# bruniss/multi-task-3d-resencoder-unet

Hardware: AMD Instinct MI355X
Metric: train patches/sec (b,c,z,y,x) ResEncM 1x128^3 (higher is better)
Workload: dtype bf16; 1 GPU; cfg2: ResEncM (6 stages, feats [32, 64, 128, 256, 512, 512], blocks [1, 3, 4, 6, 6, 6]), 1-in, heads ['sheet'], patch 128x128x128, batch 2/GPU, full train step (fwd+loss+bwd+allreduce+clip+AdamW); global_batch=2, parallelism=dp1

## Files before the change

include/rxunet.h:

```cpp
#ifndef RXUNET_H
#define RXUNET_H

#include <stddef.h>
#include <stdint.h>

#ifdef __cplusplus
extern "C" {
#endif

#define RX_OK 0
#define RX_EINVAL (-1)
#define RX_EUNSUPPORTED (-2)
#define RX_ELAUNCH (-3)
#define RX_EWORKSPACE (-4)

typedef enum { RX_F32 = 0, RX_BF16 = 1, RX_F16 = 2 } rx_dtype;
typedef enum { RX_ACT_NONE = 0, RX_ACT_SIGMOID = 1, RX_ACT_SOFTMAX = 2 } rx_head_act;

typedef struct {
  void* ptr;
  int32_t n, z, y, x, c, ld;
  int64_t cs;
} rx_act;

int rx_abi_version(void);
const char* rx_last_error(void);
int rx_device_arch_ok(void);
const char* rx_last_conv_kernel(void);

int rx_pack_conv_weight(rx_dtype dt, const float* w, int co, int ci, int taps, void* w_fwd, void* w_bwd,
                        void* stream);
int rx_pack_convT_weight(rx_dtype dt, const float* w, int ci, int co, int taps, void* w_fwd, void* w_bwd,
                         void* stream);
int rx_pack_multi(rx_dtype dt, int count, const float* const* w, const int* kind, const int* A, const int* B,
                  const int* taps, void* const* w_fwd, void* const* w_bwd, void* stream);

size_t rx_conv_workspace_hint(void);
int rx_conv3d_fwd(rx_dtype dt, const rx_act* x, const void* w_fwd, const float* bias, const rx_act* y,
                  const int32_t kernel[3], const int32_t stride[3], void* ws, size_t ws_bytes, void* stream);
int rx_conv3d_fwd_stats(rx_dtype dt, const rx_act* x, const void* w_fwd, const float* bias, const rx_act* y,
                        const int32_t kernel[3], const int32_t stride[3], float eps, float* stats, void* ws,
                        size_t ws_bytes, void* stream);
int rx_conv3d_bwd_data(rx_dtype dt, const rx_act* dy, const void* w_bwd, const rx_act* dx,
                       const int32_t kernel[3], const int32_t stride[3], int accumulate, void* ws,
                       size_t ws_bytes, void* stream);
int rx_conv3d_bwd_data_instats(rx_dtype dt, const rx_act* dy, const void* w_bwd, const rx_act* dx,
                               const int32_t kernel[3], const int32_t stride[3], int accumulate, const rx_act* in_y,
                               const float* in_stats, float slope, float* m12, int* fused, void* ws, size_t ws_bytes,
                               void* stream);
size_t rx_conv3d_bwd_weight_workspace(const rx_act* x, const rx_act* dy, const int32_t kernel[3]);
int rx_conv3d_bwd_weight(rx_dtype dt, const rx_act* x, const rx_act* dy, float* dw, const int32_t kernel[3],
                         const int32_t stride[3], void* ws, size_t ws_bytes, void* stream);

int rx_convT3d_fwd(rx_dtype dt, const rx_act* x, const void* w_fwd, const float* bias, const rx_act* y,
                   const int32_t stride[3], void* ws, size_t ws_bytes, void* stream);
int rx_convT3d_bwd_data(rx_dtype dt, const rx_act* dy, const void* w_bwd, const rx_act* dx,
                        const int32_t stride[3], int accumulate, void* ws, size_t ws_bytes, void* stream);
size_t rx_convT3d_bwd_weight_workspace(const rx_act* x, const rx_act* dy, const int32_t stride[3]);
int rx_convT3d_bwd_weight(rx_dtype dt, const rx_act* x, const rx_act* dy, float* dw, const int32_t stride[3],
                          void* ws, size_t ws_bytes, void* stream);

size_t rx_instnorm_stats_workspace(const rx_act* y);
int rx_instnorm_stats(rx_dtype dt, const rx_act* y, float eps, float* stats, void* ws, size_t ws_bytes,
                      void* stream);
int rx_instnorm_stats_mask(float* stats, const float* keep, int count, void* stream);
int rx_instnorm_act_fwd(rx_dtype dt, const rx_act* y, const float* stats, const rx_act* residual,
                        const rx_act* out, float slope, void* stream);
int rx_instnorm_fwd(rx_dtype dt, const rx_act* y, float eps, float* stats, const rx_act* residual,
                    const rx_act* out, float slope, void* ws, size_t ws_bytes, void* stream);
int rx_instnorm_act_bwd(rx_dtype dt, const rx_act* g, const rx_act* y, const float* stats, const rx_act* out,
                        float slope, const rx_act* dy, const rx_act* d_residual, int accumulate_residual,
                        void* ws, size_t ws_bytes, void* stream);

int rx_instnorm_act_bwd_res(rx_dtype dt, const rx_act* g, const rx_act* y, const float* stats, const rx_act* out,
                            float slope, const rx_act* pool_dy, const int32_t pool_stride[3], const rx_act* d_residual,
                            const rx_act* dy, void* ws, size_t ws_bytes, void* stream);

int rx_instnorm_act_bwd_apply(rx_dtype dt, const rx_act* g, const rx_act* y, const float* stats, const rx_act* out,
                              float slope, const float* m12, const rx_act* dy, const rx_act* d_residual,
                              int accumulate_residual, void* stream);

typedef struct {
  const float* w1;
  const float* b1;
  const float* w2;
  const float* b2;
  int32_t rd;
  int32_t keep_x;
} rx_se_params;
size_t rx_se_workspace(const rx_act* y);
int rx_se_gate_fwd(rx_dtype dt, const rx_act* y, const float* stats, const float* path_scale, const rx_se_params* se,
                   float* pooled, float* hidden, float* gate, float* mult, void* ws, size_t ws_bytes, void* stream);
int rx_instnorm_gate_act_fwd(rx_dtype dt, const rx_act* y, const float* stats, const float* mult, int keep_x,
                             const rx_act* residual, const rx_act* out, float slope, void* stream);
int rx_se_gate_bwd(rx_dtype dt, const rx_act* g, const rx_act* y, const float* stats, const rx_act* out, float slope,
                   const float* path_scale, const rx_se_params* se, const float* pooled, const float* hidden,
                   const float* gate, const float* mult, float* dadd, float* m12, float* dw1, float* db1, float* dw2,
                   float* db2, void* ws, size_t ws_bytes, void* stream);
int rx_instnorm_gate_act_bwd(rx_dtype dt, const rx_act* g, const rx_act* y, const float* stats, const rx_act* out,
                             float slope, const float* mult, const float* dadd, const float* m12, int keep_x,
                             const rx_act* dy, const rx_act* d_residual, int accumulate_residual, void* stream);

int rx_avgpool_fwd(rx_dtype dt, const rx_act* x, const rx_act* y, const int32_t stride[3], void* stream);
int rx_instnorm_act_pool_fwd(rx_dtype dt, const rx_act* y, const float* stats, const rx_act* residual,
                             const rx_act* out, const rx_act* pooled, const int32_t stride[3], float slope,
                             void* stream);
int rx_avgpool_bwd(rx_dtype dt, const rx_act* dy, const rx_act* dx, const int32_t stride[3], int accumulate,
                   void* stream);

int rx_stem_conv_fwd(rx_dtype dt, const float* x_ncdhw, int n, int cin, int z, int y, int x, const float* w,
                     const float* bias, const rx_act* out, const int32_t kernel[3], void* stream);
int rx_stem_conv_fwd_stats(rx_dtype dt, const float* x_ncdhw, int n, int cin, int z, int y, int x, const float* w,
                           const float* bias, const rx_act* out, const int32_t kernel[3], float eps, float* stats,
                           void* ws, size_t ws_bytes, void* stream);
size_t rx_stem_conv_bwd_weight_workspace(int cin, int cout, int taps);
int rx_stem_conv_bwd_weight(rx_dtype dt, const float* x_ncdhw, int n, int cin, int z, int y, int x,
                            const rx_act* dy, float* dw, const int32_t kernel[3], void* ws, size_t ws_bytes,
                            void* stream);

int rx_head_fwd(rx_dtype dt, const rx_act* x, const float* w, const float* b, int k, float* out_ncdhw,
                int act, void* stream);
size_t rx_head_bwd_workspace(const rx_act* x, int k);
int rx_head_bwd(rx_dtype dt, const float* dout_ncdhw, const rx_act* x, const float* w, int k, const rx_act* dx,
                float* dw, float* db, void* ws, size_t ws_bytes, void* stream);

int rx_instnorm_act_head_fwd(rx_dtype dt, const rx_act* y, const float* stats, const rx_act* out, float slope,
                             const float* head_w, const float* head_b, int k, float* out_ncdhw, int act, void* stream);

int rx_instnorm_act_bwd_head(rx_dtype dt, const float* dout_ncdhw, int k, const float* head_w, const rx_act* y,
                             const float* stats, float slope, const rx_act* dy, float* head_dw, float* head_db, void* ws,
                             size_t ws_bytes, void* stream);

size_t rx_channel_sum_workspace(const rx_act* x);
int rx_channel_sum(rx_dtype dt, const rx_act* x, float* out, void* ws, size_t ws_bytes, void* stream);

size_t rx_loss_workspace(int n, int c, long v);
int rx_bce_dice_loss_fwd(const float* logits, const float* target, int n, int c, long v, float alpha, float beta,
                         float smoothing, float eps, float* loss, float* coef, void* ws, size_t ws_bytes,
                         void* stream);
int rx_bce_dice_loss_bwd(const float* logits, const float* target, int n, int c, long v, float alpha, float beta,
                         float smoothing, const float* coef, const float* grad_loss, float* dlogits, void* stream);
int rx_masked_cosine_loss_fwd(const float* pred, const float* target, int n, int c, long v, float* loss, float* coef,
                              void* ws, size_t ws_bytes, void* stream);
int rx_masked_cosine_loss_bwd(const float* pred, const float* target, int n, int c, long v, const float* coef,
                              const float* grad_loss, float* dpred, void* stream);

typedef enum { RX_LOSS_BCE_LOGITS = 0, RX_LOSS_BCE_PROB = 1, RX_LOSS_MSE = 2 } rx_elem_loss_kind;
typedef enum { RX_REDUCE_MEAN = 0, RX_REDUCE_SUM = 1 } rx_reduction;
int rx_elem_loss_fwd(int kind, const float* x, const float* target, int n, int c, long v, float smoothing,
                     const float* alpha_z, int z, int reduction, float* loss, void* ws, size_t ws_bytes, void* stream);
int rx_elem_loss_bwd(int kind, const float* x, const float* target, int n, int c, long v, float smoothing,
                     const float* alpha_z, int z, int reduction, const float* grad_loss, float* dx, void* stream);
size_t rx_cross_entropy_loss_workspace(int n, int c, long v);
int rx_cross_entropy_loss_fwd(const float* logits, const float* target_prob, const int64_t* target_index,
                              int64_t ignore_index, int n, int c, long v, int reduction, float* loss, float* coef,
                              float* saved, void* ws, size_t ws_bytes, void* stream);
int rx_cross_entropy_loss_bwd(const float* logits, const float* target_prob, const int64_t* target_index,
                              int64_t ignore_index, int n, int c, long v, const float* coef, const float* saved,
                              const float* grad_loss, float* dlogits, void* stream);

int rx_adamw_pack(rx_dtype dt, float* p, const float* grad, float* exp_avg, float* exp_avg_sq, const float* clip, double lr,
                  double beta1, double beta2, double eps, double weight_decay, int step, int kind, int A, int B, int taps,
                  void* w_fwd, void* w_bwd, void* stream);
int rx_adamw_flat(float* p, const float* grad, float* exp_avg, float* exp_avg_sq, const float* clip, double lr, double beta1,
                  double beta2, double eps, double weight_decay, int step, long n, void* stream);
long rx_grad_norm_clip_partials(int count, const long* numel);
int rx_grad_norm_clip(int count, const float* const* grad, const long* numel, float max_norm, float* partial, long partial_len,
                      float* out, void* stream);
int rx_adamw_flat_multi(int count, float* const* p, const float* const* grad, float* const* exp_avg,
                        float* const* exp_avg_sq, const long* numel, const float* clip, double lr, double beta1,
                        double beta2, double eps, double weight_decay, int step, void* stream);

typedef struct rx_prog rx_prog;
rx_prog* rx_prog_create(void);
void rx_prog_destroy(rx_prog* p);
int rx_prog_begin(rx_prog* p, void* const* streams, int n_streams);
int rx_prog_end(rx_prog* p);
int rx_prog_len(const rx_prog* p);
const char* rx_prog_cmd_name(const rx_prog* p, int i);
const char* rx_prog_cmd_kernel(const rx_prog* p, int i);
int rx_prog_cmd_stream(const rx_prog* p, int i);
int rx_prog_run(rx_prog* p, int first, int last, void* const* streams, int n_streams, float* ms);
int rx_event_new(void);
int rx_event_free(int slot);
int rx_event_slots_in_use(void);
int rx_event_record(int slot, void* stream);
int rx_stream_wait(int slot, void* stream);

typedef enum { RX_SW_U8 = 0, RX_SW_U16 = 1, RX_SW_F32 = 2 } rx_sw_in_dtype;
typedef enum { RX_SW_SCALE = 0, RX_SW_ZSCORE = 1 } rx_sw_norm;
typedef enum { RX_SW_BLEND_AVERAGE = 0, RX_SW_BLEND_UNIT = 1, RX_SW_BLEND_NONE = 2 } rx_sw_blend;
typedef enum { RX_SW_CAST_U8 = 0, RX_SW_CAST_U16 = 1 } rx_sw_cast;
size_t rx_sw_gather_workspace(int batch, int cin, int pz, int py, int px);
int rx_sw_gather(int in_dtype, const void* slab, int cin, int ring, int y, int x, int batch, const int32_t* origins, int pz,
                 int py, int px, int norm, float* out, void* ws, size_t ws_bytes, void* stream);
int rx_sw_accumulate(const float* logits, int batch, int valid, int c, int pz, int py, int px, const int32_t* origins, int act,
                     const float* weight, float* sum, float* wsum, int ring, int y, int x, void* stream);
int rx_sw_finalize(float* sum, float* wsum, int c, int ring, int y, int x, int z0, int rows, int blend, int cast, int reset,
                   float* blended, void* final_out, float* wsum_out, void* stream);

#define RX_AUG_MAX_K 21
#define RX_AUG_MAX_BOXES 4
typedef enum { RX_AUG_PW_NONE = 0, RX_AUG_PW_AFFINE = 1, RX_AUG_PW_PLANE = 2, RX_AUG_PW_NOISE = 3 } rx_aug_pw_mode;
typedef enum { RX_AUG_G3_NONE = 0, RX_AUG_G3_FILTER = 1, RX_AUG_G3_DOWNSCALE = 2 } rx_aug_g3_mode;
typedef struct {
  int32_t pw_mode[2];
  float pw_a[2], pw_b[2];
  int32_t pw_off[2];
  uint32_t key_lo, key_hi;
  int32_t g3_mode, k, g3_off;
  int32_t nbox;
  int32_t box[RX_AUG_MAX_BOXES][6];
  float fill;
  int32_t pad_;
} rx_aug_sample;
size_t rx_aug_workspace(int batch, int c, int z, int y, int x);
int rx_aug_pointwise(const float* in, float* out, float* scratch, size_t scratch_bytes, int batch, int c, int z, int y, int x,
                     const rx_aug_sample* host_table, const void* table, long pool_words, void* stream);
int rx_aug_filter_zy(const float* scratch, float* out, int batch, int c, int z, int y, int x, const rx_aug_sample* host_table,
                     const void* table, long pool_words, void* stream);
int rx_aug_philox_u32(uint64_t key, long n, uint32_t* out, void* stream);

typedef struct {
  int32_t src_axis[3];
  int32_t flip[3];
  int32_t ch_src[3];
  int32_t ch_neg[3];
} rx_geom_sample;
int rx_geom_apply(const float* in, float* out, int batch, int c, int z, int y, int x, const rx_geom_sample* host_table,
                  int vector, void* stream);

int rx_sw_gather_geom(int in_dtype, const void* slab, int cin, int ring, int y, int x, int batch, const int32_t* origins,
                      const rx_geom_sample* ops, int pz, int py, int px, int norm, float* out, void* ws, size_t ws_bytes,
                      void* stream);
int rx_sw_accumulate_geom(const float* logits, int batch, int valid, int c, int pz, int py, int px, const int32_t* origins,
                          const rx_geom_sample* ops, int vector, int act, const float* weight, float* sum, float* wsum, int ring,
                          int y, int x, void* stream);

size_t rx_dilate_workspace(int batch, int c, int z, int y, int x);
int rx_label_dilate(const float* in, float* out, void* scratch, size_t scratch_bytes, int batch, int c, int z, int y, int x,
                    int radius, void* stream);

#ifdef __cplusplus
}
#endif
#endif
```

multi-task-3d-resencoder-unet_amd/csrc/rx_internal.h:

```cpp
#pragma once
#include "rx_common.h"

int rx_note_seq(void);

int rx_conv_halo_try(rx_dtype dt, const rx_act* in, const void* w, const float* bias, const rx_act* out, int flip, int accumulate,
                     hipStream_t st, float* stat_part, size_t stat_bytes, int* stat_chunks, const RxBwdStat* bs);
int rx_pointwise_try(rx_dtype dt, const rx_act* in, const void* w, const float* bias, const rx_act* out, const int32_t stride[3],
                     int accumulate, hipStream_t st);
int rx_dgrad_s2_halo_try(rx_dtype dt, const rx_act* dy, const void* w_bwd, const rx_act* dx, int accumulate, hipStream_t st);

size_t rx_wgrad_halo_ws_bytes(const rx_act* x, const rx_act* dy);
int rx_wgrad_halo_try(rx_dtype dt, const rx_act* x, const rx_act* dy, const int32_t stride[3], float* dw, void* ws, size_t ws_bytes,
                      hipStream_t st);
void rx_wgrad_reduce_launch(const float* slab, int S, int T_, int R, int C, float* dw, hipStream_t st);

int rx_stem_fwd_mfma_try(rx_dtype dt, const float* x, int n, int cin, int z, int y, int xx, const float* w, const float* bias,
                         const rx_act* out, const int32_t kernel[3], hipStream_t st, float* stat_part, size_t stat_bytes, int* stat_chunks);
int rx_stem_wgrad_mfma_try(rx_dtype dt, const float* x, int n, int cin, int z, int y, int xx, const rx_act* dy, const int32_t kernel[3],
                           float* partial, int max_blocks, int* nblocks_out, hipStream_t st);

void rx_colreduce_finalize_launch(hipStream_t st, const float* partial, int N, int nchunks, int nacc, int C, double V, float eps, int mode,
                                  float* out);
void rx_stats_finalize_launch(const float* partial, int N, int nchunks, int C, double V, float eps, float* stats, hipStream_t st);
void rx_inbwd_fused_finalize_launch(const float* partial, int N, int nchunks, int C, double V, const float* stats, float* m12, hipStream_t st);
```

multi-task-3d-resencoder-unet_amd/csrc/rx_pack_optim.hip:

```cpp
#include <math.h>

#include "rx_common.h"

#define RX_PACK_PB 40
#ifndef RX_PACK_THREADS
#define RX_PACK_THREADS 1024
#endif

template <typename T>
__device__ __forceinline__ void pack_tile(const float* __restrict__ w, int A, int B, int TT, unsigned inv_tt, T* __restrict__ same,
                                          int flip_same, T* __restrict__ swp, int flip_swap, const int a0, const int b0) {
  extern __shared__ __attribute__((aligned(16))) unsigned char pack_smem[];
  T* L = reinterpret_cast<T*>(pack_smem);
  const int rowlen = 32 * TT;
  const bool full = a0 + 32 <= A && b0 + 32 <= B && sizeof(T) == 2 && (B & 7) == 0 && (A & 7) == 0;
  if (full && TT > 1 && (rowlen & 3) == 0 && ((size_t)B * TT & 3) == 0) {
    const int q4 = rowlen >> 2;
    for (int q = threadIdx.x; q < 32 * q4; q += RX_PACK_THREADS) {
      const int a = q / q4, c = q - a * q4;
      const f32x4 v = *reinterpret_cast<const f32x4*>(w + ((size_t)(a0 + a) * B + b0) * TT + 4 * c);
#pragma unroll
      for (int j = 0; j < 4; ++j) {
        const unsigned r = 4 * c + j;
        const unsigned b = __umulhi(r, inv_tt), t = r - b * TT;
// ... 380 lines not shown
        pm[j][k] = mj, pv[j][k] = vj;
      }
      *reinterpret_cast<f32x4*>(w + i) = pw[j];
      *reinterpret_cast<f32x4*>(m + i) = pm[j];
      *reinterpret_cast<f32x4*>(v + i) = pv[j];
    }
    return;
  }
  const long end = base + RX_AM_CHUNK < n ? base + RX_AM_CHUNK : n;
  for (long i = base + threadIdx.x; i < end; i += 256) {
    float mj = m[i], vj = v[i];
    w[i] = adamw_update(w[i], grad[i] * cs, mj, vj, aa);
    m[i] = mj, v[i] = vj;
  }
}

extern "C" int rx_adamw_flat_multi(int count, float* const* p, const float* const* grad, float* const* exp_avg, float* const* exp_avg_sq,
                                   const long* numel, const float* clip, double lr, double beta1, double beta2, double eps,
                                   double weight_decay, int step, void* stream) {
  if (count < 0 || (count > 0 && (!p || !grad || !exp_avg || !exp_avg_sq || !numel)) || step < 1) RX_FAIL(RX_EINVAL, "rx_adamw_flat_multi: bad arguments");
  const AdamArgs aa = adam_args(lr, beta1, beta2, eps, weight_decay, step);
  for (int i = 0; i < count; ++i)
    if (!p[i] || !grad[i] || !exp_avg[i] || !exp_avg_sq[i] || numel[i] < 1) RX_FAIL(RX_EINVAL, "rx_adamw_flat_multi: bad tensor %d", i);
  for (int i0 = 0; i0 < count;) {
    AdamMulti t;
    int k = 0;
    long blocks = 0;
    for (; i0 + k < count && k < RX_AM_MAX; ++k) {
      const long nb = (numel[i0 + k] + RX_AM_CHUNK - 1) / RX_AM_CHUNK;
      if (blocks + nb > 0x3fffffffL) break;
      t.p[k] = p[i0 + k], t.g[k] = grad[i0 + k], t.m[k] = exp_avg[i0 + k], t.v[k] = exp_avg_sq[i0 + k], t.n[k] = numel[i0 + k];
      t.start[k] = (int)blocks;
      blocks += nb;
    }
    if (k == 0) RX_FAIL(RX_EINVAL, "rx_adamw_flat_multi: tensor %d too large", i0);
    for (int q = k; q <= RX_AM_MAX; ++q) t.start[q] = (int)blocks;
    for (int q = k; q < RX_AM_MAX; ++q) t.p[q] = nullptr, t.g[q] = nullptr, t.m[q] = nullptr, t.v[q] = nullptr, t.n[q] = 0;
    t.count = k;
    hipLaunchKernelGGL(adamw_multi_kernel, dim3((unsigned)blocks), dim3(256), 0, (hipStream_t)stream, t, clip, aa);
    i0 += k;
  }
  RX_CHECK_LAUNCH("rx_adamw_flat_multi");
  return RX_OK;
}

struct SqnormMulti {
  const float* g[RX_AM_MAX];
  long n[RX_AM_MAX];
  int start[RX_AM_MAX + 1];
  int count;
};

__global__ __launch_bounds__(256) void sqnorm_multi_kernel(const SqnormMulti t, float* __restrict__ partial) {
  __shared__ float red[4];
  const int b = blockIdx.x;
  int lo = 0, hi = t.count;
  while (hi - lo > 1) {
    const int mid = (lo + hi) >> 1;
    if (t.start[mid] <= b) lo = mid; else hi = mid;
  }
  const long base = (long)(b - t.start[lo]) * RX_AM_CHUNK;
  const long n = t.n[lo];
  const float* __restrict__ g = t.g[lo];
  float s = 0.f;
  if ((((uintptr_t)g) & 15) == 0 && base + RX_AM_CHUNK <= n) {
    f32x4 v[4];
#pragma unroll
    for (int j = 0; j < 4; ++j) v[j] = *reinterpret_cast<const f32x4*>(g + base + (long)(j * 256 + threadIdx.x) * 4);
#pragma unroll
    for (int j = 0; j < 4; ++j)
#pragma unroll
      for (int k = 0; k < 4; ++k) s += v[j][k] * v[j][k];
  } else {
    const long end = base + RX_AM_CHUNK < n ? base + RX_AM_CHUNK : n;
    for (long i = base + threadIdx.x; i < end; i += 256) s += g[i] * g[i];
  }
  for (int o = 32; o > 0; o >>= 1) s += __shfl_xor(s, o, 64);
  if ((threadIdx.x & 63) == 0) red[threadIdx.x >> 6] = s;
  __syncthreads();
  if (threadIdx.x == 0) partial[b] = (red[0] + red[1]) + (red[2] + red[3]);
}

__global__ __launch_bounds__(1024) void sqnorm_finalize_kernel(const float* __restrict__ partial, int nblocks, float max_norm,
                                                               float* __restrict__ out ) {
  __shared__ double red[1024];
  double s[8] = {0.0, 0.0, 0.0, 0.0, 0.0, 0.0, 0.0, 0.0};
  int i = threadIdx.x;
  for (; i + 7 * 1024 < nblocks; i += 8 * 1024) {
    float v[8];
#pragma unroll
    for (int u = 0; u < 8; ++u) v[u] = partial[i + u * 1024];
#pragma unroll
    for (int u = 0; u < 8; ++u) s[u] += (double)v[u];
  }
  for (; i < nblocks; i += 1024) s[0] += (double)partial[i];
  red[threadIdx.x] = ((s[0] + s[1]) + (s[2] + s[3])) + ((s[4] + s[5]) + (s[6] + s[7]));
  __syncthreads();
  for (int o = 512; o > 0; o >>= 1) {
    if ((int)threadIdx.x < o) red[threadIdx.x] += red[threadIdx.x + o];
    __syncthreads();
  }
  if (threadIdx.x == 0) {
    const float norm = (float)sqrt(red[0]);
    const float coef = max_norm / (norm + 1e-6f);
    out[0] = norm;
    out[1] = coef < 1.f ? coef : 1.f;
  }
}

extern "C" long rx_grad_norm_clip_partials(int count, const long* numel) {
  long blocks = 0;
  for (int i = 0; i < count; ++i) blocks += (numel[i] + RX_AM_CHUNK - 1) / RX_AM_CHUNK;
  return blocks;
}

extern "C" int rx_grad_norm_clip(int count, const float* const* grad, const long* numel, float max_norm, float* partial, long partial_len,
                                 float* out, void* stream) {
  if (count < 1 || !grad || !numel || !partial || !out) RX_FAIL(RX_EINVAL, "rx_grad_norm_clip: bad arguments");
  const long need = rx_grad_norm_clip_partials(count, numel);
  if (need > partial_len || need > 0x3fffffffL) RX_FAIL(RX_EWORKSPACE, "rx_grad_norm_clip: %ld partials needed, %ld given", need, partial_len);
  long done = 0;
  for (int i0 = 0; i0 < count;) {
    SqnormMulti t;
    int k = 0;
    long blocks = 0;
    for (; i0 + k < count && k < RX_AM_MAX; ++k) {
      if (!grad[i0 + k] || numel[i0 + k] < 1) RX_FAIL(RX_EINVAL, "rx_grad_norm_clip: bad tensor %d", i0 + k);
      t.g[k] = grad[i0 + k], t.n[k] = numel[i0 + k];
      t.start[k] = (int)blocks;
      blocks += (numel[i0 + k] + RX_AM_CHUNK - 1) / RX_AM_CHUNK;
    }
    for (int q = k; q <= RX_AM_MAX; ++q) t.start[q] = (int)blocks;
    for (int q = k; q < RX_AM_MAX; ++q) t.g[q] = nullptr, t.n[q] = 0;
    t.count = k;
    hipLaunchKernelGGL(sqnorm_multi_kernel, dim3((unsigned)blocks), dim3(256), 0, (hipStream_t)stream, t, partial + done);
    done += blocks;
    i0 += k;
  }
  hipLaunchKernelGGL(sqnorm_finalize_kernel, dim3(1), dim3(1024), 0, (hipStream_t)stream, (const float*)partial, (int)done, max_norm, out);
  RX_CHECK_LAUNCH("rx_grad_norm_clip");
  return RX_OK;
}
```

multi-task-3d-resencoder-unet_amd/csrc/rx_wgrad.hip:

```cpp
#include <stdlib.h>

#include "rx_common.h"
#include "rx_internal.h"


struct WgradGeom {
  int Qz, Qy, Qx, Vq, NQ;
  int R, ldg;
  long g_ss;
  int Zx, Yx, Xx, Cc, ldx;
  long x_ss;
  int isz, isy, isx;
  int ntaps, ksplit, q_per_split, tiles_c;
  RxTap taps[RX_MAX_TAPS];
};


typedef __attribute__((address_space(3))) s16x4 lds_s16x4;

template <typename T>
__device__ inline u32x4 fetch_frag(const T* panel, int ks, int lane) {
  if constexpr (sizeof(T) == 2) {
    const int g16 = lane >> 4, half = g16 & 1, h = g16 >> 1, l15 = lane & 15, q4 = l15 >> 2, p4 = l15 & 3;
    const T* a0 = panel + (ks * 16 + 8 * h + q4) * 32 + 16 * half + 4 * p4;
// ... 50 lines not shown
        const int n = q / g.Vq, vq = q - n * g.Vq;
        const int qx = vq % g.Qx, t = vq / g.Qx;
        const int qy = t % g.Qy, qz = t / g.Qy;
        const int z = qz * g.isz + tp.dz, y = qy * g.isy + tp.dy, x = qx * g.isx + tp.dx;
        if ((unsigned)z < (unsigned)g.Zx && (unsigned)y < (unsigned)g.Yx && (unsigned)x < (unsigned)g.Xx)
          v = *reinterpret_cast<const u32x4*>(xt + n * g.x_ss + ((long)(z * g.Yx + y) * g.Xx + x) * g.ldx + c0 + cv * P);
      }
      xr[j] = v;
    }
  };
  auto store_tile = [&](int buf) {
    T* base = sbuf + buf * TILE_ELEMS;
#pragma unroll
    for (int j = 0; j < GV; ++j) {
      const int i = tid + 256 * j, vox = i / (BR / P), cv = i - vox * (BR / P);
      const int c = cv * P;
      *reinterpret_cast<u32x4*>(base + ((c >> 5) * 64 + vox) * 32 + (c & 31)) = gr[j];
    }
    T* xb = base + 64 * BR;
#pragma unroll
    for (int j = 0; j < XV; ++j) {
      const int i = tid + 256 * j, vox = i / (BC / P), cv = i - vox * (BC / P);
      const int c = cv * P;
      *reinterpret_cast<u32x4*>(xb + ((c >> 5) * 64 + vox) * 32 + (c & 31)) = xr[j];
    }
  };

  f32x16 acc[NR][NC];
#pragma unroll
  for (int a = 0; a < NR; ++a)
#pragma unroll
    for (int b = 0; b < NC; ++b)
#pragma unroll
      for (int r = 0; r < 16; ++r) acc[a][b][r] = 0.f;

  if (q_begin < q_end) {
    load_tile(q_begin);
    store_tile(0);
  }
  __syncthreads();
  int it = 0;
  for (int q0 = q_begin; q0 < q_end; q0 += 64, ++it) {
    const int buf = it & 1;
    if (q0 + 64 < q_end) load_tile(q0 + 64);
    const T* base = sbuf + buf * TILE_ELEMS;
#pragma unroll
    for (int kk = 0; kk < KSTEPS / 4; ++kk) {
      const int ks = wave + 4 * kk;
      u32x4 af[NR], bf[NC];
#pragma unroll
      for (int a = 0; a < NR; ++a) af[a] = fetch_frag<T>(base + a * 64 * 32, ks, lane);
#pragma unroll
      for (int b = 0; b < NC; ++b) bf[b] = fetch_frag<T>(base + 64 * BR + b * 64 * 32, ks, lane);
#pragma unroll
      for (int a = 0; a < NR; ++a)
#pragma unroll
        for (int b = 0; b < NC; ++b) Mma<T>::run(acc[a][b], af[a], bf[b]);
    }
    if (q0 + 64 < q_end) store_tile(buf ^ 1);
    __syncthreads();
  }

  float* red = reinterpret_cast<float*>(smem);
  const int col = lane & 31, fh = lane >> 5;
#pragma unroll
  for (int a = 0; a < NR; ++a)
#pragma unroll
    for (int b = 0; b < NC; ++b)
#pragma unroll
      for (int r = 0; r < 16; ++r) {
        const int row = (r & 3) + 8 * (r >> 2) + 4 * fh;
        red[(((wave * NR + a) * NC + b) * 32 + row) * 32 + col] = acc[a][b][r];
      }
  __syncthreads();
  float* out = slab + ((long)blockIdx.z * g.ntaps + blockIdx.y) * g.R * g.Cc;
  for (int i = tid; i < NR * NC * 1024; i += 256) {
    const int blk = i >> 10, rc = i & 1023, row = rc >> 5, cc = rc & 31;
    const int a = blk / NC, b = blk - a * NC;
    float s = red[i] + red[i + NR * NC * 1024] + red[i + 2 * NR * NC * 1024] + red[i + 3 * NR * NC * 1024];
    out[(long)(r0 + a * 32 + row) * g.Cc + c0 + b * 32 + cc] = s;
  }
}

__global__ __launch_bounds__(256) void wgrad_reduce(const float* __restrict__ slab, int S, int T_, int R, int C, float* __restrict__ dw) {
  __shared__ float tile[27 * 257];
  const long RC = (long)R * C;
  const long base = (long)blockIdx.x * 256;
  const long i = base + threadIdx.x;
  for (int t = 0; t < T_; ++t) {
    float s = 0.f;
    if (i < RC)
      for (int k = 0; k < S; ++k) s += slab[((long)k * T_ + t) * RC + i];
    tile[t * 257 + threadIdx.x] = s;
  }
  __syncthreads();
  const long n_here = (RC - base < 256 ? RC - base : 256) * T_;
  for (long j = threadIdx.x; j < n_here; j += 256) {
    int pair = (int)(j / T_), t = (int)(j - (long)pair * T_);
    dw[base * T_ + j] = tile[t * 257 + pair];
  }
}

__global__ __launch_bounds__(256) void wgrad_reduce_manysplits(const float* __restrict__ slab, int S, int T_, int R, int C,
                                                               float* __restrict__ dw) {
  const long RC = (long)R * C;
  const long i = (long)blockIdx.x * 256 + threadIdx.x;
  const int t = blockIdx.y;
  if (i >= RC) return;
  const float* p = slab + (long)t * RC + i;
  const long stride = (long)T_ * RC;
  float a0 = 0.f, a1 = 0.f, a2 = 0.f, a3 = 0.f, a4 = 0.f, a5 = 0.f, a6 = 0.f, a7 = 0.f;
  int k = 0;
  for (; k + 8 <= S; k += 8) {
    a0 += p[(k + 0) * stride];
    a1 += p[(k + 1) * stride];
    a2 += p[(k + 2) * stride];
    a3 += p[(k + 3) * stride];
    a4 += p[(k + 4) * stride];
    a5 += p[(k + 5) * stride];
    a6 += p[(k + 6) * stride];
    a7 += p[(k + 7) * stride];
  }
  for (; k < S; ++k) a0 += p[k * stride];
  dw[i * T_ + t] = ((a0 + a1) + (a2 + a3)) + ((a4 + a5) + (a6 + a7));
}

static int plan_split(const WgradGeom& g, int BR, int BC, size_t ws_bytes, int* ksplit, int* qps) {
  const long tiles = (long)(g.R / BR) * (g.Cc / BC) * g.ntaps;
  const long ktiles = ((long)g.NQ + 63) / 64;
  long S = (1024 + tiles - 1) / tiles;
  if (S > ktiles / 4) S = ktiles / 4;
  if (S < 1) S = 1;
  const size_t slab1 = (size_t)g.ntaps * g.R * g.Cc * sizeof(float);
  while (S > 1 && S * slab1 > ws_bytes) --S;
  if (slab1 > ws_bytes) return RX_EWORKSPACE;
  long per = (ktiles + S - 1) / S;
  S = (ktiles + per - 1) / per;
  *ksplit = (int)S;
  *qps = (int)(per * 64);
  return RX_OK;
}

static size_t wgrad_ws_bytes(int R, int C, int taps, long NQ) {
  const size_t slab1 = (size_t)taps * R * C * sizeof(float);
  const long tiles = (long)((R + 63) / 64) * ((C + 63) / 64) * taps;
  long S = (1024 + tiles - 1) / tiles;
  long ktiles = (NQ + 63) / 64;
  if (S > ktiles / 4) S = ktiles / 4;
  if (S < 1) S = 1;
  if (R % 64 || C % 64) {
    const long t32 = (long)(R / 32) * (C / 32) * taps;
    long S2 = (1024 + t32 - 1) / t32;
    if (S2 > S) S = S2;
  }
  return S * slab1 + 256;
}

template <typename T>
static void wgrad_dispatch(int BR, int BC, dim3 grid, hipStream_t st, const void* gt, const void* xt, float* slab, const WgradGeom& g) {
  const size_t lds = 65536;
#define RX_WG(BR_, BC_)                                                                                                            \
  do {                                                                                                                             \
    (void)hipFuncSetAttribute(reinterpret_cast<const void*>(&wgrad_kernel<T, BR_, BC_>), hipFuncAttributeMaxDynamicSharedMemorySize, \
                              (int)lds);                                                                                           \
    hipLaunchKernelGGL((wgrad_kernel<T, BR_, BC_>), grid, dim3(256), lds, st, (const T*)gt, (const T*)xt, slab, g);                \
  } while (0)
  if (BR == 64 && BC == 64)
    RX_WG(64, 64);
  else if (BR == 64 && BC == 32)
    RX_WG(64, 32);
  else if (BR == 32 && BC == 64)
    RX_WG(32, 64);
  else
    RX_WG(32, 32);
#undef RX_WG
}

static int wgrad_launch(rx_dtype dt, const void* gt, const void* xt, float* dw, WgradGeom& g, void* ws, size_t ws_bytes, hipStream_t st) {
  const int per16 = dt == RX_F32 ? 4 : 8;
  if (g.R % 32 || g.Cc % 32) RX_FAIL(RX_EUNSUPPORTED, "wgrad: channel counts must be multiples of 32 (R=%d C=%d)", g.R, g.Cc);
  if (g.ldg % per16 || g.ldx % per16 || ((uintptr_t)gt & 15) || ((uintptr_t)xt & 15)) RX_FAIL(RX_EUNSUPPORTED, "wgrad: misaligned operand");
  if (!ws || !dw) RX_FAIL(RX_EINVAL, "wgrad: null workspace / output");
  const int BR = g.R % 64 == 0 ? 64 : 32, BC = g.Cc % 64 == 0 ? 64 : 32;
  g.tiles_c = g.Cc / BC;
  int rc = plan_split(g, BR, BC, ws_bytes, &g.ksplit, &g.q_per_split);
  if (rc) RX_FAIL(rc, "wgrad: workspace too small (%zu bytes)", ws_bytes);
  dim3 grid((g.R / BR) * (g.Cc / BC), g.ntaps, g.ksplit);
  rx_note_kernel(BR == 64 ? (BC == 64 ? "wgrad_kernel<64,64>" : "wgrad_kernel<64,32>") : (BC == 64 ? "wgrad_kernel<32,64>" : "wgrad_kernel<32,32>"));
  RX_DISPATCH_DTYPE(dt, T, wgrad_dispatch<T>(BR, BC, grid, st, gt, xt, (float*)ws, g));
  rx_wgrad_reduce_launch((const float*)ws, g.ksplit, g.ntaps, g.R, g.Cc, dw, st);
  RX_CHECK_LAUNCH("wgrad");
  return RX_OK;
}

static int conv_out_dim(int in, int k, int s) { return (in + 2 * ((k - 1) / 2) - k) / s + 1; }

void rx_wgrad_reduce_launch(const float* slab, int S, int T_, int R, int C, float* dw, hipStream_t st) {
  long RC = (long)R * C;
  if (S >= 8 || T_ > 27)
    hipLaunchKernelGGL(wgrad_reduce_manysplits, dim3((unsigned)((RC + 255) / 256), T_), dim3(256), 0, st, slab, S, T_, R, C, dw);
  else
    hipLaunchKernelGGL(wgrad_reduce, dim3((unsigned)((RC + 255) / 256)), dim3(256), 0, st, slab, S, T_, R, C, dw);
}

extern "C" size_t rx_conv3d_bwd_weight_workspace(const rx_act* x, const rx_act* dy, const int32_t kernel[3]) {
  if (!rx_act_ok_planar(x) || !rx_act_ok(dy)) return 0;
  size_t a = wgrad_ws_bytes(dy->c, x->c, kernel[0] * kernel[1] * kernel[2], (long)dy->n * rx_act_voxels(dy));
  size_t b = (kernel[0] == 3 && kernel[1] == 3 && kernel[2] == 3) ? rx_wgrad_halo_ws_bytes(x, dy) : 0;
  return a > b ? a : b;
}

extern "C" int rx_conv3d_bwd_weight(rx_dtype dt, const rx_act* x, const rx_act* dy, float* dw, const int32_t kernel[3],
                                    const int32_t stride[3], void* ws, size_t ws_bytes, void* stream) {
  RX_RECORD(stream, [=, x_ = RxActV(x), dy_ = RxActV(dy), kernel_ = RxI3V(kernel), stride_ = RxI3V(stride)](void* s) { return rx_conv3d_bwd_weight(dt, x_.p(), dy_.p(), dw, kernel_.v, stride_.v, ws, ws_bytes, s); });
  if (!rx_act_ok_planar(x) || !rx_act_ok(dy)) RX_FAIL(RX_EINVAL, "rx_conv3d_bwd_weight: bad arguments");
  for (int i = 0; i < 3; ++i) {
    if (kernel[i] < 1 || kernel[i] > RX_MAX_KERNEL) RX_FAIL(RX_EUNSUPPORTED, "rx_conv3d_bwd_weight: kernel sizes must be 1..%d per axis", RX_MAX_KERNEL);
    if (stride[i] < 1 || stride[i] > RX_MAX_STRIDE) RX_FAIL(RX_EUNSUPPORTED, "rx_conv3d_bwd_weight: strides must be 1..%d per axis", RX_MAX_STRIDE);
  }
  if (dy->n != x->n || dy->z != conv_out_dim(x->z, kernel[0], stride[0]) || dy->y != conv_out_dim(x->y, kernel[1], stride[1]) ||
      dy->x != conv_out_dim(x->x, kernel[2], stride[2]))
    RX_FAIL(RX_EINVAL, "rx_conv3d_bwd_weight: geometry mismatch");
  if (kernel[0] == 3 && kernel[1] == 3 && kernel[2] == 3 && ws && dw) {
    int rc = rx_wgrad_halo_try(dt, x, dy, stride, dw, ws, ws_bytes, (hipStream_t)stream);
    if (rc < 0) return rc;
    if (rc == 1) return RX_OK;
  }
  if (x->cs) RX_FAIL(RX_EUNSUPPORTED, "rx_conv3d_bwd_weight: a planar-concat x needs the LDS-halo weight-gradient kernels");
  WgradGeom g;
  memset(&g, 0, sizeof(g));
  g.Qz = dy->z, g.Qy = dy->y, g.Qx = dy->x, g.Vq = (int)rx_act_voxels(dy), g.NQ = dy->n * g.Vq;
  g.R = dy->c, g.ldg = dy->ld, g.g_ss = (long)g.Vq * dy->ld;
  g.Zx = x->z, g.Yx = x->y, g.Xx = x->x, g.Cc = x->c, g.ldx = x->ld, g.x_ss = rx_act_voxels(x) * (long)x->ld;
  g.isz = stride[0], g.isy = stride[1], g.isx = stride[2];
  const int pz = (kernel[0] - 1) / 2, py = (kernel[1] - 1) / 2, px = (kernel[2] - 1) / 2;
  for (int a = 0; a < kernel[0]; ++a)
    for (int b = 0; b < kernel[1]; ++b)
      for (int c = 0; c < kernel[2]; ++c) {
        RxTap& t = g.taps[g.ntaps];
        t.dz = (int8_t)(a - pz), t.dy = (int8_t)(b - py), t.dx = (int8_t)(c - px);
        t.w = (uint16_t)g.ntaps;
        ++g.ntaps;
      }
  return wgrad_launch(dt, dy->ptr, x->ptr, dw, g, ws, ws_bytes, (hipStream_t)stream);
}

struct ConvTWgGeom {
  int Vq, NQ, Qy, Qx;
  int R, ldr;
  long r_ss;
  int Yf, Xf, Cc, ldc;
  long c_ss;
  int sz, sy, sx, ntaps;
  int q_per_split;
};

template <typename T, int NR, int NC>
__global__ __launch_bounds__(512) void convT_wgrad_kernel(const T* __restrict__ xt, const T* __restrict__ yt, float* __restrict__ slab,
                                                          const ConvTWgGeom g) {
  constexpr int P = Elem<T>::PER16;
  constexpr int BR = 32 * NR, BC = 32 * NC;
  constexpr int XV = (64 * BR / P + 511) / 512;
  constexpr int YV = (64 * BC / P + 511) / 512;
  extern __shared__ __attribute__((aligned(16))) unsigned char smem[];
  T* sX = reinterpret_cast<T*>(smem);
  T* sY = sX + 64 * BR;
  const int tid = threadIdx.x, lane = tid & 63;
  const int wave = __builtin_amdgcn_readfirstlane(tid >> 6);
  const int q_begin = blockIdx.x * g.q_per_split;
  const int q_end = min(g.NQ, q_begin + g.q_per_split);

  u32x4 xr[XV], yr[8][YV];
  auto load_tile = [&](int q0) {
#pragma unroll
    for (int j = 0; j < XV; ++j) {
      const int i = tid + 512 * j, vox = i / (BR / P), cv = i - vox * (BR / P);
      const int q = q0 + vox;
      u32x4 v = u32x4{0u, 0u, 0u, 0u};
      if (vox < 64 && q < q_end) {
        const int n = q / g.Vq, vq = q - n * g.Vq;
        v = *reinterpret_cast<const u32x4*>(xt + n * g.r_ss + (long)vq * g.ldr + cv * P);
      }
      xr[j] = v;
    }
#pragma unroll
    for (int j = 0; j < YV; ++j) {
      const int i = tid + 512 * j, vox = i / (BC / P), cv = i - vox * (BC / P);
      const int q = q0 + vox;
      const bool ok = vox < 64 && q < q_end;
      const int n = ok ? q / g.Vq : 0, vq = ok ? q - n * g.Vq : 0;
      const int qx = vq % g.Qx, t2 = vq / g.Qx;
      const int qy = t2 % g.Qy, qz = t2 / g.Qy;
      const T* base = yt + n * g.c_ss + cv * P;
#pragma unroll
      for (int t = 0; t < 8; ++t) {
        u32x4 v = u32x4{0u, 0u, 0u, 0u};
        if (ok && t < g.ntaps) {
          const int c = t % g.sx, b = (t / g.sx) % g.sy, a = t / (g.sx * g.sy);
          const long fv = ((long)(qz * g.sz + a) * g.Yf + (qy * g.sy + b)) * g.Xf + (qx * g.sx + c);
          v = *reinterpret_cast<const u32x4*>(base + fv * g.ldc);
        }
        yr[t][j] = v;
      }
    }
  };
  auto store_tile = [&]() {
#pragma unroll
    for (int j = 0; j < XV; ++j) {
      const int i = tid + 512 * j, vox = i / (BR / P), cv = i - vox * (BR / P);
      const int c = cv * P;
      if (vox < 64) *reinterpret_cast<u32x4*>(sX + ((c >> 5) * 64 + vox) * 32 + (c & 31)) = xr[j];
    }
#pragma unroll
    for (int j = 0; j < YV; ++j) {
      const int i = tid + 512 * j, vox = i / (BC / P), cv = i - vox * (BC / P);
      const int c = cv * P;
      if (vox < 64) {
#pragma unroll
        for (int t = 0; t < 8; ++t)
          if (t < g.ntaps) *reinterpret_cast<u32x4*>(sY + (long)t * 64 * BC + ((c >> 5) * 64 + vox) * 32 + (c & 31)) = yr[t][j];
      }
    }
  };

  f32x16 acc[NR][NC];
#pragma unroll
  for (int a = 0; a < NR; ++a)
#pragma unroll
    for (int b = 0; b < NC; ++b)
#pragma unroll
      for (int r = 0; r < 16; ++r) acc[a][b][r] = 0.f;

  if (q_begin < q_end) load_tile(q_begin);
  for (int q0 = q_begin; q0 < q_end; q0 += 64) {
    __syncthreads();
    store_tile();
    __syncthreads();
    if (q0 + 64 < q_end) load_tile(q0 + 64);
    if (wave < g.ntaps) {
      const T* yb = sY + (long)wave * 64 * BC;
#pragma unroll
      for (int ks = 0; ks < 4; ++ks) {
        u32x4 af[NR], bf[NC];
#pragma unroll
        for (int a = 0; a < NR; ++a) af[a] = fetch_frag<T>(sX + a * 64 * 32, ks, lane);
#pragma unroll
        for (int b = 0; b < NC; ++b) bf[b] = fetch_frag<T>(yb + b * 64 * 32, ks, lane);
#pragma unroll
        for (int a = 0; a < NR; ++a)
#pragma unroll
          for (int b = 0; b < NC; ++b) Mma<T>::run(acc[a][b], af[a], bf[b]);
      }
    }
  }
  if (wave < g.ntaps) {
    const int col = lane & 31, fh = lane >> 5;
    float* out = slab + ((long)blockIdx.x * g.ntaps + wave) * g.R * g.Cc;
#pragma unroll
    for (int a = 0; a < NR; ++a)
#pragma unroll
      for (int b = 0; b < NC; ++b)
#pragma unroll
        for (int r = 0; r < 16; ++r) {
          const int row = (r & 3) + 8 * (r >> 2) + 4 * fh;
          out[(long)(a * 32 + row) * g.Cc + b * 32 + col] = acc[a][b][r];
        }
  }
}

static int convT_wgrad_splits(long NQ, size_t slab1) {
  long ktiles = (NQ + 63) / 64;
  long S = ktiles / 8;
  if (S > 256) S = 256;
  while (S > 32 && (size_t)S * slab1 > ((size_t)32 << 20)) S /= 2;
  if (S < 1) S = 1;
  return (int)S;
}

static int convT_wgrad_try(rx_dtype dt, const rx_act* x, const rx_act* dy, const int32_t stride[3], float* dw, void* ws, size_t ws_bytes,
                           hipStream_t st) {
  const int taps = stride[0] * stride[1] * stride[2];
  const int R = x->c, C = dy->c;
  if (dt == RX_F32 || taps > 8 || R % 32 || C % 32 || x->ld % 8 || dy->ld % 8 || ((uintptr_t)x->ptr & 15) || ((uintptr_t)dy->ptr & 15)) return 0;
  const int NR = R / 32, NC = C / 32;
  if (!((NR == 2 && NC == 1) || (NR == 4 && NC == 2) || (NR == 1 && NC == 1) || (NR == 2 && NC == 2))) return 0;
  const long NQ = (long)x->n * rx_act_voxels(x);
  if (NQ < 32768) return 0;
  const size_t slab1 = (size_t)taps * R * C * sizeof(float);
  const int S = convT_wgrad_splits(NQ, slab1);
  if ((size_t)S * slab1 > ws_bytes) return 0;
  ConvTWgGeom g;
  g.Vq = (int)rx_act_voxels(x), g.NQ = (int)NQ, g.Qy = x->y, g.Qx = x->x;
  g.R = R, g.ldr = x->ld, g.r_ss = (long)g.Vq * x->ld;
  g.Yf = dy->y, g.Xf = dy->x, g.Cc = C, g.ldc = dy->ld, g.c_ss = rx_act_voxels(dy) * (long)dy->ld;
  g.sz = stride[0], g.sy = stride[1], g.sx = stride[2], g.ntaps = taps;
  const long ktiles = (NQ + 63) / 64;
  g.q_per_split = (int)(((ktiles + S - 1) / S) * 64);
  const int S2 = (int)((NQ + g.q_per_split - 1) / g.q_per_split);
  const size_t lds = (size_t)64 * (R + taps * C) * 2;
  rx_note_kernel("convT_wgrad_kernel");
#define RX_CTW(NR_, NC_)                                                                                                              \
  do {                                                                                                                                \
    (void)hipFuncSetAttribute(reinterpret_cast<const void*>(&convT_wgrad_kernel<T, NR_, NC_>), hipFuncAttributeMaxDynamicSharedMemorySize, 160 * 1024); \
    hipLaunchKernelGGL((convT_wgrad_kernel<T, NR_, NC_>), dim3(S2), dim3(512), lds, st, (const T*)x->ptr, (const T*)dy->ptr, (float*)ws, g);            \
  } while (0)
#define RX_CTW_ALL()                       \
  if (NR == 2 && NC == 1) RX_CTW(2, 1);    \
  else if (NR == 4 && NC == 2) RX_CTW(4, 2); \
  else if (NR == 1 && NC == 1) RX_CTW(1, 1); \
  else RX_CTW(2, 2)
  if (dt == RX_BF16) {
    using T = bf16_t;
    RX_CTW_ALL();
  } else {
    using T = f16_t;
    RX_CTW_ALL();
  }
#undef RX_CTW_ALL
#undef RX_CTW
  rx_wgrad_reduce_launch((const float*)ws, S2, taps, R, C, dw, st);
  return 1;
}

extern "C" size_t rx_convT3d_bwd_weight_workspace(const rx_act* x, const rx_act* dy, const int32_t stride[3]) {
  if (!rx_act_ok(x) || !rx_act_ok(dy)) return 0;
  const int taps = stride[0] * stride[1] * stride[2];
  const long NQ = (long)x->n * rx_act_voxels(x);
  const size_t slab1 = (size_t)taps * x->c * dy->c * sizeof(float);
  const size_t a = wgrad_ws_bytes(x->c, dy->c, taps, NQ);
  const size_t b = (size_t)convT_wgrad_splits(NQ, slab1) * slab1 + 256;
  return a > b ? a : b;
}

extern "C" int rx_convT3d_bwd_weight(rx_dtype dt, const rx_act* x, const rx_act* dy, float* dw, const int32_t stride[3], void* ws,
                                     size_t ws_bytes, void* stream) {
  RX_RECORD(stream, [=, x_ = RxActV(x), dy_ = RxActV(dy), stride_ = RxI3V(stride)](void* s) { return rx_convT3d_bwd_weight(dt, x_.p(), dy_.p(), dw, stride_.v, ws, ws_bytes, s); });
  if (!rx_act_ok(x) || !rx_act_ok(dy)) RX_FAIL(RX_EINVAL, "rx_convT3d_bwd_weight: bad arguments");
  for (int i = 0; i < 3; ++i)
    if (stride[i] < 1 || stride[i] > RX_MAX_STRIDE) RX_FAIL(RX_EUNSUPPORTED, "rx_convT3d_bwd_weight: strides must be 1..%d per axis", RX_MAX_STRIDE);
  if (dy->n != x->n || dy->z != x->z * stride[0] || dy->y != x->y * stride[1] || dy->x != x->x * stride[2])
    RX_FAIL(RX_EINVAL, "rx_convT3d_bwd_weight: geometry mismatch");
  if (ws && dw) {
    const int rc = convT_wgrad_try(dt, x, dy, stride, dw, ws, ws_bytes, (hipStream_t)stream);
    if (rc < 0) return rc;
    if (rc == 1) {
      RX_CHECK_LAUNCH("rx_convT3d_bwd_weight(convT_wgrad)");
      return RX_OK;
    }
  }
  WgradGeom g;
  memset(&g, 0, sizeof(g));
  g.Qz = x->z, g.Qy = x->y, g.Qx = x->x, g.Vq = (int)rx_act_voxels(x), g.NQ = x->n * g.Vq;
  g.R = x->c, g.ldg = x->ld, g.g_ss = (long)g.Vq * x->ld;
  g.Zx = dy->z, g.Yx = dy->y, g.Xx = dy->x, g.Cc = dy->c, g.ldx = dy->ld, g.x_ss = rx_act_voxels(dy) * (long)dy->ld;
  g.isz = stride[0], g.isy = stride[1], g.isx = stride[2];
  for (int a = 0; a < stride[0]; ++a)
    for (int b = 0; b < stride[1]; ++b)
      for (int c = 0; c < stride[2]; ++c) {
        RxTap& t = g.taps[g.ntaps];
        t.dz = (int8_t)a, t.dy = (int8_t)b, t.dx = (int8_t)c;
        t.w = (uint16_t)g.ntaps;
        ++g.ntaps;
      }
  return wgrad_launch(dt, x->ptr, dy->ptr, dw, g, ws, ws_bytes, (hipStream_t)stream);
}
```

multi-task-3d-resencoder-unet_amd/csrc/rx_wgrad_halo.hip:

```cpp
#include <stdlib.h>

#include <type_traits>

#include "rx_common.h"
#include "rx_internal.h"

struct WgHaloGeom {
  int N, Z, Y, X;
  int R, Cc, ldg, ldx;
  long g_ss, x_ss;
  long x_cs;
  int TZ, TY, TX, lTX, lTY;
  int HY, HX, HV, VT;
  int tz_n, ty_n, tx_n, NT;
  int S, tiles_per_split, panels_c;
  int sz, sy, sx;
  int Zi, Yi, Xi;
  int order;
  int dbg;
};

typedef __attribute__((address_space(3))) s16x4 lds_s16x4_h;

#define RX_WGH_MAX_HV 768
#define RX_WGH_MAX_VT 256
#define RX_WGH_XPIECES ((RX_WGH_MAX_HV * 4 + 255) / 256)
#define RX_WGH_GPIECES (RX_WGH_MAX_VT * 4 / 256)

template <typename T>
__device__ inline u32x4 tr_frag(const T* p0, const T* p1) {
  s16x4 t0 = __builtin_amdgcn_ds_read_tr16_b64_v4i16((lds_s16x4_h*)(p0));
  s16x4 t1 = __builtin_amdgcn_ds_read_tr16_b64_v4i16((lds_s16x4_h*)(p1));
  u32x2 lo = __builtin_bit_cast(u32x2, t0), hi = __builtin_bit_cast(u32x2, t1);
  return u32x4{lo[0], lo[1], hi[0], hi[1]};
}

template <typename T>
__global__ __launch_bounds__(256, 2) void wgrad_halo_kernel(const T* __restrict__ gt, const T* __restrict__ xt, float* __restrict__ slab,
                                                            float* __restrict__ dw, const WgHaloGeom g) {
  extern __shared__ __attribute__((aligned(16))) unsigned char smem[];
  T* sG = reinterpret_cast<T*>(smem);
  T* sX = sG + RX_WGH_MAX_VT * 32;

  const int tid = threadIdx.x, lane = tid & 63;
  const int wave = __builtin_amdgcn_readfirstlane(tid >> 6);
  const int PPn = gridDim.x, lid = rx_xcd_remap(blockIdx.y * PPn + blockIdx.x, PPn * gridDim.y);
  const int split = lid / PPn, pp = lid - split * PPn;
  const int pr = pp / g.panels_c, pc = pp - pr * g.panels_c;
  const int r0 = pr * 32, c0 = pc * 32;
  const long xc0 = g.x_cs ? (long)pc * g.x_cs : (long)c0;
  const int t_begin = split * g.tiles_per_split;
  const int t_end = min(g.NT, t_begin + g.tiles_per_split);

  const int chunk = tid & 3;
  int xh[RX_WGH_XPIECES];
#pragma unroll
  for (int p = 0; p < RX_WGH_XPIECES; ++p) {
    int row = (tid >> 2) + 64 * p;
    if (row < g.HV) {
      int hx = row % g.HX, t = row / g.HX;
      int hy = t % g.HY, hz = t / g.HY;
      xh[p] = (hz << 16) | (hy << 8) | hx;
    } else
      xh[p] = -1;
  }

  const int g16 = lane >> 4, half = g16 & 1, h = g16 >> 1, l15 = lane & 15, q4 = l15 >> 2, p4 = l15 & 3;
  const int coloff = 16 * half + 4 * p4;
  int toff[7];
#pragma unroll
  for (int j = 0; j < 7; ++j) {
    int t = wave + 4 * j;
    int dz = t / 9 - 1, dy = (t / 3) % 3 - 1, dx = t % 3 - 1;
    toff[j] = t < 27 ? ((dz * g.HY + dy) * g.HX + dx) * 32 : 0;
  }

  f32x16 acc[7];
#pragma unroll
  for (int j = 0; j < 7; ++j)
#pragma unroll
    for (int r = 0; r < 16; ++r) acc[j][r] = 0.f;

  const int ksteps = g.VT >> 4;
  u32x4 gv[RX_WGH_GPIECES], xv[RX_WGH_XPIECES];
  auto load_tile = [&](int tile) {
    int tx, ty, tz, n;
    rx_tile_coords(tile, g.tx_n, g.ty_n, g.tz_n, g.order, n, tz, ty, tx);
    const int z0 = tz * g.TZ, y0 = ty * g.TY, x0 = tx * g.TX;
    const T* gn = gt + n * g.g_ss + r0;
    const T* xn = xt + n * g.x_ss + xc0;
#pragma unroll
    for (int p = 0; p < RX_WGH_GPIECES; ++p) {
      int v = (tid >> 2) + 64 * p;
      u32x4 val = u32x4{0u, 0u, 0u, 0u};
      if (v < g.VT) {
        int vx = v & (g.TX - 1), vy = (v >> g.lTX) & (g.TY - 1), vz = v >> (g.lTX + g.lTY);
        int z = z0 + vz, y = y0 + vy, x = x0 + vx;
        if (z < g.Z && y < g.Y && x < g.X)
          val = *reinterpret_cast<const u32x4*>(gn + ((long)(z * g.Y + y) * g.X + x) * g.ldg + chunk * 8);
      }
      gv[p] = val;
    }
#pragma unroll
    for (int p = 0; p < RX_WGH_XPIECES; ++p) {
      u32x4 val = u32x4{0u, 0u, 0u, 0u};
      if (xh[p] >= 0) {
        int z = z0 * g.sz + (xh[p] >> 16) - 1, y = y0 * g.sy + ((xh[p] >> 8) & 255) - 1, x = x0 * g.sx + (xh[p] & 255) - 1;
        if ((unsigned)z < (unsigned)g.Zi && (unsigned)y < (unsigned)g.Yi && (unsigned)x < (unsigned)g.Xi)
          val = *reinterpret_cast<const u32x4*>(xn + ((long)(z * g.Yi + y) * g.Xi + x) * g.ldx + chunk * 8);
      }
      xv[p] = val;
    }
  };
  if (t_begin < t_end) load_tile(t_begin);
  for (int tile = t_begin; tile < t_end; ++tile) {
    __syncthreads();
#pragma unroll
    for (int p = 0; p < RX_WGH_GPIECES; ++p) {
      int v = (tid >> 2) + 64 * p;
      if (v < g.VT) *reinterpret_cast<u32x4*>(sG + v * 32 + chunk * 8) = gv[p];
    }
#pragma unroll
    for (int p = 0; p < RX_WGH_XPIECES; ++p) {
      int row = (tid >> 2) + 64 * p;
      if (xh[p] >= 0) *reinterpret_cast<u32x4*>(sX + row * 32 + chunk * 8) = xv[p];
    }
    __syncthreads();
    if (tile + 1 < t_end) load_tile(tile + 1);
    for (int s = 0; s < ksteps; ++s) {
      const int v = 16 * s + 8 * h + q4;
      const int vx = v & (g.TX - 1), vy = (v >> g.lTX) & (g.TY - 1), vz = v >> (g.lTX + g.lTY);
      const int hr = ((vz * g.sz + 1) * g.HY + (vy * g.sy + 1)) * g.HX + vx * g.sx + 1;
      int hr4;
      if (g.TX >= 8)
        hr4 = hr + 4 * g.sx;
      else {
        const int v2 = v + 4;
        const int vy2 = (v2 >> g.lTX) & (g.TY - 1), vz2 = v2 >> (g.lTX + g.lTY);
        hr4 = ((vz2 * g.sz + 1) * g.HY + (vy2 * g.sy + 1)) * g.HX + (v2 & (g.TX - 1)) * g.sx + 1;
      }
      const u32x4 a = tr_frag<T>(sG + v * 32 + coloff, sG + (v + 4) * 32 + coloff);
      const T* b0 = sX + hr * 32 + coloff;
      const T* b1 = sX + hr4 * 32 + coloff;
      u32x4 bf[7];
#pragma unroll
      for (int j = 0; j < 7; ++j)
        if (j < 6 || wave < 3) bf[j] = tr_frag<T>(b0 + toff[j], b1 + toff[j]);
      __builtin_amdgcn_sched_barrier(0);
#pragma unroll
      for (int j = 0; j < 7; ++j)
        if (j < 6 || wave < 3) Mma<T>::run(acc[j], a, bf[j]);
      __builtin_amdgcn_sched_barrier(0);
    }
  }

  const int col = lane & 31, fh = lane >> 5;
  if (g.S == 1) {
    float* sT = reinterpret_cast<float*>(smem);
#pragma unroll
    for (int hb = 0; hb < 2; ++hb) {
      __syncthreads();
#pragma unroll
      for (int j = 0; j < 7; ++j) {
        const int t = wave + 4 * j;
        if (t < 27) {
#pragma unroll
          for (int r = 8 * hb; r < 8 * hb + 8; ++r) {
            const int lr = (r & 3) + 8 * ((r >> 2) & 1) + 4 * fh;
            sT[(lr * 32 + col) * 27 + t] = acc[j][r];
          }
        }
      }
      __syncthreads();
      for (int idx = tid; idx < 16 * 216; idx += 256) {
        const int lr = idx / 216, i = idx - lr * 216;
        *reinterpret_cast<f32x4*>(dw + ((long)(r0 + 16 * hb + lr) * g.Cc + c0) * 27 + 4 * i) = *reinterpret_cast<const f32x4*>(sT + 4 * idx);
      }
    }
    return;
  }
#pragma unroll
  for (int j = 0; j < 7; ++j) {
    const int t = wave + 4 * j;
    if (t < 27) {
      float* out = slab + (((long)split * 27 + t) * g.R + r0) * g.Cc + c0;
#pragma unroll
      for (int r = 0; r < 16; ++r) {
        const int row = (r & 3) + 8 * (r >> 2) + 4 * fh;
        out[(long)row * g.Cc + col] = acc[j][r];
      }
    }
  }
}


typedef __attribute__((address_space(3))) unsigned char lds_byte;

__device__ inline u32x4 tr_frag_at(const lds_byte* p, int off0, int off1) {
  s16x4 t0 = __builtin_amdgcn_ds_read_tr16_b64_v4i16((lds_s16x4_h*)(p + off0));
  s16x4 t1 = __builtin_amdgcn_ds_read_tr16_b64_v4i16((lds_s16x4_h*)(p + off1));
  u32x2 lo = __builtin_bit_cast(u32x2, t0), hi = __builtin_bit_cast(u32x2, t1);
  return u32x4{lo[0], lo[1], hi[0], hi[1]};
}

#define WGH16_HY 6
#define WGH16_HX 18
#define WGH16_HV 648
#define WGH16_XPIECES 11

template <typename T, int W, typename Stage>
__device__ __forceinline__ void wgh16_tile_mma(const lds_byte* gb, const lds_byte* xb, f32x16 (&acc)[7], Stage&& stage) {
  constexpr int NT = W < 3 ? 7 : 6;
  u32x4 fa[2], fb[7];
  auto read_a = [&](int s) { return tr_frag_at(gb, s * 1024, s * 1024 + 256); };
  auto read_b = [&](int s, int j) {
    const int vy = s & 3, vz = s >> 2;
    const int t = W + 4 * j;
    const int dz = t / 9, dy = (t / 3) % 3, dx = t % 3;
    const int off = (((vz + dz) * WGH16_HY + (vy + dy)) * WGH16_HX + dx) * 64;
    return tr_frag_at(xb, off, off + 256);
  };
  fa[0] = read_a(0);
#pragma unroll
  for (int j = 0; j < NT; ++j) fb[j] = read_b(0, j);
#pragma unroll
  for (int s = 0; s < 16; ++s) {
    if (s + 1 < 16) fa[(s + 1) & 1] = read_a(s + 1);
    __builtin_amdgcn_sched_barrier(0);
#pragma unroll
    for (int j = 0; j < NT; ++j) {
      Mma<T>::run(acc[j], fa[s & 1], fb[j]);
      if (s + 1 < 16) fb[j] = read_b(s + 1, j);
      __builtin_amdgcn_sched_barrier(0);
    }
    stage(s);
    __builtin_amdgcn_sched_barrier(0);
  }
}

#define WGH16_BUF_BYTES ((256 + WGH16_HV) * 64)

template <typename T, bool DMA>
__global__ __launch_bounds__(512, 1) void wgrad_halo16ws_kernel(const T* __restrict__ gt, const T* __restrict__ xt, float* __restrict__ slab,
                                                                float* __restrict__ dw, const WgHaloGeom g) {
  extern __shared__ __attribute__((aligned(16))) unsigned char smem[];
  const int tid = threadIdx.x, lane = tid & 63;
  const int wave = __builtin_amdgcn_readfirstlane(tid >> 6);
  const int PPn = gridDim.x, lid = rx_xcd_remap(blockIdx.y * PPn + blockIdx.x, PPn * gridDim.y);
  const int split = lid / PPn, pp = lid - split * PPn;
  const int pr = pp / g.panels_c, pc = pp - pr * g.panels_c;
  const int r0 = pr * 32, c0 = pc * 32;
  const long xc0 = g.x_cs ? (long)pc * g.x_cs : (long)c0;
  const int t_begin = split * g.tiles_per_split;
  const int t_end = min(g.NT, t_begin + g.tiles_per_split);

  f32x16 acc[7];
  if (wave >= 4) {
    const int ptid = tid - 256, chunk = ptid & 3;
    int xh[WGH16_XPIECES];
#pragma unroll
    for (int p = 0; p < WGH16_XPIECES; ++p) {
// ... 42 lines not shown
      __amdgpu_buffer_rsrc_t rG = __builtin_amdgcn_make_buffer_rsrc((void*)gt, 0, (unsigned)(gbytes > 0xfffffff0L ? 0xfffffff0L : gbytes), 0x00020000);
      __amdgpu_buffer_rsrc_t rX = __builtin_amdgcn_make_buffer_rsrc((void*)xt, 0, (unsigned)(xbytes > 0xfffffff0L ? 0xfffffff0L : xbytes), 0x00020000);
      const int pw = wave - 4;
      auto dma_tile = [&](int tile, int buf) {
        int tx, ty, tz, n;
        rx_tile_coords(tile, g.tx_n, g.ty_n, g.tz_n, g.order, n, tz, ty, tx);
        const int z0 = tz * 4, y0 = ty * 4, x0 = tx * 16;
        const unsigned gbase = (unsigned)((n * g.g_ss + r0 + chunk * 8) * 2);
        const unsigned xbase = (unsigned)((n * g.x_ss + xc0 + chunk * 8) * 2);
        __attribute__((address_space(3))) unsigned char* lG =
            (__attribute__((address_space(3))) unsigned char*)(smem + buf * WGH16_BUF_BYTES) + 1024 * pw;
        __attribute__((address_space(3))) unsigned char* lX = lG + 256 * 64;
#pragma unroll
        for (int p = 0; p < 4; ++p) {
          const int v = (ptid >> 2) + 64 * p;
          const int z = z0 + (v >> 6), y = y0 + ((v >> 4) & 3), x = x0 + (v & 15);
          const unsigned off = (z < g.Z && y < g.Y && x < g.X) ? gbase + (unsigned)(((z * g.Y + y) * g.X + x) * g.ldg * 2) : OOB;
          __builtin_amdgcn_raw_ptr_buffer_load_lds(rG, (__attribute__((address_space(3))) void*)(lG + 4096 * p), 16, off, 0, 0, 0);
        }
#pragma unroll
        for (int p = 0; p < WGH16_XPIECES; ++p) {
          if (xh[p] >= 0) {
            const int z = z0 + (xh[p] >> 16) - 1, y = y0 + ((xh[p] >> 8) & 255) - 1, x = x0 + (xh[p] & 255) - 1;
            const bool ok = (unsigned)z < (unsigned)g.Z && (unsigned)y < (unsigned)g.Y && (unsigned)x < (unsigned)g.X;
            const unsigned off = ok ? xbase + (unsigned)(((z * g.Y + y) * g.X + x) * g.ldx * 2) : OOB;
            __builtin_amdgcn_raw_ptr_buffer_load_lds(rX, (__attribute__((address_space(3))) void*)(lX + 4096 * p), 16, off, 0, 0, 0);
          }
        }
      };
      if (t_begin < t_end) dma_tile(t_begin, 0);
      asm volatile("s_waitcnt vmcnt(0)" ::: "memory");
      __syncthreads();
      for (int tile = t_begin; tile < t_end; ++tile) {
        const int buf = (tile - t_begin) & 1;
        if (tile + 1 < t_end) dma_tile(tile + 1, buf ^ 1);
        asm volatile("s_waitcnt vmcnt(0)" ::: "memory");
        __syncthreads();
      }
    } else {
    if (t_begin < t_end) {
      load_tile(t_begin);
      commit(0);
      if (t_begin + 1 < t_end) load_tile(t_begin + 1);
    }
    __syncthreads();
    for (int tile = t_begin; tile < t_end; ++tile) {
      const int buf = (tile - t_begin) & 1;
      if (tile + 1 < t_end) {
        commit(buf ^ 1);
        if (tile + 2 < t_end) load_tile(tile + 2);
      }
      __syncthreads();
    }
    }
  } else {
#pragma unroll
    for (int j = 0; j < 7; ++j)
#pragma unroll
      for (int r = 0; r < 16; ++r) acc[j][r] = 0.f;
    const int g16 = lane >> 4, half = g16 & 1, h = g16 >> 1, l15 = lane & 15, q4 = l15 >> 2, p4 = l15 & 3;
    const int lane_off = ((8 * h + q4) * 32 + 16 * half + 4 * p4) * 2;
    auto stage = [](int) {};
    auto run = [&](auto wc) {
      constexpr int W = decltype(wc)::value;
      __syncthreads();
      for (int tile = t_begin; tile < t_end; ++tile) {
        const int buf = (tile - t_begin) & 1;
        const lds_byte* gb = (const lds_byte*)(smem) + buf * WGH16_BUF_BYTES + lane_off;
        if (!RX_ABLATE(g, 2)) wgh16_tile_mma<T, W>(gb, gb + 256 * 64, acc, stage);
        __syncthreads();
      }
    };
    switch (wave) {
      case 0: run(std::integral_constant<int, 0>{}); break;
      case 1: run(std::integral_constant<int, 1>{}); break;
      case 2: run(std::integral_constant<int, 2>{}); break;
      default: run(std::integral_constant<int, 3>{}); break;
    }
  }

  const int col = lane & 31, fh = lane >> 5;
  if (g.S == 1) {
    float* sT = reinterpret_cast<float*>(smem);
#pragma unroll
    for (int hb = 0; hb < 2; ++hb) {
      __syncthreads();
      if (wave < 4) {
#pragma unroll
        for (int j = 0; j < 7; ++j) {
          const int t = wave + 4 * j;
          if (t < 27) {
#pragma unroll
            for (int r = 8 * hb; r < 8 * hb + 8; ++r) {
              const int lr = (r & 3) + 8 * ((r >> 2) & 1) + 4 * fh;
              sT[(lr * 32 + col) * 27 + t] = acc[j][r];
            }
          }
        }
      }
      __syncthreads();
      for (int idx = tid; idx < 16 * 216; idx += 512) {
        const int lr = idx / 216, i = idx - lr * 216;
        *reinterpret_cast<f32x4*>(dw + ((long)(r0 + 16 * hb + lr) * g.Cc + c0) * 27 + 4 * i) = *reinterpret_cast<const f32x4*>(sT + 4 * idx);
      }
    }
    return;
  }
  if (wave < 4) {
#pragma unroll
    for (int j = 0; j < 7; ++j) {
      const int t = wave + 4 * j;
      if (t < 27) {
        float* out = slab + (((long)split * 27 + t) * g.R + r0) * g.Cc + c0;
#pragma unroll
        for (int r = 0; r < 16; ++r) {
          const int row = (r & 3) + 8 * (r >> 2) + 4 * fh;
          out[(long)row * g.Cc + col] = acc[j][r];
        }
      }
    }
  }
}

static int p2ceil(int v) {
  int p = 1;
  while (p < v) p <<= 1;
  return p;
}
static int ilog2(int v) {
  int l = 0;
  while ((1 << l) < v) ++l;
  return l;
}

static int wgh_plan(const rx_act* x, const rx_act* dy, const int32_t stride[3], WgHaloGeom* g, size_t ws_bytes) {
  memset(g, 0, sizeof(*g));
  g->N = dy->n, g->Z = dy->z, g->Y = dy->y, g->X = dy->x;
  g->Zi = x->z, g->Yi = x->y, g->Xi = x->x;
  g->sz = stride[0], g->sy = stride[1], g->sx = stride[2];
  g->R = dy->c, g->Cc = x->c, g->ldg = dy->ld, g->ldx = x->ld;
  g->g_ss = rx_act_voxels(dy) * (long)dy->ld;
  g->x_ss = rx_act_voxels(x) * (long)x->ld;
  g->x_cs = x->cs;
  const bool strided = stride[0] > 1 || stride[1] > 1 || stride[2] > 1;
  int TX = p2ceil(g->X);
  TX = TX < 4 ? 4 : (TX > 16 ? 16 : TX);
  if (strided && TX > 8) TX = 8;
  int budget = strided ? 64 : 256;
  int rem = budget / TX;
  int TY = p2ceil(g->Y);
  int capy = TX == 16 ? 4 : (strided ? 4 : 8);
  if (TY > capy) TY = capy;
  if (TY > rem) TY = rem;
  int TZ = p2ceil(g->Z);
  if (TZ > rem / TY) TZ = rem / TY;
  g->TZ = TZ, g->TY = TY, g->TX = TX, g->lTX = ilog2(TX), g->lTY = ilog2(TY);
  g->VT = TZ * TY * TX;
  const int HZ = g->sz * (TZ - 1) + 3;
  g->HY = g->sy * (TY - 1) + 3, g->HX = g->sx * (TX - 1) + 3, g->HV = HZ * g->HY * g->HX;
  if (g->VT < 16 || g->VT > RX_WGH_MAX_VT || g->HV > RX_WGH_MAX_HV || HZ > 255 || g->HY > 255 || g->HX > 255) return 0;
  g->tz_n = (g->Z + TZ - 1) / TZ, g->ty_n = (g->Y + TY - 1) / TY, g->tx_n = (g->X + TX - 1) / TX;
  g->NT = g->N * g->tz_n * g->ty_n * g->tx_n;
  g->panels_c = g->Cc / 32;
  const long PP = (long)(g->R / 32) * g->panels_c;
  long target = (!strided && TZ == 4 && TY == 4 && TX == 16) ? 256 : 512;
  if (target == 256 && g->NT * PP < 16 * 256) target = 512;
  long S = (target + PP - 1) / PP;
  if (PP >= 256) S = 1;
  if (S > g->NT) S = g->NT;
  if (S < 1) S = 1;
  const size_t slab1 = (size_t)27 * g->R * g->Cc * sizeof(float);
  while (S > 1 && S * slab1 > ws_bytes) --S;
  if (S > 1 && slab1 > ws_bytes) return 0;
  g->tiles_per_split = (int)((g->NT + S - 1) / S);
  g->S = (g->NT + g->tiles_per_split - 1) / g->tiles_per_split;
  return 1;
}

size_t rx_wgrad_halo_ws_bytes(const rx_act* x, const rx_act* dy) {
  const long PP = (long)(dy->c / 32) * (x->c / 32);
  long S = PP > 0 ? (512 + PP - 1) / PP : 1;
  return (size_t)S * 27 * dy->c * x->c * sizeof(float) + 256;
}

int rx_wgrad_halo_try(rx_dtype dt, const rx_act* x, const rx_act* dy, const int32_t stride[3], float* dw, void* ws, size_t ws_bytes,
                      hipStream_t st) {
  if (dt == RX_F32) return 0;
  if (x->c % 32 || dy->c % 32 || x->ld % 8 || dy->ld % 8 || ((uintptr_t)x->ptr & 15) || ((uintptr_t)dy->ptr & 15)) return 0;
  WgHaloGeom g;
  if (!wgh_plan(x, dy, stride, &g, ws_bytes)) return 0;
  const size_t lds = (size_t)(RX_WGH_MAX_VT + RX_WGH_MAX_HV) * 64;
  dim3 grid((g.R / 32) * g.panels_c, g.S);
  static const int dbg = rx_env_mask("RX_DBG");
  g.dbg = dbg;
  g.order = 1;
  if (g.TZ == 4 && g.TY == 4 && g.TX == 16 && g.sz == 1 && g.sy == 1 && g.sx == 1) {
    const size_t lds16 = (size_t)WGH16_BUF_BYTES;
    (void)hipFuncSetAttribute(reinterpret_cast<const void*>(&wgrad_halo16ws_kernel<bf16_t, false>), hipFuncAttributeMaxDynamicSharedMemorySize, (int)(2 * lds16));
    (void)hipFuncSetAttribute(reinterpret_cast<const void*>(&wgrad_halo16ws_kernel<f16_t, false>), hipFuncAttributeMaxDynamicSharedMemorySize, (int)(2 * lds16));
    (void)hipFuncSetAttribute(reinterpret_cast<const void*>(&wgrad_halo16ws_kernel<bf16_t, true>), hipFuncAttributeMaxDynamicSharedMemorySize, (int)(2 * lds16));
    (void)hipFuncSetAttribute(reinterpret_cast<const void*>(&wgrad_halo16ws_kernel<f16_t, true>), hipFuncAttributeMaxDynamicSharedMemorySize, (int)(2 * lds16));
    rx_note_kernel("wgrad_halo16ws_kernel");
    const bool dma_ok = (long)g.N * g.g_ss * 2 < 0x7fffff00L &&
                        ((long)g.N * g.x_ss + (g.x_cs ? (long)(g.Cc / 32 - 1) * g.x_cs : 0)) * 2 < 0x7fffff00L;
    if (dma_ok && dt == RX_BF16)
      hipLaunchKernelGGL((wgrad_halo16ws_kernel<bf16_t, true>), grid, dim3(512), 2 * lds16, st, (const bf16_t*)dy->ptr, (const bf16_t*)x->ptr, (float*)ws, dw, g);
    else if (dma_ok)
      hipLaunchKernelGGL((wgrad_halo16ws_kernel<f16_t, true>), grid, dim3(512), 2 * lds16, st, (const f16_t*)dy->ptr, (const f16_t*)x->ptr, (float*)ws, dw, g);
    else if (dt == RX_BF16)
      hipLaunchKernelGGL((wgrad_halo16ws_kernel<bf16_t, false>), grid, dim3(512), 2 * lds16, st, (const bf16_t*)dy->ptr, (const bf16_t*)x->ptr, (float*)ws, dw, g);
    else
      hipLaunchKernelGGL((wgrad_halo16ws_kernel<f16_t, false>), grid, dim3(512), 2 * lds16, st, (const f16_t*)dy->ptr, (const f16_t*)x->ptr, (float*)ws, dw, g);
    if (g.S > 1) rx_wgrad_reduce_launch((const float*)ws, g.S, 27, g.R, g.Cc, dw, st);
    hipError_t e16 = hipGetLastError();
    if (e16 != hipSuccess) {
      rx_set_error("wgrad_halo16: %s", hipGetErrorString(e16));
      return RX_ELAUNCH;
    }
    return 1;
  }
  rx_note_kernel("wgrad_halo_kernel");
  if (dt == RX_BF16) {
    (void)hipFuncSetAttribute(reinterpret_cast<const void*>(&wgrad_halo_kernel<bf16_t>), hipFuncAttributeMaxDynamicSharedMemorySize, (int)lds);
    hipLaunchKernelGGL((wgrad_halo_kernel<bf16_t>), grid, dim3(256), lds, st, (const bf16_t*)dy->ptr, (const bf16_t*)x->ptr, (float*)ws, dw, g);
  } else {
    (void)hipFuncSetAttribute(reinterpret_cast<const void*>(&wgrad_halo_kernel<f16_t>), hipFuncAttributeMaxDynamicSharedMemorySize, (int)lds);
    hipLaunchKernelGGL((wgrad_halo_kernel<f16_t>), grid, dim3(256), lds, st, (const f16_t*)dy->ptr, (const f16_t*)x->ptr, (float*)ws, dw, g);
  }
  if (g.S > 1) rx_wgrad_reduce_launch((const float*)ws, g.S, 27, g.R, g.Cc, dw, st);
  hipError_t e = hipGetLastError();
  if (e != hipSuccess) {
    rx_set_error("wgrad_halo: %s", hipGetErrorString(e));
    return RX_ELAUNCH;
  }
  return 1;
}
```

multi-task-3d-resencoder-unet_amd/engine/lib.py:

```python
import ctypes
import os
from ctypes import POINTER, c_char_p, c_double, c_float, c_int, c_int32, c_long, c_size_t, c_void_p

import torch

_HERE = os.path.dirname(os.path.abspath(__file__))
LIB_PATH = os.environ.get("RX_LIBRARY") or os.path.join(os.path.dirname(_HERE), "csrc", "librxunet.so")

RX_F32, RX_BF16, RX_F16 = 0, 1, 2
RX_ACT_NONE, RX_ACT_SIGMOID, RX_ACT_SOFTMAX = 0, 1, 2
DTYPE_CODE = {torch.float32: RX_F32, torch.bfloat16: RX_BF16, torch.float16: RX_F16}
RX_SW_U8, RX_SW_U16, RX_SW_F32 = 0, 1, 2
RX_SW_SCALE, RX_SW_ZSCORE = 0, 1
RX_SW_BLEND_AVERAGE, RX_SW_BLEND_UNIT, RX_SW_BLEND_NONE = 0, 1, 2
RX_SW_CAST_U8, RX_SW_CAST_U16 = 0, 1
RX_AUG_PW_NONE, RX_AUG_PW_AFFINE, RX_AUG_PW_PLANE, RX_AUG_PW_NOISE = 0, 1, 2, 3
RX_AUG_G3_NONE, RX_AUG_G3_FILTER, RX_AUG_G3_DOWNSCALE = 0, 1, 2
RX_AUG_MAX_K, RX_AUG_MAX_BOXES = 21, 4
RX_LOSS_BCE_LOGITS, RX_LOSS_BCE_PROB, RX_LOSS_MSE = 0, 1, 2
RX_REDUCE_MEAN, RX_REDUCE_SUM = 0, 1


class RxError(RuntimeError):
    pass


class RxAct(ctypes.Structure):
    _fields_ = [("ptr", c_void_p), ("n", c_int32), ("z", c_int32), ("y", c_int32), ("x", c_int32),
                ("c", c_int32), ("ld", c_int32), ("cs", ctypes.c_int64)]


class RxSeParams(ctypes.Structure):
    _fields_ = [("w1", c_void_p), ("b1", c_void_p), ("w2", c_void_p), ("b2", c_void_p), ("rd", c_int32),
                ("keep_x", c_int32)]


I3 = c_int32 * 3
_P = POINTER(RxAct)
_PSE = POINTER(RxSeParams)

_SIGNATURES = {
    "rx_abi_version": (c_int, []),
    "rx_last_error": (c_char_p, []),
    "rx_device_arch_ok": (c_int, []),
    "rx_last_conv_kernel": (c_char_p, []),
    "rx_pack_conv_weight": (c_int, [c_int, c_void_p, c_int, c_int, c_int, c_void_p, c_void_p, c_void_p]),
    "rx_pack_convT_weight": (c_int, [c_int, c_void_p, c_int, c_int, c_int, c_void_p, c_void_p, c_void_p]),
    "rx_pack_multi": (c_int, [c_int, c_int, c_void_p, c_void_p, c_void_p, c_void_p, c_void_p, c_void_p, c_void_p, c_void_p]),
    "rx_conv_workspace_hint": (c_size_t, []),
    "rx_conv3d_fwd": (c_int, [c_int, _P, c_void_p, c_void_p, _P, I3, I3, c_void_p, c_size_t, c_void_p]),
    "rx_conv3d_fwd_stats": (c_int, [c_int, _P, c_void_p, c_void_p, _P, I3, I3, c_float, c_void_p, c_void_p, c_size_t, c_void_p]),
    "rx_conv3d_bwd_data": (c_int, [c_int, _P, c_void_p, _P, I3, I3, c_int, c_void_p, c_size_t, c_void_p]),
    "rx_conv3d_bwd_data_instats": (c_int, [c_int, _P, c_void_p, _P, I3, I3, c_int, _P, c_void_p, c_float, c_void_p, POINTER(c_int),
                                           c_void_p, c_size_t, c_void_p]),
    "rx_instnorm_act_bwd_apply": (c_int, [c_int, _P, _P, c_void_p, _P, c_float, c_void_p, _P, _P, c_int, c_void_p]),
    "rx_conv3d_bwd_weight_workspace": (c_size_t, [_P, _P, I3]),
    "rx_conv3d_bwd_weight": (c_int, [c_int, _P, _P, c_void_p, I3, I3, c_void_p, c_size_t, c_void_p]),
    "rx_convT3d_fwd": (c_int, [c_int, _P, c_void_p, c_void_p, _P, I3, c_void_p, c_size_t, c_void_p]),
    "rx_convT3d_bwd_data": (c_int, [c_int, _P, c_void_p, _P, I3, c_int, c_void_p, c_size_t, c_void_p]),
    "rx_convT3d_bwd_weight_workspace": (c_size_t, [_P, _P, I3]),
    "rx_convT3d_bwd_weight": (c_int, [c_int, _P, _P, c_void_p, I3, c_void_p, c_size_t, c_void_p]),
    "rx_instnorm_stats_workspace": (c_size_t, [_P]),
    "rx_instnorm_stats": (c_int, [c_int, _P, c_float, c_void_p, c_void_p, c_size_t, c_void_p]),
    "rx_instnorm_act_fwd": (c_int, [c_int, _P, c_void_p, _P, _P, c_float, c_void_p]),
    "rx_instnorm_stats_mask": (c_int, [c_void_p, c_void_p, c_int, c_void_p]),
    "rx_instnorm_fwd": (c_int, [c_int, _P, c_float, c_void_p, _P, _P, c_float, c_void_p, c_size_t, c_void_p]),
    "rx_instnorm_act_bwd": (c_int, [c_int, _P, _P, c_void_p, _P, c_float, _P, _P, c_int, c_void_p, c_size_t,
                                    c_void_p]),
    "rx_instnorm_act_bwd_res": (c_int, [c_int, _P, _P, c_void_p, _P, c_float, _P, I3, _P, _P, c_void_p, c_size_t, c_void_p]),
    "rx_se_workspace": (c_size_t, [_P]),
    "rx_se_gate_fwd": (c_int, [c_int, _P, c_void_p, c_void_p, _PSE, c_void_p, c_void_p, c_void_p, c_void_p, c_void_p, c_size_t,
                               c_void_p]),
    "rx_instnorm_gate_act_fwd": (c_int, [c_int, _P, c_void_p, c_void_p, c_int, _P, _P, c_float, c_void_p]),
    "rx_se_gate_bwd": (c_int, [c_int, _P, _P, c_void_p, _P, c_float, c_void_p, _PSE, c_void_p, c_void_p, c_void_p, c_void_p,
                               c_void_p, c_void_p, c_void_p, c_void_p, c_void_p, c_void_p, c_void_p, c_size_t, c_void_p]),
    "rx_instnorm_gate_act_bwd": (c_int, [c_int, _P, _P, c_void_p, _P, c_float, c_void_p, c_void_p, c_void_p, c_int, _P, _P,
                                         c_int, c_void_p]),
    "rx_avgpool_fwd": (c_int, [c_int, _P, _P, I3, c_void_p]),
    "rx_instnorm_act_pool_fwd": (c_int, [c_int, _P, c_void_p, _P, _P, _P, I3, c_float, c_void_p]),
    "rx_avgpool_bwd": (c_int, [c_int, _P, _P, I3, c_int, c_void_p]),
    "rx_stem_conv_fwd": (c_int, [c_int, c_void_p, c_int, c_int, c_int, c_int, c_int, c_void_p, c_void_p, _P, I3,
                                 c_void_p]),
    "rx_stem_conv_fwd_stats": (c_int, [c_int, c_void_p, c_int, c_int, c_int, c_int, c_int, c_void_p, c_void_p, _P, I3,
                                       c_float, c_void_p, c_void_p, c_size_t, c_void_p]),
    "rx_stem_conv_bwd_weight_workspace": (c_size_t, [c_int, c_int, c_int]),
    "rx_stem_conv_bwd_weight": (c_int, [c_int, c_void_p, c_int, c_int, c_int, c_int, c_int, _P, c_void_p, I3,
                                        c_void_p, c_size_t, c_void_p]),
    "rx_head_fwd": (c_int, [c_int, _P, c_void_p, c_void_p, c_int, c_void_p, c_int, c_void_p]),
    "rx_head_bwd_workspace": (c_size_t, [_P, c_int]),
    "rx_instnorm_act_head_fwd": (c_int, [c_int, _P, c_void_p, _P, c_float, c_void_p, c_void_p, c_int, c_void_p, c_int, c_void_p]),
    "rx_instnorm_act_bwd_head": (c_int, [c_int, c_void_p, c_int, c_void_p, _P, c_void_p, c_float, _P, c_void_p, c_void_p, c_void_p, c_size_t,
                                         c_void_p]),
    "rx_grad_norm_clip_partials": (ctypes.c_long, [c_int, c_void_p]),
    "rx_grad_norm_clip": (c_int, [c_int, c_void_p, c_void_p, c_float, c_void_p, ctypes.c_long, c_void_p, c_void_p]),
    "rx_head_bwd": (c_int, [c_int, c_void_p, _P, c_void_p, c_int, _P, c_void_p, c_void_p, c_void_p, c_size_t,
                            c_void_p]),
    "rx_channel_sum_workspace": (c_size_t, [_P]),
    "rx_channel_sum": (c_int, [c_int, _P, c_void_p, c_void_p, c_size_t, c_void_p]),
    "rx_loss_workspace": (c_size_t, [c_int, c_int, c_long]),
    "rx_bce_dice_loss_fwd": (c_int, [c_void_p, c_void_p, c_int, c_int, c_long, c_float, c_float, c_float, c_float, c_void_p,
                                     c_void_p, c_void_p, c_size_t, c_void_p]),
    "rx_bce_dice_loss_bwd": (c_int, [c_void_p, c_void_p, c_int, c_int, c_long, c_float, c_float, c_float, c_void_p, c_void_p,
                                     c_void_p, c_void_p]),
    "rx_masked_cosine_loss_fwd": (c_int, [c_void_p, c_void_p, c_int, c_int, c_long, c_void_p, c_void_p, c_void_p, c_size_t,
                                          c_void_p]),
    "rx_masked_cosine_loss_bwd": (c_int, [c_void_p, c_void_p, c_int, c_int, c_long, c_void_p, c_void_p, c_void_p, c_void_p]),
    "rx_elem_loss_fwd": (c_int, [c_int, c_void_p, c_void_p, c_int, c_int, c_long, c_float, c_void_p, c_int, c_int, c_void_p, c_void_p,
                                 c_size_t, c_void_p]),
    "rx_elem_loss_bwd": (c_int, [c_int, c_void_p, c_void_p, c_int, c_int, c_long, c_float, c_void_p, c_int, c_int, c_void_p, c_void_p,
                                 c_void_p]),
    "rx_cross_entropy_loss_workspace": (c_size_t, [c_int, c_int, c_long]),
    "rx_cross_entropy_loss_fwd": (c_int, [c_void_p, c_void_p, c_void_p, ctypes.c_int64, c_int, c_int, c_long, c_int, c_void_p, c_void_p,
                                          c_void_p, c_void_p, c_size_t, c_void_p]),
    "rx_cross_entropy_loss_bwd": (c_int, [c_void_p, c_void_p, c_void_p, ctypes.c_int64, c_int, c_int, c_long, c_void_p, c_void_p,
                                          c_void_p, c_void_p, c_void_p]),
    "rx_adamw_pack": (c_int, [c_int, c_void_p, c_void_p, c_void_p, c_void_p, c_void_p, c_double, c_double, c_double, c_double, c_double,
                              c_int, c_int, c_int, c_int, c_int, c_void_p, c_void_p, c_void_p]),
    "rx_adamw_flat_multi": (c_int, [c_int, c_void_p, c_void_p, c_void_p, c_void_p, c_void_p, c_void_p, c_double, c_double, c_double,
                                    c_double, c_double, c_int, c_void_p]),
    "rx_prog_create": (c_void_p, []),
    "rx_prog_destroy": (None, [c_void_p]),
    "rx_prog_begin": (c_int, [c_void_p, c_void_p, c_int]),
    "rx_prog_end": (c_int, [c_void_p]),
    "rx_prog_len": (c_int, [c_void_p]),
    "rx_prog_cmd_name": (c_char_p, [c_void_p, c_int]),
    "rx_prog_cmd_kernel": (c_char_p, [c_void_p, c_int]),
    "rx_prog_cmd_stream": (c_int, [c_void_p, c_int]),
    "rx_prog_run": (c_int, [c_void_p, c_int, c_int, c_void_p, c_int, c_void_p]),
    "rx_event_new": (c_int, []),
    "rx_event_free": (c_int, [c_int]),
    "rx_event_slots_in_use": (c_int, []),
    "rx_event_record": (c_int, [c_int, c_void_p]),
    "rx_stream_wait": (c_int, [c_int, c_void_p]),
    "rx_adamw_flat": (c_int, [c_void_p, c_void_p, c_void_p, c_void_p, c_void_p, c_double, c_double, c_double, c_double, c_double, c_int,
                              c_long, c_void_p]),
    "rx_sw_gather_workspace": (c_size_t, [c_int, c_int, c_int, c_int, c_int]),
    "rx_sw_gather": (c_int, [c_int, c_void_p, c_int, c_int, c_int, c_int, c_int, c_void_p, c_int, c_int, c_int, c_int, c_void_p,
                             c_void_p, c_size_t, c_void_p]),
    "rx_sw_accumulate": (c_int, [c_void_p, c_int, c_int, c_int, c_int, c_int, c_int, c_void_p, c_int, c_void_p, c_void_p, c_void_p,
                                 c_int, c_int, c_int, c_void_p]),
    "rx_sw_finalize": (c_int, [c_void_p, c_void_p, c_int, c_int, c_int, c_int, c_int, c_int, c_int, c_int, c_int, c_void_p, c_void_p,
                               c_void_p, c_void_p]),
    "rx_aug_workspace": (c_size_t, [c_int, c_int, c_int, c_int, c_int]),
    "rx_aug_pointwise": (c_int, [c_void_p, c_void_p, c_void_p, c_size_t, c_int, c_int, c_int, c_int, c_int, c_void_p, c_void_p, c_long,
                                 c_void_p]),
    "rx_aug_filter_zy": (c_int, [c_void_p, c_void_p, c_int, c_int, c_int, c_int, c_int, c_void_p, c_void_p, c_long, c_void_p]),
    "rx_aug_philox_u32": (c_int, [ctypes.c_uint64, c_long, c_void_p, c_void_p]),
    "rx_geom_apply": (c_int, [c_void_p, c_void_p, c_int, c_int, c_int, c_int, c_int, c_void_p, c_int, c_void_p]),
    "rx_sw_gather_geom": (c_int, [c_int, c_void_p, c_int, c_int, c_int, c_int, c_int, c_void_p, c_void_p, c_int, c_int, c_int, c_int,
                                  c_void_p, c_void_p, c_size_t, c_void_p]),
    "rx_sw_accumulate_geom": (c_int, [c_void_p, c_int, c_int, c_int, c_int, c_int, c_int, c_void_p, c_void_p, c_int, c_int, c_void_p,
                                      c_void_p, c_void_p, c_int, c_int, c_int, c_void_p]),
    "rx_dilate_workspace": (c_size_t, [c_int, c_int, c_int, c_int, c_int]),
    "rx_label_dilate": (c_int, [c_void_p, c_void_p, c_void_p, c_size_t, c_int, c_int, c_int, c_int, c_int, c_int, c_void_p]),
}

_lib = None


def load():
    global _lib
    if _lib is not None:
        return _lib
    if not os.path.exists(LIB_PATH):
        raise RxError(f"{LIB_PATH} not found: build it with `python __graft_entry__.py` "
                      "(hipcc --offload-arch=gfx950); this engine has no PyTorch/CPU fallback")
    lib = ctypes.CDLL(LIB_PATH)
    for name, (res, args) in _SIGNATURES.items():
        fn = getattr(lib, name)
        fn.restype = res
        fn.argtypes = args
    _lib = lib
    return lib


def exported_symbols():
    return sorted(_SIGNATURES)
# ... 24 lines not shown
```

multi-task-3d-resencoder-unet_amd/engine/ops.py:

```python
from ctypes import byref, c_void_p

import numpy as np
import torch

from . import lib as _l
from .lib import I3, RxAct, check, load, stream_ptr

_WS = {}
_PROF = None


def set_profiler(p):
    global _PROF
    _PROF = p


class LaunchProfiler:

    def __init__(self):
        self.pending = []
        self.groups = {}
        self.pending_hbm = []
        self.hbm = {}

# ... 240 lines not shown
    if n == 0:
        return
    VP, IA = ctypes.c_void_p * n, ctypes.c_int * n
    wp = VP(*[w.data_ptr() for w, _, _, _ in items])
    kind = IA(*[k for _, k, _, _ in items])
    A = IA(*[w.shape[0] for w, _, _, _ in items])
    B = IA(*[w.shape[1] for w, _, _, _ in items])
    T = IA(*[w[0, 0].numel() for w, _, _, _ in items])
    fw = VP(*[(f.data_ptr() if f is not None else None) for _, _, f, _ in items])
    bw = VP(*[(b.data_ptr() if b is not None else None) for _, _, _, b in items])
    esz = torch.empty((), dtype=dtype).element_size()
    nbytes = sum(w.numel() * (4 + (esz if f is not None else 0) + (esz if b is not None else 0)) for w, _, f, b in items)
    timed_bytes("pack", nbytes, lambda: check(load().rx_pack_multi(_code(dtype), n, wp, kind, A, B, T, fw, bw, stream_ptr()),
                                             "rx_pack_multi"))


def _taps(kernel):
    return kernel[0] * kernel[1] * kernel[2]


def conv3d_fwd(x, w_fwd, bias, y, kernel, stride, ws=None):
    ws = workspace() if ws is None else ws

    def go():
        check(load().rx_conv3d_fwd(_code(x.dtype), byref(x.desc()), _ptr(w_fwd), _ptr(bias), byref(y.desc()),
                                   I3(*kernel), I3(*stride), *_ws_args(ws), stream_ptr()), "rx_conv3d_fwd")
    if _PROF is None:
        return go()
    n = y.dims[0]
    _PROF.run("fwd:" + LaunchProfiler.igemm_name(y.voxels, y.c), 2.0 * n * y.voxels * y.c * x.c * _taps(kernel), 1, go)


def conv3d_fwd_stats(x, w_fwd, bias, y, kernel, stride, stats, eps=1e-5, ws=None):
    ws = workspace() if ws is None else ws

    def go():
        check(load().rx_conv3d_fwd_stats(_code(x.dtype), byref(x.desc()), _ptr(w_fwd), _ptr(bias), byref(y.desc()),
                                         I3(*kernel), I3(*stride), float(eps), _ptr(stats), *_ws_args(ws), stream_ptr()),
              "rx_conv3d_fwd_stats")
    if _PROF is None:
        return go()
    n = y.dims[0]
    _PROF.run("fwd:" + LaunchProfiler.igemm_name(y.voxels, y.c), 2.0 * n * y.voxels * y.c * x.c * _taps(kernel), 1, go)


def conv3d_bwd_data(dy, w_bwd, dx, kernel, stride, accumulate=False, ws=None):
    ws = workspace() if ws is None else ws

    def go():
        check(load().rx_conv3d_bwd_data(_code(dy.dtype), byref(dy.desc()), _ptr(w_bwd), byref(dx.desc()), I3(*kernel),
                                        I3(*stride), int(accumulate), *_ws_args(ws), stream_ptr()),
              "rx_conv3d_bwd_data")
    if _PROF is None:
        return go()
    n = dy.dims[0]
    _PROF.run("dgrad:" + LaunchProfiler.igemm_name(dx.voxels, dx.c), 2.0 * n * dy.voxels * dy.c * dx.c * _taps(kernel), 1, go)


def conv3d_bwd_data_instats(dy, w_bwd, dx, kernel, stride, accumulate, in_y, in_stats, slope, m12, ws=None):
    from ctypes import c_int
    ws = workspace() if ws is None else ws
    fused = c_int(0)

    def go():
        check(load().rx_conv3d_bwd_data_instats(_code(dy.dtype), byref(dy.desc()), _ptr(w_bwd), byref(dx.desc()), I3(*kernel),
                                                I3(*stride), int(accumulate), byref(in_y.desc()), _ptr(in_stats), float(slope),
                                                _ptr(m12), byref(fused), *_ws_args(ws), stream_ptr()), "rx_conv3d_bwd_data_instats")
    if _PROF is None:
        go()
    else:
        n = dx.dims[0]
        _PROF.run("dgrad:" + LaunchProfiler.igemm_name(dx.voxels, dx.c), 2.0 * n * dx.voxels * dx.c * dy.c * _taps(kernel), 1, go)
    return bool(fused.value)


def instnorm_act_bwd_apply(g, y, stats, out, dy, m12, slope=0.01, d_residual=None, accumulate_residual=False):
    check(load().rx_instnorm_act_bwd_apply(_code(y.dtype), byref(g.desc()), byref(y.desc()), _ptr(stats),
                                           byref(out.desc()) if out is not None else None, float(slope), _ptr(m12),
                                           byref(dy.desc()),
                                           byref(d_residual.desc()) if d_residual is not None else None,
                                           int(accumulate_residual), stream_ptr()), "rx_instnorm_act_bwd_apply")


def conv3d_bwd_weight(x, dy, dw, kernel, stride, ws=None):
    need = load().rx_conv3d_bwd_weight_workspace(byref(x.desc()), byref(dy.desc()), I3(*kernel))
    ws = workspace(need) if ws is None else ws

    def go():
        check(load().rx_conv3d_bwd_weight(_code(x.dtype), byref(x.desc()), byref(dy.desc()), _ptr(dw), I3(*kernel),
                                          I3(*stride), *_ws_args(ws), stream_ptr()), "rx_conv3d_bwd_weight")
    if _PROF is None:
        return go()
    n = dy.dims[0]
    name = f"wgrad:wgrad_kernel<{64 if dy.c % 64 == 0 else 32},{64 if x.c % 64 == 0 else 32}>"
    _PROF.run(name, 2.0 * n * dy.voxels * dy.c * x.c * _taps(kernel), 1, go)


def convT3d_fwd(x, w_fwd, bias, y, stride, ws=None):
    ws = workspace() if ws is None else ws
    check(load().rx_convT3d_fwd(_code(x.dtype), byref(x.desc()), _ptr(w_fwd), _ptr(bias), byref(y.desc()),
                                I3(*stride), *_ws_args(ws), stream_ptr()), "rx_convT3d_fwd")


def convT3d_bwd_data(dy, w_bwd, dx, stride, accumulate=False, ws=None):
    ws = workspace() if ws is None else ws
    check(load().rx_convT3d_bwd_data(_code(dy.dtype), byref(dy.desc()), _ptr(w_bwd), byref(dx.desc()), I3(*stride),
                                     int(accumulate), *_ws_args(ws), stream_ptr()), "rx_convT3d_bwd_data")


def convT3d_bwd_weight(x, dy, dw, stride, ws=None):
    need = load().rx_convT3d_bwd_weight_workspace(byref(x.desc()), byref(dy.desc()), I3(*stride))
    ws = workspace(need) if ws is None else ws
    check(load().rx_convT3d_bwd_weight(_code(x.dtype), byref(x.desc()), byref(dy.desc()), _ptr(dw), I3(*stride),
                                       *_ws_args(ws), stream_ptr()), "rx_convT3d_bwd_weight")


def instnorm_stats(y, stats, eps=1e-5, ws=None):
    ws = workspace() if ws is None else ws
    check(load().rx_instnorm_stats(_code(y.dtype), byref(y.desc()), eps, _ptr(stats), *_ws_args(ws), stream_ptr()),
          "rx_instnorm_stats")


def instnorm_stats_mask(stats, keep):
    check(load().rx_instnorm_stats_mask(_ptr(stats), _ptr(keep), int(keep.numel()), stream_ptr()), "rx_instnorm_stats_mask")


def instnorm_act_fwd(y, stats, out, slope=0.01, residual=None):
    check(load().rx_instnorm_act_fwd(_code(y.dtype), byref(y.desc()), _ptr(stats),
                                     byref(residual.desc()) if residual is not None else None, byref(out.desc()),
                                     float(slope), stream_ptr()), "rx_instnorm_act_fwd")


def instnorm_fwd(y, stats, out, slope=0.01, residual=None, eps=1e-5, ws=None):
    ws = workspace() if ws is None else ws
    check(load().rx_instnorm_fwd(_code(y.dtype), byref(y.desc()), eps, _ptr(stats),
                                 byref(residual.desc()) if residual is not None else None, byref(out.desc()),
                                 float(slope), *_ws_args(ws), stream_ptr()), "rx_instnorm_fwd")


def instnorm_act_bwd(g, y, stats, out, dy, slope=0.01, d_residual=None, accumulate_residual=False, ws=None):
    ws = workspace() if ws is None else ws
    check(load().rx_instnorm_act_bwd(_code(y.dtype), byref(g.desc()), byref(y.desc()), _ptr(stats),
                                     byref(out.desc()) if out is not None else None, float(slope), byref(dy.desc()),
                                     byref(d_residual.desc()) if d_residual is not None else None,
                                     int(accumulate_residual), *_ws_args(ws), stream_ptr()), "rx_instnorm_act_bwd")


def instnorm_act_bwd_res(g, y, stats, out, dy, d_residual, slope=0.01, pool_dy=None, pool_stride=(1, 1, 1), ws=None):
    ws = workspace() if ws is None else ws
    check(load().rx_instnorm_act_bwd_res(_code(y.dtype), byref(g.desc()), byref(y.desc()), _ptr(stats), byref(out.desc()),
                                         float(slope), byref(pool_dy.desc()) if pool_dy is not None else None, I3(*pool_stride),
                                         byref(d_residual.desc()), byref(dy.desc()), *_ws_args(ws), stream_ptr()),
          "rx_instnorm_act_bwd_res")


def _se_params(se):
    if se is None:
        return None
    return byref(_l.RxSeParams(se["w1"].data_ptr(), se["b1"].data_ptr(), se["w2"].data_ptr(), se["b2"].data_ptr(),
                               int(se["rd"]), int(se["keep_x"])))


def se_workspace_bytes(y):
    return load().rx_se_workspace(byref(y.desc()))


def se_gate_fwd(y, stats, se, pooled, hidden, gate, mult, path_scale=None, ws=None):
    ws = workspace(se_workspace_bytes(y)) if ws is None else ws
    check(load().rx_se_gate_fwd(_code(y.dtype), byref(y.desc()), _ptr(stats), _ptr(path_scale), _se_params(se), _ptr(pooled),
                                _ptr(hidden), _ptr(gate), _ptr(mult), *_ws_args(ws), stream_ptr()), "rx_se_gate_fwd")


def instnorm_gate_act_fwd(y, stats, mult, keep_x, out, slope=0.01, residual=None):
    check(load().rx_instnorm_gate_act_fwd(_code(y.dtype), byref(y.desc()), _ptr(stats), _ptr(mult), int(keep_x),
                                          byref(residual.desc()) if residual is not None else None, byref(out.desc()),
                                          float(slope), stream_ptr()), "rx_instnorm_gate_act_fwd")


def se_gate_bwd(g, y, stats, out, slope, se, pooled, hidden, gate, mult, dadd, m12, dw1=None, db1=None, dw2=None, db2=None,
                path_scale=None, ws=None):
    ws = workspace(se_workspace_bytes(y)) if ws is None else ws
    check(load().rx_se_gate_bwd(_code(y.dtype), byref(g.desc()), byref(y.desc()), _ptr(stats),
                                byref(out.desc()) if out is not None else None, float(slope), _ptr(path_scale), _se_params(se),
                                _ptr(pooled), _ptr(hidden), _ptr(gate), _ptr(mult), _ptr(dadd), _ptr(m12), _ptr(dw1), _ptr(db1),
                                _ptr(dw2), _ptr(db2), *_ws_args(ws), stream_ptr()), "rx_se_gate_bwd")


def instnorm_gate_act_bwd(g, y, stats, out, slope, mult, dadd, m12, keep_x, dy, d_residual=None, accumulate_residual=False):
    check(load().rx_instnorm_gate_act_bwd(_code(y.dtype), byref(g.desc()), byref(y.desc()), _ptr(stats),
                                          byref(out.desc()) if out is not None else None, float(slope), _ptr(mult), _ptr(dadd),
                                          _ptr(m12), int(keep_x), byref(dy.desc()),
                                          byref(d_residual.desc()) if d_residual is not None else None,
                                          int(accumulate_residual), stream_ptr()), "rx_instnorm_gate_act_bwd")


def avgpool_fwd(x, y, stride):
    check(load().rx_avgpool_fwd(_code(x.dtype), byref(x.desc()), byref(y.desc()), I3(*stride), stream_ptr()),
# ... 222 lines not shown
    check(load().rx_label_dilate(_ptr(src), _ptr(out), _ptr(scratch), nbytes, b, c, z, y, x, int(radius), stream_ptr()),
          "rx_label_dilate")
    if out is src and src is not tensor:
        tensor.copy_(src)
        return tensor
    return out


def aug_philox_u32(key, n, device):
    out = torch.empty(n, dtype=torch.int32, device=device)
    check(load().rx_aug_philox_u32(int(key), n, _ptr(out), stream_ptr()), "rx_aug_philox_u32")
    return out.to(torch.int64) & 0xFFFFFFFF


def timed_bytes(name, nbytes, fn):
    if _PROF is None:
        return fn()
    return _PROF.run_bytes(name, nbytes, fn)


def _tb(a):
    return 0 if a is None else a.dims[0] * a.voxels * a.c * a.t.element_size()


def _hbm(label, nbytes):
    def deco(f):
        def wrapped(*a, **k):
            if _PROF is None:
                return f(*a, **k)
            return _PROF.run_bytes(label, nbytes(*a, **k), lambda: f(*a, **k))
        wrapped.__name__, wrapped.__doc__ = f.__name__, f.__doc__
        return wrapped
    return deco


def _bwd_bytes(g, y, out, dy, d_residual, acc):
    return _tb(g) + _tb(y) + _tb(dy) + _tb(out) + _tb(d_residual) * (2 if acc else 1)


def _pack_bytes(w, dtype, w_fwd=None, w_bwd=None, want_fwd=True, want_bwd=True):
    e = torch.empty((), dtype=dtype).element_size()
    return w.numel() * (4 + (e if want_fwd else 0) + (e if want_bwd else 0))


instnorm_stats = _hbm("in_stats(colreduce)", lambda y, stats, eps=1e-5, ws=None: _tb(y))(instnorm_stats)
instnorm_act_fwd = _hbm("in_act_fwd", lambda y, stats, out, slope=0.01, residual=None: _tb(y) + _tb(out) + _tb(residual))(instnorm_act_fwd)
instnorm_fwd = _hbm("in_fwd(stats+apply)", lambda y, stats, out, slope=0.01, residual=None, eps=1e-5, ws=None:
                    _tb(y) + _tb(out) + _tb(residual))(instnorm_fwd)
instnorm_act_bwd = _hbm("in_act_bwd(colreduce+apply)",
                        lambda g, y, stats, out, dy, slope=0.01, d_residual=None, accumulate_residual=False, ws=None:
                        _bwd_bytes(g, y, out, dy, d_residual, accumulate_residual))(instnorm_act_bwd)
instnorm_act_bwd_res = _hbm("in_act_bwd_res(colreduce+apply)",
                            lambda g, y, stats, out, dy, d_residual, slope=0.01, pool_dy=None, pool_stride=(1, 1, 1), ws=None:
                            _tb(g) + _tb(y) + _tb(out) + _tb(dy) + _tb(d_residual) + _tb(pool_dy))(instnorm_act_bwd_res)
instnorm_act_bwd_apply = _hbm("in_act_bwd_apply",
                              lambda g, y, stats, out, dy, m12, slope=0.01, d_residual=None, accumulate_residual=False:
                              _bwd_bytes(g, y, out, dy, d_residual, accumulate_residual))(instnorm_act_bwd_apply)
se_gate_fwd = _hbm("se_gate_fwd(linesum+gate)", lambda y, *a, **k: _tb(y))(se_gate_fwd)
instnorm_gate_act_fwd = _hbm("in_gate_act_fwd", lambda y, stats, mult, keep_x, out, slope=0.01, residual=None:
                             _tb(y) + _tb(out) + _tb(residual))(instnorm_gate_act_fwd)
se_gate_bwd = _hbm("se_gate_bwd(linesums+gate)", lambda g, y, stats, out, *a, **k: _tb(g) + _tb(y) + _tb(out))(se_gate_bwd)
instnorm_gate_act_bwd = _hbm("in_gate_act_bwd",
                             lambda g, y, stats, out, slope, mult, dadd, m12, keep_x, dy, d_residual=None, accumulate_residual=False:
                             _bwd_bytes(g, y, out, dy, d_residual, accumulate_residual))(instnorm_gate_act_bwd)
avgpool_fwd = _hbm("avgpool_fwd", lambda x, y, stride: _tb(x) + _tb(y))(avgpool_fwd)
instnorm_act_pool_fwd = _hbm("in_act_pool_fwd", lambda y, stats, out, pooled, stride, slope=0.01, residual=None:
                             _tb(y) + _tb(out) + _tb(pooled) + _tb(residual))(instnorm_act_pool_fwd)
avgpool_bwd = _hbm("avgpool_bwd", lambda dy, dx, stride, accumulate=False: _tb(dy) + _tb(dx) * (2 if accumulate else 1))(avgpool_bwd)
head_fwd = _hbm("head_fwd", lambda x, w, b, out_ncdhw, act=0: _tb(x) + out_ncdhw.numel() * 4)(head_fwd)
head_bwd = _hbm("head_bwd", lambda dout_ncdhw, x, w, dx, dw, db, ws=None: dout_ncdhw.numel() * 4 + _tb(x) + _tb(dx))(head_bwd)
instnorm_act_head_fwd = _hbm("in_act_head_fwd", lambda y, stats, out, w, b, out_ncdhw, act, slope=0.01:
                             _tb(y) + _tb(out) + out_ncdhw.numel() * 4)(instnorm_act_head_fwd)
instnorm_act_bwd_head = _hbm("in_act_bwd_head(colreduce+apply)", lambda dout_ncdhw, w, y, stats, dy, slope=0.01, ws=None, dw=None, db=None:
                             dout_ncdhw.numel() * 4 + _tb(y) + _tb(dy))(instnorm_act_bwd_head)
channel_sum = _hbm("channel_sum", lambda x, out, ws=None: _tb(x))(channel_sum)
pack_conv_weight = _hbm("pack", _pack_bytes)(pack_conv_weight)
pack_convT_weight = _hbm("pack", _pack_bytes)(pack_convT_weight)
stem_conv_fwd = _hbm("stem_conv_fwd", lambda x_ncdhw, w, bias, out, kernel: x_ncdhw.numel() * 4 + _tb(out))(stem_conv_fwd)
stem_conv_fwd_stats = _hbm("stem_conv_fwd", lambda x_ncdhw, w, bias, out, kernel, stats, eps=1e-5, ws=None: x_ncdhw.numel() * 4 + _tb(out))(stem_conv_fwd_stats)
stem_conv_bwd_weight = _hbm("stem_conv_bwd_weight", lambda x_ncdhw, dy, dw, kernel, ws=None: x_ncdhw.numel() * 4 + _tb(dy))(stem_conv_bwd_weight)
convT3d_fwd = _hbm("convT_fwd", lambda x, w_fwd, bias, y, stride, ws=None: _tb(x) + _tb(y))(convT3d_fwd)
convT3d_bwd_data = _hbm("convT_bwd_data", lambda dy, w_bwd, dx, stride, accumulate=False, ws=None:
                        _tb(dy) + _tb(dx) * (2 if accumulate else 1))(convT3d_bwd_data)
convT3d_bwd_weight = _hbm("convT_bwd_weight", lambda x, dy, dw, stride, ws=None: _tb(x) + _tb(dy))(convT3d_bwd_weight)
```

multi-task-3d-resencoder-unet_amd/engine/plan.py:

```python
from dataclasses import dataclass, field
from typing import Callable, Dict, List, Optional

import os

import torch
from torch import nn

from . import lib as _l
from . import ops
from .ops import Act


class UnsupportedConfig(NotImplementedError):
    pass


_SIDE_STREAMS: Dict[str, "torch.cuda.Stream"] = {}


def side_stream(device):
    key = str(device)
    st = _SIDE_STREAMS.get(key)
    if st is None:
        st = _SIDE_STREAMS[key] = torch.cuda.Stream(device=device)
    return st


class _NullCtx:
    def __enter__(self):
        return self

    def __exit__(self, *a):
        return False


@dataclass(eq=False)
class AT:
    act: Act
    name: str
    gact: Optional[Act] = None
    written: bool = False
    needs_grad: bool = True


@dataclass(eq=False)
class Rec:
    kind: str
    a: dict = field(default_factory=dict)


def _slope_of(nonlin):
    if nonlin is None:
        return 1.0
    if isinstance(nonlin, nn.LeakyReLU):
        return float(nonlin.negative_slope)
    if isinstance(nonlin, nn.ReLU):
        return 0.0
    raise UnsupportedConfig(f"nonlinearity {type(nonlin).__name__} has no HIP kernel (LeakyReLU / ReLU only)")


def _check_norm(norm):
    if norm is None:
        raise UnsupportedConfig("conv blocks without a norm layer are never produced by NetworkFromConfig")
    if not isinstance(norm, (nn.InstanceNorm3d, nn.InstanceNorm2d)) or norm.affine or norm.track_running_stats:
        raise UnsupportedConfig("only InstanceNorm(affine=False, track_running_stats=False) has a HIP kernel")
    return float(norm.eps)


class Plan:
    def __init__(self, net, in_shape, dtype, device, needs_grad):
        device = torch.device(device)
        if device.type != "meta":
            _l.require_device()
        self.net = net
        self.dtype = dtype
        self.device = device
        self.needs_grad = needs_grad
        self.in_shape = tuple(in_shape)
        self.generation = 0
        self.two_d = net.op_dims == 2
        B, Cin = in_shape[0], in_shape[1]
        spatial = tuple(in_shape[2:])
        if self.two_d:
            spatial = (1,) + spatial
        self.B, self.Cin, self.spatial = B, Cin, spatial

        self.params: List[nn.Parameter] = []
        self._pidx: Dict[int, int] = {}
        self.packs: List[dict] = []
        self.enc_tape: List[Rec] = []
        self.dec_tapes: List[List[Rec]] = []
        self.fwd: List[Callable] = []
        self.bwd: List[Callable] = []
        self.dy_pool: Dict[tuple, Act] = {}
        self._gbase: Dict[int, torch.Tensor] = {}
        self.outputs: Dict[str, torch.Tensor] = {}
        self.bytes_alloc = 0
        self._x = None
        self._dlogits: Dict[str, torch.Tensor] = {}
        self._grads: List[Optional[torch.Tensor]] = []
        self.grad_order: List[int] = []
        self.grad_sync = None
        import os
        self.overlap_wgrad = os.environ.get("RX_OVERLAP_WGRAD", "1") != "0"
        self.dy_ring = 4
        self._side = None
        self._ws2 = None
        self._dy_turn: Dict[tuple, int] = {}
        self._dy_free: Dict[int, int] = {}
        self._dy_ev: Dict[int, int] = {}
        self._ev_fork = None
        self._ev_join = None
        self._pack_groups = None
        self._gates: List[dict] = []
        self._drops: List[dict] = []
        self._shadows: List[dict] = []
        self._shadow_of: Dict[int, dict] = {}
        self._pad_idx: Dict[int, dict] = {}
        self._pad_done: List[int] = []
        self.use_programs = os.environ.get("RX_PROGRAMS", "1") == "1"
        self._pstate: Dict[tuple, dict] = {}
        self._gflat = None
        self._gviews: Dict[int, torch.Tensor] = {}
        self._marks: List[tuple] = []
        self._recording = None
        self._on_side = False
        self._use_gstore = False
        self._gflat_range = (0, 0)
        self._pack_slots: List[int] = []
        self._unstable_params = False
        self._ws_refs: List[object] = []
        self._raw_seen = None
        self.use_graphs = os.environ.get("RX_GRAPHS", "0") == "1"
        self._gstate: Dict[tuple, dict] = {}
        self._x_static = None
        self._dl_static: Dict[str, torch.Tensor] = {}
        self._image_t = None
        self._pack_delay_at = None
        self._pack_deferred = None
        self._build()

    def release(self):
        try:
            self._pstate.clear()
            slots = set(self._dy_ev.values()) | set(self._pack_slots)
            for s in (self._ev_fork, self._ev_join):
                if s is not None:
                    slots.add(s)
            self._dy_ev, self._pack_slots, self._ev_fork, self._ev_join = {}, [], None, None
            self._dy_free = {}
            for ent in self.packs:
                ent["event"] = None
            for s in slots:
                ops.event_free(s)
        except Exception:
            pass

    def __del__(self):
        self.release()

    def _k3(self, v):
        v = list(v)
        return [1] + v if self.two_d else v

    def _check_extent(self, numel, name):
        per_sample = numel // max(self.B, 1)
        if per_sample * self.dtype.itemsize > (1 << 31):
            raise UnsupportedConfig(f"activation tensor {name} would have {per_sample} elements per sample "
                                    f"({per_sample * self.dtype.itemsize} bytes > 2^31): lower the patch size")

    def _new(self, dims, c, name, ld=None, needs_grad=True):
        self._check_extent(self.B * dims[0] * dims[1] * dims[2] * (ld or c), name)
        t = torch.empty((self.B, *dims, ld or c), dtype=self.dtype, device=self.device)
        self.bytes_alloc += t.numel() * t.element_size()
        return AT(Act(t, 0, c), name, needs_grad=needs_grad)

    def _new_cat(self, dims, c, name, allow_planar=True):
        vox = dims[0] * dims[1] * dims[2]
        min_vox = int(os.environ.get("RX_PLANAR_MIN_VOXELS", str(64 ** 3)))
        planar = (allow_planar and c == 32 and self.dtype != torch.float32 and not self.two_d and dims[2] % 16 == 0 and vox >= min_vox
                  and self.B * (dims[0] // 4) * (dims[1] // 4) * (dims[2] // 16) >= 256
                  and os.environ.get("RX_PLANAR_CAT", "1") != "0")
        if not planar:
            return self._new(dims, 2 * c, name, ld=2 * c)
        self._check_extent(self.B * vox * 32, name)
        root = torch.empty((2, self.B, *dims, 32), dtype=self.dtype, device=self.device)
        self.bytes_alloc += root.numel() * root.element_size()
        return AT(Act.planar(root), name)

    def _param(self, p):
        if id(p) not in self._pidx:
            self._pidx[id(p)] = len(self.params)
            self.params.append(p)
        return self._pidx[id(p)]

    def _pack(self, p, kind):
        if p.dim() != (4 if self.two_d else 5):
            raise UnsupportedConfig("unexpected weight rank")
        a, b = p.shape[0], p.shape[1]
        taps = p[0, 0].numel()
        co, ci = (a, b) if kind == "conv" else (b, a)
        ent = dict(param=p, kind=kind, version=-1,
                   w_fwd=torch.empty((taps, co, ci), dtype=self.dtype, device=self.device),
                   w_bwd=torch.empty((taps, ci, co), dtype=self.dtype, device=self.device) if self.needs_grad else None)
        self.bytes_alloc += 2 * ent["w_fwd"].numel() * ent["w_fwd"].element_size()
        self.packs.append(ent)
        return ent

    def _cp(self, c):
        return (c + 31) // 32 * 32

# ... 573 lines not shown
                                a["head_dw_fused"] = True
                                gw[1]["dw_fused"] = True
                    if (gw[0] == "conv" and a["gate"] is None and res is None and self.dtype != torch.float32
                            and out.act.full_buffer and out.act.root is None and out.act.c % 32 == 0 and out.act.voxels > 512
                            and out.act.dims[3] >= 16):
                        a["m12"] = torch.empty((self.B, out.act.c, 2), dtype=torch.float32, device=self.device)
                        a["m12_valid"] = False
                        gw[1]["inact"] = a
                    def gistep(a=a, gout=gout, dy=dy, gres=gres, acc=acc):
                        g = a["gate"]
                        before_dy_write(dy)
                        if g["se"] is None and g.get("scale_now") is None:
                            ops.instnorm_act_bwd(gout, a["y"].act, a["stats"],
                                                 a["out"].act if (a["slope"] != 1.0 and a["res"] is not None) else None, dy,
                                                 a["slope"], gres, acc)
                            return
                        grads = [new_grad(i) for i in g["se"]["idx"]] if g["se"] is not None else [None] * 4
                        ops.se_gate_bwd(gout, a["y"].act, a["stats"], a["out"].act, a["slope"], P._se_args(g), g["pooled"],
                                        g["hidden"], g["gate"], g["mult"], g["dadd"], g["m12"], *grads,
                                        path_scale=g.get("scale_now"))
                        ops.instnorm_gate_act_bwd(gout, a["y"].act, a["stats"], a["out"].act, a["slope"], g["mult"], g["dadd"],
                                                  g["m12"], g["keep_x"], dy, gres, acc)
                        if g["se"] is not None:
                            for i in g["se"]["idx"]:
                                done(i)
                    if a["gate"] is not None:
                        if a["gate"]["se"] is not None:
                            order += a["gate"]["se"]["idx"]
                        b.append(gistep)
                        continue

                    pend = getattr(out, "_pool_pending", None)
                    out._pool_pending = None
                    fuse_res = gres is not None and not acc and res is not None and y.act.voxels > 512
                    if pend is not None and not fuse_res:
                        b.append(lambda pend=pend: ops.avgpool_bwd(pend["gy"], pend["gx"], pend["stride"], True))
                        pend = None
                    if fuse_res:
                        def rstep(a=a, gout=gout, dy=dy, gres=gres, pend=pend):
                            before_dy_write(dy)
                            ops.instnorm_act_bwd_res(gout, a["y"].act, a["stats"], a["out"].act, dy, gres, a["slope"],
                                                     pool_dy=pend["gy"] if pend is not None else None,
                                                     pool_stride=pend["stride"] if pend is not None else (1, 1, 1))
                        b.append(rstep)
                        continue

                    def istep(a=a, gout=gout, dy=dy, gres=gres, acc=acc):
                        before_dy_write(dy)
                        mask_out = a["out"].act if (a["slope"] != 1.0 and a["res"] is not None) else None
                        hs = a.get("head_src")
                        dl = P._dlogits.get(hs["name"]) if hs is not None else None
                        if dl is not None and a.get("head_dw_fused"):
                            dw, db = new_grad(hs["widx"]), new_grad(hs["bidx"])
                            ops.instnorm_act_bwd_head(dl, hs["w"].view(hs["k"], -1), a["y"].act, a["stats"], dy, a["slope"],
                                                      dw=dw.view(hs["k"], -1), db=db)
                            done(hs["widx"])
                            done(hs["bidx"])
                        elif dl is not None:
                            ops.instnorm_act_bwd_head(dl, hs["w"].view(hs["k"], -1), a["y"].act, a["stats"], dy, a["slope"])
                        elif a.get("m12_valid"):
                            a["m12_valid"] = False
                            ops.instnorm_act_bwd_apply(gout, a["y"].act, a["stats"], mask_out, dy, a["m12"], a["slope"], gres, acc)
                        elif "inbwd_reduce" in skip and a["y"].act.voxels > 512:
                            if "m12x" not in a:
                                a["m12x"] = torch.zeros((self.B, a["y"].act.c, 2), dtype=torch.float32, device=self.device)
                            ops.instnorm_act_bwd_apply(gout, a["y"].act, a["stats"], mask_out, dy, a["m12x"], a["slope"], gres, acc)
                        else:
                            ops.instnorm_act_bwd(gout, a["y"].act, a["stats"], mask_out, dy, a["slope"], gres, acc)
                    b.append(istep)
                elif rec.kind in ("conv", "stem"):
                    y = a["y"]
                    dy = y.gact

                    def wstep(a=a, dy=dy, kind=rec.kind):
                        dw = new_grad(a["widx"])
                        db = new_grad(a["bidx"]) if a["bidx"] is not None else None

                        def launches(ws):
                            if "wgrad" in skip and kind != "stem":
                                pass
                            elif kind == "stem":
                                ops.stem_conv_bwd_weight(P._x, dy, dw, a["kernel"], ws)
                            else:
                                ops.conv3d_bwd_weight(a["x"].act, dy, dw, a["kernel"], a["stride"], ws)
                            done(a["widx"])
                            if db is not None:
                                ops.channel_sum(dy, db, ws)
                                done(a["bidx"])
                        side_run(launches, dy)
                    order += [a["widx"]] + ([a["bidx"]] if a["bidx"] is not None else [])
                    b.append(wstep)
                    if rec.kind == "conv" and a["x"].needs_grad:
                        x = a["x"]
                        gx = self._grad_buf(x)
                        acc = view_written(x)
                        x.written = True
                        if x.act.full_buffer:
                            mark_cat(x)
                        bsinfo = {"inact": None}
                        wrote(x, "conv", bsinfo)

                        def dstep(a=a, dy=dy, gx=gx, acc=acc, bsinfo=bsinfo):
                            if "dgrad" in skip:
                                return
                            ia = bsinfo["inact"]
                            if ia is None:
                                ops.conv3d_bwd_data(dy, a["pk"]["w_bwd"], gx, a["kernel"], a["stride"], acc)
                            else:
                                ia["m12_valid"] = ops.conv3d_bwd_data_instats(dy, a["pk"]["w_bwd"], gx, a["kernel"], a["stride"], acc,
                                                                              ia["y"].act, ia["stats"], ia["slope"], ia["m12"])
                        b.append(dstep)
                elif rec.kind == "convT":
                    x, y = a["x"], a["y"]
                    if not view_written(y):
                        raise RuntimeError("plan bug: concat gradient not initialised before the transposed conv")
                    gy = y.act.like(a["cat"].gact.root if a["cat"].gact.root is not None else a["cat"].gact.t)
                    gx = self._grad_buf(x)
                    acc = view_written(x)
                    x.written = True
                    wrote(x, "convT")

                    def step(a=a, gy=gy, gx=gx, acc=acc):
                        dw = new_grad(a["widx"])
                        db = new_grad(a["bidx"]) if a["bidx"] is not None else None

                        def launches(ws):
                            ops.convT3d_bwd_weight(a["x"].act, gy, dw, a["stride"], ws)
                            done(a["widx"])
                            if db is not None:
                                ops.channel_sum(gy, db, ws)
                                done(a["bidx"])
                        side_run(launches, gy)
                        ops.convT3d_bwd_data(gy, a["pk"]["w_bwd"], gx, a["stride"], acc)
                    order += [a["widx"]] + ([a["bidx"]] if a["bidx"] is not None else [])
                    b.append(step)
                elif rec.kind == "pool":
                    x, y = a["x"], a["y"]
                    if not x.needs_grad:
                        continue
                    gx = self._grad_buf(x)
                    acc = view_written(x)
                    x.written = True
                    wrote(x, "pool")
                    assert y.gact is not None, "plan bug: pooled tensor has no gradient"
                    ti = next(i for i, r in enumerate(tape) if r is rec)
                    prev = tape[ti - 1] if ti > 0 else None
                    if (acc and prev is not None and prev.kind == "inact" and prev.a["out"] is x and prev.a["res"] is not None
                            and prev.a["gate"] is None and x.act.voxels > 512):
                        x._pool_pending = dict(gy=y.gact, gx=gx, stride=a["stride"])
                        continue
                    b.append(lambda a=a, gy=y.gact, gx=gx, acc=acc: ops.avgpool_bwd(gy, gx, a["stride"], acc))
                elif rec.kind == "copy":
                    x, y = a["x"], a["y"]
                    gy = y.act.like(a["cat"].gact.root if a["cat"].gact.root is not None else a["cat"].gact.t)
                    gx = self._grad_buf(x)
                    acc = view_written(x)
                    x.written = True
                    wrote(x, "copy")
                    b.append(lambda gy=gy, gx=gx, acc=acc: ops.avgpool_bwd(gy, gx, (1, 1, 1), acc))

    def _grad_buf(self, at: AT):
        if at.gact is not None:
            return at.gact
        base = at.act.root if at.act.root is not None else at.act.t
        if at.act.key not in self._gbase:
            t = torch.empty_like(base)
            self.bytes_alloc += t.numel() * t.element_size()
            self._gbase[at.act.key] = t
        at.gact = at.act.like(self._gbase[at.act.key])
        return at.gact

    def _ensure_side(self):
        if self.device.type == "cuda" and self.overlap_wgrad and self._side is None:
            self._side = side_stream(self.device)
            self._ws2 = torch.empty(ops.workspace().numel(), dtype=torch.uint8, device=self.device)
        if self._ev_fork is None and self.device.type == "cuda":
            self._ev_fork, self._ev_join = ops.event_new(), ops.event_new()

    def _await_pack(self, ent):
        if ent.get("deferred") and self._pack_deferred is not None:
            self._issue_deferred_packs()
        slot = ent.get("event")
        if slot is not None:
            ops.stream_wait(slot)
            for e in ent["group"]:
                e["event"] = None

    def _packs_stale(self, force=False):
        epoch = getattr(self.net, "_weights_epoch", 0)
        return [e for e in self.packs
                if force or e.get("epoch") != epoch
                or not (e["version"] == e["param"]._version and e.get("ptr") == e["param"].data_ptr())]

    def refresh_packs(self, force=False):
        stale = self._packs_stale(force)
        if not stale:
            return
        side = None
        if self.device.type == "cuda" and self.overlap_wgrad:
            self._ensure_side()
            side = self._side
            ops.event_record(self._ev_fork)
            ops.stream_wait(self._ev_fork, side)
        self._pack_entries(stale, side, defer=True)

    def _issue_deferred_packs(self):
        d, self._pack_deferred = self._pack_deferred, None
        if d is not None:
            groups, side = d
            ops.event_record(self._ev_fork)
# ... 24 lines not shown
    def _pack_groups_now(self, groups, side, gi0):
        ctx = torch.cuda.stream(side) if side is not None else _NullCtx()
        with ctx:
            for gi, grp in enumerate(groups, gi0):
                items = []
                for ent in grp:
                    w = ent["param"].detach()
                    if w.dtype != torch.float32 or not w.is_contiguous():
                        w = w.float().contiguous()
                        self._unstable_params = True
                    if self.two_d:
                        w = w.unsqueeze(2)
                    items.append((w, 0 if ent["kind"] == "conv" else 1, ent["w_fwd"], ent["w_bwd"]))
                ops.pack_weights_multi(items, self.dtype)
                slot = None
                if side is not None:
                    while len(self._pack_slots) <= gi:
                        self._pack_slots.append(ops.event_new())
                    slot = self._pack_slots[gi]
                    ops.event_record(slot)
                for ent in grp:
                    p = ent["param"]
                    ent["deferred"] = False
                    ent["event"], ent["group"] = slot, grp
                    ent["version"], ent["ptr"] = p._version, p.data_ptr()
                    ent["epoch"] = getattr(self.net, "_weights_epoch", 0)

    def repack(self, entries):
        self._pack_entries(entries, self._side)

    def _programs_on(self):
        return (self.use_programs and not self.use_graphs and self.device.type == "cuda" and ops._PROF is None
                and not getattr(self, "_unstable_params", False))

    def _streams(self):
        main = torch.cuda.current_stream()
        return [main] + ([self._side] if self._side is not None else [])

    def _programmed(self, key, body, segments=None):
        st = self._pstate.setdefault(key, {"calls": 0})
        ptrs = self._param_ptrs()
        if st.get("prog") is not None and st["ptrs"] != ptrs:
            st.clear()
            st["calls"] = 0
        if st.get("prog") is not None:
            streams = self._streams()
            if segments is not None:
                segments(st, streams)
            else:
                st["prog"].run(streams)
            return st, True
        if st["calls"] < 2:
            st["calls"] += 1
            st["result"] = body()
            return st, False
        prog = ops.Program()
        self._ws_refs += [ops.workspace(), self._ws2]
        self._marks = []
        self._recording = prog
        self._on_side = False
        prog.begin(self._streams())
        try:
            st["result"] = body()
        finally:
            self._recording = None
            prog.end()
        st["prog"], st["ptrs"], st["marks"] = prog, ptrs, list(self._marks)
        return st, False

    def _grad_store(self):
        if self._gflat is None:
            offs, n = {}, 0
            for idx in self.grad_order:
                if idx not in offs:
                    offs[idx] = n
                    n += (self.params[idx].numel() + 63) // 64 * 64
            self._gflat = torch.empty(max(n, 1), dtype=torch.float32, device=self.device)
            self.bytes_alloc += self._gflat.numel() * 4
            lo, hi = self._gflat.data_ptr(), self._gflat.data_ptr() + self._gflat.numel() * 4
            self._gflat_range = (lo, hi)
            for idx, o in offs.items():
                p = self.params[idx]
                self._gviews[idx] = self._gflat[o:o + p.numel()].view(p.shape)
        lo, hi = self._gflat_range
        for p in self.params:
            gr = p.grad
            if gr is not None and lo <= gr.data_ptr() < hi:
                p.grad = gr.clone()

    def _graphs_on(self):
        return (self.use_graphs and self.device.type == "cuda" and self.needs_grad
                and self.grad_sync is None and ops._PROF is None and not self._drops)

    def _param_ptrs(self):
        return tuple(p.data_ptr() for p in self.params)

    def _graphed(self, key, body):
        st = self._gstate.setdefault(key, {"calls": 0})
        ptrs = self._param_ptrs()
        if st.get("graph") is not None and st["ptrs"] != ptrs:
            st.clear()
            st["calls"] = 0
        if st.get("graph") is not None:
            st["graph"].replay()
        elif st["calls"] < 2:
            st["calls"] += 1
            st["result"] = body()
            st["eager"] = True
            return st
        else:
            torch.cuda.synchronize(self.device)
            g = torch.cuda.CUDAGraph()
            with torch.cuda.graph(g):
                st["result"] = body()
            st["graph"], st["ptrs"] = g, ptrs
            g.replay()
        st["eager"] = False
        return st

    def _forward_pre(self):
        ev = getattr(self.net, "_raw_param_event", None)
        if ev is not None and ev is not self._raw_seen:
            torch.cuda.current_stream().wait_event(ev)
            self._raw_seen = ev
        for g in self._gates:
            g["scale_now"] = self._draw_path_scale(g)
        if self._shadows:
            self._refresh_shadows()
        training = bool(self.net.training)
        for d in self._drops:
            d["active"] = training
            d["eps_now"] = d["eps"] * (1.0 - d["p"]) ** 2 if training else d["eps"]
            if training:
                self._draw_dropout(d)

    def _forward_body(self, force_packs):
        self.refresh_packs(force=force_packs)
        for i, step in enumerate(self.fwd):
            if i == self._pack_delay_at:
                self._issue_deferred_packs()
            step()
        self._issue_deferred_packs()
        for ent in self.packs:
            self._await_pack(ent)

    def _mark_packs_fresh(self):
        epoch = getattr(self.net, "_weights_epoch", 0)
        for ent in self.packs:
            ent["version"], ent["ptr"], ent["event"] = ent["param"]._version, ent["param"].data_ptr(), None
            ent["epoch"] = epoch

    def run_forward(self, x, apply_act):
        if tuple(x.shape) != self.in_shape:
            raise ValueError(f"plan built for input {self.in_shape}, got {tuple(x.shape)}")
        x = x.detach()
        if x.dtype != torch.float32 or not x.is_contiguous():
            x = x.float().contiguous()
        self._apply_act = apply_act
        self._forward_pre()
        if self._graphs_on():
            if self._x_static is None:
                self._x_static = torch.empty(self.in_shape, dtype=torch.float32, device=self.device)
            self._x_static.copy_(x)
            self._x = self._x_static.unsqueeze(2) if self.two_d else self._x_static
            self._fill_image_t()
            st = self._gstate.get(("f", apply_act))
            capturing = st is not None and st.get("graph") is None and st["calls"] >= 2
            self._graphed(("f", apply_act), lambda: self._forward_body(force_packs=capturing))
            st = self._gstate[("f", apply_act)]
            if not st["eager"]:
                self._mark_packs_fresh()
# ... 64 lines not shown
            want = (self.B, c, *at.act.dims[1:4])
            if tuple(t.shape) != want:
                raise ValueError(f"encoder output of shape {tuple(t.shape)} where the plan holds {want}")
            act = at.act
            act.t[..., act.c0:act.c0 + c].copy_(t.permute(0, 2, 3, 4, 1))
            if act.c > c:
                act.t[..., act.c0 + c:act.c0 + act.c].zero_()
        a = self.fwd_dec_start[d]
        b = self.fwd_dec_start[d + 1] if d + 1 < len(self.fwd_dec_start) else len(self.fwd)
        for step in self.fwd[a:b]:
            step()
        self.generation += 1
        v = self.outputs[name]
        return (v.squeeze(2) if self.two_d else v).clone()

    def _backward_body(self):
        self._dy_free.clear()
        for step in self.bwd:
            step()
        if self._side is not None:
            ops.event_record(self._ev_join, self._side)
            ops.stream_wait(self._ev_join)

    def _backward_finish(self):
        grads = self._grads
        if self._pad_idx:
            sync = self.grad_sync
            for idx in sorted(set(self._pad_done)):
                ent = self._pad_idx[idx]
                q = ent["param"]
                if sync is not None:
                    real = sync.alloc(idx)
                elif self._use_gstore:
                    real = self._gviews[idx]
                else:
                    real = torch.empty_like(q, memory_format=torch.contiguous_format)
                for dst, sidx in ent["pairs"]:
                    real[sidx].copy_(ent["gpad"][dst])
                grads[idx] = real
                if sync is not None:
                    sync.ready(idx)
            self._pad_done = []
        if self.grad_sync is not None:
            self.grad_sync.finish()
            if not self.grad_sync.returns_grads:
                grads = [None] * len(self.params)
        self._grads = []
        return grads

    def _replay_backward_segments(self, st, streams):
        prog, sync, pos = st["prog"], self.grad_sync, 0
        for cmd, idx, on_side in st["marks"]:
            if cmd > pos:
                prog.run(streams, pos, cmd)
                pos = cmd
            self._grads[idx] = sync.alloc(idx)
            if on_side and self._side is not None:
                with torch.cuda.stream(self._side):
                    sync.ready(idx)
            else:
                sync.ready(idx)
        prog.run(streams, pos, -1)

    def run_backward(self, dlogits: Dict[str, Optional[torch.Tensor]]):
        graphs = self._graphs_on()
        programs = (not graphs) and self._programs_on() and all(dlogits.get(k) is not None for k in self.outputs)
        self._dlogits = {}
        for k, g in dlogits.items():
            if g is None:
                continue
            g = g.detach()
            if g.dtype != torch.float32 or not g.is_contiguous():
                g = g.float().contiguous()
            if graphs or programs:
                buf = self._dl_static.get(k)
                if buf is None or buf.shape != g.shape:
                    buf = self._dl_static[k] = torch.empty_like(g)
                buf.copy_(g)
                g = buf
            self._dlogits[k] = g.unsqueeze(2) if self.two_d else g
        self._ensure_side()
        self.net._weights_epoch = getattr(self.net, "_weights_epoch", 0) + 1
        self._grads = [None] * len(self.params)
        if programs:
            sync = self.grad_sync
            self._use_gstore = sync is None
            if sync is None:
                self._grad_store()
            else:
                sync.persistent = True
                sync.begin(self)
            key = ("b", tuple(sorted(self._dlogits)), id(sync) if sync is not None else 0, self.overlap_wgrad)
            st, replayed = self._programmed(key, self._backward_body,
                                            segments=self._replay_backward_segments if sync is not None else None)
            if replayed:
                self._pad_done = [idx for idx in set(self.grad_order) if idx in self._pad_idx]
            if replayed and sync is None:
                for idx in set(self.grad_order):
                    self._grads[idx] = self._gviews[idx]
            grads = self._backward_finish()
            return [t.detach() if t is not None else None for t in grads]
        self._use_gstore = False
        if self.grad_sync is not None:
            self.grad_sync.persistent = False
            self.grad_sync.begin(self)
        if not graphs:
            self._backward_body()
            return self._backward_finish()
        key = ("b", tuple(sorted(self._dlogits)))
        st = self._gstate.get(key)
        if st is not None and st.get("graph") is not None:
            owned = st["owned"]
            for p in self.params:
                gr = p.grad
                if gr is not None and gr.data_ptr() in owned:
                    p.grad = gr.clone()

        def body():
            self._backward_body()
            return self._backward_finish()
        st = self._graphed(key, body)
        grads = st["result"]
        if st["eager"]:
            return grads
        if "owned" not in st:
            st["owned"] = {t.data_ptr() for t in grads if t is not None}
        return [t.detach() if t is not None else None for t in grads]
```

multi-task-3d-resencoder-unet_amd/training/optim/engine_adamw.py:

```python
import ctypes
from ctypes import c_void_p

import torch

from ...engine import lib as _l
from ...engine.lib import check, load, stream_ptr


def _p(t):
    return c_void_p(t.data_ptr()) if t is not None else c_void_p(0)


class EngineAdamW(torch.optim.Optimizer):
    def __init__(self, params, model=None, lr=1e-3, betas=(0.9, 0.999), eps=1e-8, weight_decay=1e-2):
        defaults = dict(lr=lr, betas=betas, eps=eps, weight_decay=weight_decay)
        super().__init__(params, defaults)
        self.model = model
        self._clip = None
        self._norm_ws = None

    @torch.no_grad()
    def clip_grad_norm(self, max_norm, norm_type=2.0):
        grads = [p.grad for g in self.param_groups for p in g["params"] if p.grad is not None]
        if not grads:
            return torch.zeros(())
        if (float(norm_type) == 2.0
                and all(g.is_cuda and g.dtype == torch.float32 and g.is_contiguous() for g in grads)):
            n = len(grads)
            VP, LP = ctypes.c_void_p * n, ctypes.c_long * n
            numel = LP(*[g.numel() for g in grads])
            need = load().rx_grad_norm_clip_partials(n, numel)
            if self._norm_ws is None or self._norm_ws.numel() < need or self._norm_ws.device != grads[0].device:
                self._norm_ws = torch.empty(int(need), dtype=torch.float32, device=grads[0].device)
            out = torch.empty(2, dtype=torch.float32, device=grads[0].device)
            from ...engine import ops as _ops
            _ops.timed_bytes("grad_norm_clip", 4 * sum(g.numel() for g in grads), lambda: check(
                load().rx_grad_norm_clip(n, VP(*[g.data_ptr() for g in grads]), numel, float(max_norm), _p(self._norm_ws),
                                         self._norm_ws.numel(), _p(out), stream_ptr()), "rx_grad_norm_clip"))
            self._clip = out[1:2]
            return out[0]
        norms = torch._foreach_norm(grads, norm_type)
        total = torch.linalg.vector_norm(torch.stack(norms), norm_type)
        self._clip = torch.clamp(max_norm / (total + 1e-6), max=1.0).to(torch.float32).reshape(1)
        return total

    def _plan(self):
        plans = [p for p in getattr(self.model, "_plans", {}).values() if p.needs_grad and p.device.type == "cuda"] \
            if self.model is not None else []
        return plans[0] if len(plans) == 1 and not plans[0]._shadows else None

    @torch.no_grad()
    def step(self, closure=None):
        loss = None
        if closure is not None:
            with torch.enable_grad():
                loss = closure()
        plan = self._plan()
        packed = {id(e["param"]): e for e in plan.packs} if plan is not None else {}
        if plan is not None and plan._side is not None:
            torch.cuda.current_stream().wait_stream(plan._side)
        lib = load()
        clip = self._clip
        self._clip = None
        for group in self.param_groups:
            b1, b2 = group["betas"]
            flat = []
            for p in group["params"]:
                if p.grad is None:
                    continue
                if not p.is_cuda or p.dtype != torch.float32 or not p.is_contiguous():
                    raise _l.RxError("EngineAdamW updates contiguous fp32 parameters on the HIP device only")
                g = p.grad if p.grad.is_contiguous() else p.grad.contiguous()
                st = self.state[p]
                if not st:
                    st["step"] = 0
                    st["exp_avg"] = torch.zeros_like(p, memory_format=torch.contiguous_format)
                    st["exp_avg_sq"] = torch.zeros_like(p, memory_format=torch.contiguous_format)
                st["step"] = int(st["step"]) + 1
                ent = packed.get(id(p))
                if ent is not None:
                    kind = 0 if ent["kind"] == "conv" else 1
                    A, B = p.shape[0], p.shape[1]
                    taps = p[0, 0].numel()
                    check(lib.rx_adamw_pack(_l.DTYPE_CODE[plan.dtype], _p(p), _p(g), _p(st["exp_avg"]), _p(st["exp_avg_sq"]), _p(clip),
                                            group["lr"], b1, b2, group["eps"], group["weight_decay"], st["step"], kind, A, B, taps,
                                            _p(ent["w_fwd"]), _p(ent["w_bwd"]), stream_ptr()), "rx_adamw_pack")
                    ent["version"], ent["ptr"], ent["event"] = p._version, p.data_ptr(), None
                    ent["epoch"] = getattr(plan.net, "_weights_epoch", 0)
                else:
                    flat.append((p, g, st))
            self._flat_update(group, flat, clip)
        return loss

    def _flat_update(self, group, items, clip):
        b1, b2 = group["betas"]
        by_step = {}
        for p, g, st in items:
            by_step.setdefault(st["step"], []).append((p, g, st))
        for step_no, its in by_step.items():
            n = len(its)
            VP, LP = ctypes.c_void_p * n, ctypes.c_long * n
            from ...engine import ops as _ops
            _ops.timed_bytes("adamw", 28 * sum(p.numel() for p, _, _ in its), lambda: check(
                load().rx_adamw_flat_multi(n, VP(*[p.data_ptr() for p, _, _ in its]), VP(*[g.data_ptr() for _, g, _ in its]),
                                           VP(*[st["exp_avg"].data_ptr() for _, _, st in its]),
                                           VP(*[st["exp_avg_sq"].data_ptr() for _, _, st in its]),
                                           LP(*[p.numel() for p, _, _ in its]), _p(clip), group["lr"], b1, b2, group["eps"],
                                           group["weight_decay"], step_no, stream_ptr()), "rx_adamw_flat_multi"))

    def take_clip(self):
        clip, self._clip = self._clip, None
        return clip

    @torch.no_grad()
    def update_subset(self, params, clip):
        group_of = {id(p): g for g in self.param_groups for p in g["params"]}
        per_group = {}
        for p in params:
            if p.grad is None:
                continue
            if not p.is_cuda or p.dtype != torch.float32 or not p.is_contiguous():
# ... 13 lines not shown
```

Before: 118.1 patches/s.

## Fuse grad sum-of-squares into wgrad reduce and reuse partials for clipping

The weight-gradient reduce kernels now have variants that also write per-block sum-of-squares partials while storing dw. The plan keeps a partials buffer per conv weight and stamps it with the gradient store version. The clip step then sums these small partials instead of re-reading the full conv gradients, scanning only the tensors that have no valid span. This removes a full read of most gradient memory in grad-norm clipping, at the cost of extra reductions and syncs in the wgrad reduce, extra bookkeeping, and version checks that may silently fall back to the full scan.

```diff
diff --git a/include/rxunet.h b/include/rxunet.h
--- a/include/rxunet.h
+++ b/include/rxunet.h
@@ -51,6 +51,10 @@
 size_t rx_conv3d_bwd_weight_workspace(const rx_act* x, const rx_act* dy, const int32_t kernel[3]);
 int rx_conv3d_bwd_weight(rx_dtype dt, const rx_act* x, const rx_act* dy, float* dw, const int32_t kernel[3],
                          const int32_t stride[3], void* ws, size_t ws_bytes, void* stream);
+long rx_conv3d_bwd_weight_sq_partials(rx_dtype dt, const rx_act* x, const rx_act* dy, const int32_t kernel[3],
+                                      const int32_t stride[3], void* ws, size_t ws_bytes);
+int rx_conv3d_bwd_weight_sq(rx_dtype dt, const rx_act* x, const rx_act* dy, float* dw, const int32_t kernel[3],
+                            const int32_t stride[3], void* ws, size_t ws_bytes, float* sq_partial, long sq_len, void* stream);
 
 int rx_convT3d_fwd(rx_dtype dt, const rx_act* x, const void* w_fwd, const float* bias, const rx_act* y,
                    const int32_t stride[3], void* ws, size_t ws_bytes, void* stream);
@@ -59,6 +63,10 @@
 size_t rx_convT3d_bwd_weight_workspace(const rx_act* x, const rx_act* dy, const int32_t stride[3]);
 int rx_convT3d_bwd_weight(rx_dtype dt, const rx_act* x, const rx_act* dy, float* dw, const int32_t stride[3],
                           void* ws, size_t ws_bytes, void* stream);
+long rx_convT3d_bwd_weight_sq_partials(rx_dtype dt, const rx_act* x, const rx_act* dy, const int32_t stride[3], void* ws,
+                                       size_t ws_bytes);
+int rx_convT3d_bwd_weight_sq(rx_dtype dt, const rx_act* x, const rx_act* dy, float* dw, const int32_t stride[3],
+                             void* ws, size_t ws_bytes, float* sq_partial, long sq_len, void* stream);
 
 size_t rx_instnorm_stats_workspace(const rx_act* y);
 int rx_instnorm_stats(rx_dtype dt, const rx_act* y, float eps, float* stats, void* ws, size_t ws_bytes,
@@ -167,6 +175,9 @@
 long rx_grad_norm_clip_partials(int count, const long* numel);
 int rx_grad_norm_clip(int count, const float* const* grad, const long* numel, float max_norm, float* partial, long partial_len,
                       float* out, void* stream);
+int rx_grad_norm_clip_spans(int count, const float* const* grad, const long* numel, int nspans, const float* const* span,
+                            const long* span_len, float max_norm, float* partial, long partial_len, double* span_sums, float* out,
+                            void* stream);
 int rx_adamw_flat_multi(int count, float* const* p, const float* const* grad, float* const* exp_avg,
                         float* const* exp_avg_sq, const long* numel, const float* clip, double lr, double beta1,
                         double beta2, double eps, double weight_decay, int step, void* stream);
diff --git a/multi-task-3d-resencoder-unet_amd/csrc/rx_internal.h b/multi-task-3d-resencoder-unet_amd/csrc/rx_internal.h
--- a/multi-task-3d-resencoder-unet_amd/csrc/rx_internal.h
+++ b/multi-task-3d-resencoder-unet_amd/csrc/rx_internal.h
@@ -9,10 +9,18 @@
                      int accumulate, hipStream_t st);
 int rx_dgrad_s2_halo_try(rx_dtype dt, const rx_act* dy, const void* w_bwd, const rx_act* dx, int accumulate, hipStream_t st);
 
+struct RxSqOut {
+  float* ptr;
+  long cap;
+  long n;
+  bool dry;
+};
+
 size_t rx_wgrad_halo_ws_bytes(const rx_act* x, const rx_act* dy);
 int rx_wgrad_halo_try(rx_dtype dt, const rx_act* x, const rx_act* dy, const int32_t stride[3], float* dw, void* ws, size_t ws_bytes,
-                      hipStream_t st);
-void rx_wgrad_reduce_launch(const float* slab, int S, int T_, int R, int C, float* dw, hipStream_t st);
+                      hipStream_t st, RxSqOut* sq);
+long rx_wgrad_reduce_sq_partials(int S, int T_, int R, int C);
+int rx_wgrad_reduce_launch(const float* slab, int S, int T_, int R, int C, float* dw, hipStream_t st, RxSqOut* sq);
 
 int rx_stem_fwd_mfma_try(rx_dtype dt, const float* x, int n, int cin, int z, int y, int xx, const float* w, const float* bias,
                          const rx_act* out, const int32_t kernel[3], hipStream_t st, float* stat_part, size_t stat_bytes, int* stat_chunks);
diff --git a/multi-task-3d-resencoder-unet_amd/csrc/rx_pack_optim.hip b/multi-task-3d-resencoder-unet_amd/csrc/rx_pack_optim.hip
--- a/multi-task-3d-resencoder-unet_amd/csrc/rx_pack_optim.hip
+++ b/multi-task-3d-resencoder-unet_amd/csrc/rx_pack_optim.hip
@@ -486,7 +486,8 @@
 }
 
 __global__ __launch_bounds__(1024) void sqnorm_finalize_kernel(const float* __restrict__ partial, int nblocks, float max_norm,
-                                                               float* __restrict__ out ) {
+                                                               float* __restrict__ out ,
+                                                               const double* __restrict__ span_sums, int nspans) {
   __shared__ double red[1024];
   double s[8] = {0.0, 0.0, 0.0, 0.0, 0.0, 0.0, 0.0, 0.0};
   int i = threadIdx.x;
@@ -505,7 +506,9 @@
     __syncthreads();
   }
   if (threadIdx.x == 0) {
-    const float norm = (float)sqrt(red[0]);
+    double total = red[0];
+    for (int k = 0; k < nspans; ++k) total += span_sums[k];
+    const float norm = (float)sqrt(total);
     const float coef = max_norm / (norm + 1e-6f);
     out[0] = norm;
     out[1] = coef < 1.f ? coef : 1.f;
@@ -518,9 +521,57 @@
   return blocks;
 }
 
+#define RX_SPAN_MAX 128
+struct SqSpans {
+  const float* p[RX_SPAN_MAX];
+  int n[RX_SPAN_MAX];
+};
+
+__global__ __launch_bounds__(1024) void sqnorm_spans_kernel(const SqSpans t, double* __restrict__ span_sums) {
+  __shared__ double red[16];
+  const float* __restrict__ p = t.p[blockIdx.x];
+  const int n = t.n[blockIdx.x];
+  double s0 = 0.0, s1 = 0.0, s2 = 0.0, s3 = 0.0;
+  int i = threadIdx.x;
+  for (; i + 3 * 1024 < n; i += 4 * 1024) {
+    const float v0 = p[i], v1 = p[i + 1024], v2 = p[i + 2048], v3 = p[i + 3072];
+    s0 += (double)v0, s1 += (double)v1, s2 += (double)v2, s3 += (double)v3;
+  }
+  for (; i < n; i += 1024) s0 += (double)p[i];
+  double s = wave_sum_d((s0 + s1) + (s2 + s3));
+  if ((threadIdx.x & 63) == 0) red[threadIdx.x >> 6] = s;
+  __syncthreads();
+  if (threadIdx.x == 0) {
+    s = 0.0;
+    for (int w = 0; w < 16; ++w) s += red[w];
+    span_sums[blockIdx.x] = s;
+  }
+}
+
+static int grad_norm_clip_impl(int count, const float* const* grad, const long* numel, int nspans, const float* const* span,
+                               const long* span_len, float max_norm, float* partial, long partial_len, double* span_sums, float* out,
+                               void* stream);
+
 extern "C" int rx_grad_norm_clip(int count, const float* const* grad, const long* numel, float max_norm, float* partial, long partial_len,
                                  float* out, void* stream) {
   if (count < 1 || !grad || !numel || !partial || !out) RX_FAIL(RX_EINVAL, "rx_grad_norm_clip: bad arguments");
+  return grad_norm_clip_impl(count, grad, numel, 0, nullptr, nullptr, max_norm, partial, partial_len, nullptr, out, stream);
+}
+
+extern "C" int rx_grad_norm_clip_spans(int count, const float* const* grad, const long* numel, int nspans, const float* const* span,
+                                       const long* span_len, float max_norm, float* partial, long partial_len, double* span_sums,
+                                       float* out, void* stream) {
+  if (count < 0 || nspans < 0 || count + nspans < 1 || !out || (count > 0 && (!grad || !numel || !partial)) ||
+      (nspans > 0 && (!span || !span_len || !span_sums)))
+    RX_FAIL(RX_EINVAL, "rx_grad_norm_clip_spans: bad arguments");
+  for (int i = 0; i < nspans; ++i)
+    if (!span[i] || span_len[i] < 1 || span_len[i] > 0x3fffffffL) RX_FAIL(RX_EINVAL, "rx_grad_norm_clip_spans: bad span %d", i);
+  return grad_norm_clip_impl(count, grad, numel, nspans, span, span_len, max_norm, partial, partial_len, span_sums, out, stream);
+}
+
+static int grad_norm_clip_impl(int count, const float* const* grad, const long* numel, int nspans, const float* const* span,
+                               const long* span_len, float max_norm, float* partial, long partial_len, double* span_sums, float* out,
+                               void* stream) {
   const long need = rx_grad_norm_clip_partials(count, numel);
   if (need > partial_len || need > 0x3fffffffL) RX_FAIL(RX_EWORKSPACE, "rx_grad_norm_clip: %ld partials needed, %ld given", need, partial_len);
   long done = 0;
@@ -541,7 +592,14 @@
     done += blocks;
     i0 += k;
   }
-  hipLaunchKernelGGL(sqnorm_finalize_kernel, dim3(1), dim3(1024), 0, (hipStream_t)stream, (const float*)partial, (int)done, max_norm, out);
+  for (int i0 = 0; i0 < nspans; i0 += RX_SPAN_MAX) {
+    SqSpans t;
+    const int k = nspans - i0 < RX_SPAN_MAX ? nspans - i0 : RX_SPAN_MAX;
+    for (int j = 0; j < RX_SPAN_MAX; ++j) t.p[j] = j < k ? span[i0 + j] : nullptr, t.n[j] = j < k ? (int)span_len[i0 + j] : 0;
+    hipLaunchKernelGGL(sqnorm_spans_kernel, dim3((unsigned)k), dim3(1024), 0, (hipStream_t)stream, t, span_sums + i0);
+  }
+  hipLaunchKernelGGL(sqnorm_finalize_kernel, dim3(1), dim3(1024), 0, (hipStream_t)stream, (const float*)partial, (int)done, max_norm, out,
+                     (const double*)span_sums, nspans);
   RX_CHECK_LAUNCH("rx_grad_norm_clip");
   return RX_OK;
 }
diff --git a/multi-task-3d-resencoder-unet_amd/csrc/rx_wgrad.hip b/multi-task-3d-resencoder-unet_amd/csrc/rx_wgrad.hip
--- a/multi-task-3d-resencoder-unet_amd/csrc/rx_wgrad.hip
+++ b/multi-task-3d-resencoder-unet_amd/csrc/rx_wgrad.hip
@@ -156,7 +156,17 @@
   }
 }
 
-__global__ __launch_bounds__(256) void wgrad_reduce(const float* __restrict__ slab, int S, int T_, int R, int C, float* __restrict__ dw) {
+__device__ __forceinline__ void wg256_sq_store(float sq, float* __restrict__ sq_partial, long index) {
+  __shared__ float sq_red[4];
+  sq = wave_sum(sq);
+  if ((threadIdx.x & 63) == 0) sq_red[threadIdx.x >> 6] = sq;
+  __syncthreads();
+  if (threadIdx.x == 0) sq_partial[index] = (sq_red[0] + sq_red[1]) + (sq_red[2] + sq_red[3]);
+}
+
+template <bool SQ>
+__device__ __forceinline__ void wgrad_reduce_body(const float* __restrict__ slab, int S, int T_, int R, int C, float* __restrict__ dw,
+                                                  float* __restrict__ sq_partial) {
   __shared__ float tile[27 * 257];
   const long RC = (long)R * C;
   const long base = (long)blockIdx.x * 256;
@@ -169,34 +179,58 @@
   }
   __syncthreads();
   const long n_here = (RC - base < 256 ? RC - base : 256) * T_;
+  float sq = 0.f;
   for (long j = threadIdx.x; j < n_here; j += 256) {
     int pair = (int)(j / T_), t = (int)(j - (long)pair * T_);
-    dw[base * T_ + j] = tile[t * 257 + pair];
-  }
-}
-
-__global__ __launch_bounds__(256) void wgrad_reduce_manysplits(const float* __restrict__ slab, int S, int T_, int R, int C,
-                                                               float* __restrict__ dw) {
+    const float v = tile[t * 257 + pair];
+    dw[base * T_ + j] = v;
+    if constexpr (SQ) sq += v * v;
+  }
+  if constexpr (SQ) wg256_sq_store(sq, sq_partial, blockIdx.x);
+}
+__global__ __launch_bounds__(256) void wgrad_reduce(const float* __restrict__ slab, int S, int T_, int R, int C, float* __restrict__ dw) {
+  wgrad_reduce_body<false>(slab, S, T_, R, C, dw, nullptr);
+}
+__global__ __launch_bounds__(256) void wgrad_reduce_sq(const float* __restrict__ slab, int S, int T_, int R, int C, float* __restrict__ dw,
+                                                       float* __restrict__ sq_partial) {
+  wgrad_reduce_body<true>(slab, S, T_, R, C, dw, sq_partial);
+}
+
+template <bool SQ>
+__device__ __forceinline__ void wgrad_reduce_manysplits_body(const float* __restrict__ slab, int S, int T_, int R, int C,
+                                                             float* __restrict__ dw, float* __restrict__ sq_partial) {
   const long RC = (long)R * C;
   const long i = (long)blockIdx.x * 256 + threadIdx.x;
   const int t = blockIdx.y;
-  if (i >= RC) return;
-  const float* p = slab + (long)t * RC + i;
-  const long stride = (long)T_ * RC;
-  float a0 = 0.f, a1 = 0.f, a2 = 0.f, a3 = 0.f, a4 = 0.f, a5 = 0.f, a6 = 0.f, a7 = 0.f;
-  int k = 0;
-  for (; k + 8 <= S; k += 8) {
-    a0 += p[(k + 0) * stride];
-    a1 += p[(k + 1) * stride];
-    a2 += p[(k + 2) * stride];
-    a3 += p[(k + 3) * stride];
-    a4 += p[(k + 4) * stride];
-    a5 += p[(k + 5) * stride];
-    a6 += p[(k + 6) * stride];
-    a7 += p[(k + 7) * stride];
-  }
-  for (; k < S; ++k) a0 += p[k * stride];
-  dw[i * T_ + t] = ((a0 + a1) + (a2 + a3)) + ((a4 + a5) + (a6 + a7));
+  float v = 0.f;
+  if (i < RC) {
+    const float* p = slab + (long)t * RC + i;
+    const long stride = (long)T_ * RC;
+    float a0 = 0.f, a1 = 0.f, a2 = 0.f, a3 = 0.f, a4 = 0.f, a5 = 0.f, a6 = 0.f, a7 = 0.f;
+    int k = 0;
+    for (; k + 8 <= S; k += 8) {
+      a0 += p[(k + 0) * stride];
+      a1 += p[(k + 1) * stride];
+      a2 += p[(k + 2) * stride];
+      a3 += p[(k + 3) * stride];
+      a4 += p[(k + 4) * stride];
+      a5 += p[(k + 5) * stride];
+      a6 += p[(k + 6) * stride];
+      a7 += p[(k + 7) * stride];
+    }
+    for (; k < S; ++k) a0 += p[k * stride];
+    v = ((a0 + a1) + (a2 + a3)) + ((a4 + a5) + (a6 + a7));
+    dw[i * T_ + t] = v;
+  }
+  if constexpr (SQ) wg256_sq_store(v * v, sq_partial, (long)blockIdx.y * gridDim.x + blockIdx.x);
+}
+__global__ __launch_bounds__(256) void wgrad_reduce_manysplits(const float* __restrict__ slab, int S, int T_, int R, int C,
+                                                               float* __restrict__ dw) {
+  wgrad_reduce_manysplits_body<false>(slab, S, T_, R, C, dw, nullptr);
+}
+__global__ __launch_bounds__(256) void wgrad_reduce_manysplits_sq(const float* __restrict__ slab, int S, int T_, int R, int C,
+                                                                  float* __restrict__ dw, float* __restrict__ sq_partial) {
+  wgrad_reduce_manysplits_body<true>(slab, S, T_, R, C, dw, sq_partial);
 }
 
 static int plan_split(const WgradGeom& g, int BR, int BC, size_t ws_bytes, int* ksplit, int* qps) {
@@ -250,7 +284,8 @@
 #undef RX_WG
 }
 
-static int wgrad_launch(rx_dtype dt, const void* gt, const void* xt, float* dw, WgradGeom& g, void* ws, size_t ws_bytes, hipStream_t st) {
+static int wgrad_launch(rx_dtype dt, const void* gt, const void* xt, float* dw, WgradGeom& g, void* ws, size_t ws_bytes, hipStream_t st,
+                        RxSqOut* sq) {
   const int per16 = dt == RX_F32 ? 4 : 8;
   if (g.R % 32 || g.Cc % 32) RX_FAIL(RX_EUNSUPPORTED, "wgrad: channel counts must be multiples of 32 (R=%d C=%d)", g.R, g.Cc);
   if (g.ldg % per16 || g.ldx % per16 || ((uintptr_t)gt & 15) || ((uintptr_t)xt & 15)) RX_FAIL(RX_EUNSUPPORTED, "wgrad: misaligned operand");
@@ -259,22 +294,46 @@
   g.tiles_c = g.Cc / BC;
   int rc = plan_split(g, BR, BC, ws_bytes, &g.ksplit, &g.q_per_split);
   if (rc) RX_FAIL(rc, "wgrad: workspace too small (%zu bytes)", ws_bytes);
+  if (sq && sq->dry) {
+    sq->n = rx_wgrad_reduce_sq_partials(g.ksplit, g.ntaps, g.R, g.Cc);
+    return RX_OK;
+  }
   dim3 grid((g.R / BR) * (g.Cc / BC), g.ntaps, g.ksplit);
   rx_note_kernel(BR == 64 ? (BC == 64 ? "wgrad_kernel<64,64>" : "wgrad_kernel<64,32>") : (BC == 64 ? "wgrad_kernel<32,64>" : "wgrad_kernel<32,32>"));
   RX_DISPATCH_DTYPE(dt, T, wgrad_dispatch<T>(BR, BC, grid, st, gt, xt, (float*)ws, g));
-  rx_wgrad_reduce_launch((const float*)ws, g.ksplit, g.ntaps, g.R, g.Cc, dw, st);
+  rc = rx_wgrad_reduce_launch((const float*)ws, g.ksplit, g.ntaps, g.R, g.Cc, dw, st, sq);
+  if (rc) return rc;
   RX_CHECK_LAUNCH("wgrad");
   return RX_OK;
 }
 
 static int conv_out_dim(int in, int k, int s) { return (in + 2 * ((k - 1) / 2) - k) / s + 1; }
 
-void rx_wgrad_reduce_launch(const float* slab, int S, int T_, int R, int C, float* dw, hipStream_t st) {
+static bool reduce_manysplits(int S, int T_) { return S >= 8 || T_ > 27; }
+
+long rx_wgrad_reduce_sq_partials(int S, int T_, int R, int C) {
+  const long groups = ((long)R * C + 255) / 256;
+  return reduce_manysplits(S, T_) ? groups * T_ : groups;
+}
+
+int rx_wgrad_reduce_launch(const float* slab, int S, int T_, int R, int C, float* dw, hipStream_t st, RxSqOut* sq) {
   long RC = (long)R * C;
-  if (S >= 8 || T_ > 27)
-    hipLaunchKernelGGL(wgrad_reduce_manysplits, dim3((unsigned)((RC + 255) / 256), T_), dim3(256), 0, st, slab, S, T_, R, C, dw);
+  const dim3 grid = reduce_manysplits(S, T_) ? dim3((unsigned)((RC + 255) / 256), T_) : dim3((unsigned)((RC + 255) / 256));
+  if (sq && sq->ptr) {
+    const long need = rx_wgrad_reduce_sq_partials(S, T_, R, C);
+    if (need > sq->cap) RX_FAIL(RX_EWORKSPACE, "wgrad reduce: %ld sum-of-squares partials needed, room for %ld", need, sq->cap);
+    sq->n = need;
+    if (reduce_manysplits(S, T_))
+      hipLaunchKernelGGL(wgrad_reduce_manysplits_sq, grid, dim3(256), 0, st, slab, S, T_, R, C, dw, sq->ptr);
+    else
+      hipLaunchKernelGGL(wgrad_reduce_sq, grid, dim3(256), 0, st, slab, S, T_, R, C, dw, sq->ptr);
+    return RX_OK;
+  }
+  if (reduce_manysplits(S, T_))
+    hipLaunchKernelGGL(wgrad_reduce_manysplits, grid, dim3(256), 0, st, slab, S, T_, R, C, dw);
   else
-    hipLaunchKernelGGL(wgrad_reduce, dim3((unsigned)((RC + 255) / 256)), dim3(256), 0, st, slab, S, T_, R, C, dw);
+    hipLaunchKernelGGL(wgrad_reduce, grid, dim3(256), 0, st, slab, S, T_, R, C, dw);
+  return RX_OK;
 }
 
 extern "C" size_t rx_conv3d_bwd_weight_workspace(const rx_act* x, const rx_act* dy, const int32_t kernel[3]) {
@@ -284,9 +343,8 @@
   return a > b ? a : b;
 }
 
-extern "C" int rx_conv3d_bwd_weight(rx_dtype dt, const rx_act* x, const rx_act* dy, float* dw, const int32_t kernel[3],
-                                    const int32_t stride[3], void* ws, size_t ws_bytes, void* stream) {
-  RX_RECORD(stream, [=, x_ = RxActV(x), dy_ = RxActV(dy), kernel_ = RxI3V(kernel), stride_ = RxI3V(stride)](void* s) { return rx_conv3d_bwd_weight(dt, x_.p(), dy_.p(), dw, kernel_.v, stride_.v, ws, ws_bytes, s); });
+static int conv3d_bwd_weight_impl(rx_dtype dt, const rx_act* x, const rx_act* dy, float* dw, const int32_t kernel[3],
+                                  const int32_t stride[3], void* ws, size_t ws_bytes, void* stream, RxSqOut* sq) {
   if (!rx_act_ok_planar(x) || !rx_act_ok(dy)) RX_FAIL(RX_EINVAL, "rx_conv3d_bwd_weight: bad arguments");
   for (int i = 0; i < 3; ++i) {
     if (kernel[i] < 1 || kernel[i] > RX_MAX_KERNEL) RX_FAIL(RX_EUNSUPPORTED, "rx_conv3d_bwd_weight: kernel sizes must be 1..%d per axis", RX_MAX_KERNEL);
@@ -296,7 +354,7 @@
       dy->x != conv_out_dim(x->x, kernel[2], stride[2]))
     RX_FAIL(RX_EINVAL, "rx_conv3d_bwd_weight: geometry mismatch");
   if (kernel[0] == 3 && kernel[1] == 3 && kernel[2] == 3 && ws && dw) {
-    int rc = rx_wgrad_halo_try(dt, x, dy, stride, dw, ws, ws_bytes, (hipStream_t)stream);
+    int rc = rx_wgrad_halo_try(dt, x, dy, stride, dw, ws, ws_bytes, (hipStream_t)stream, sq);
     if (rc < 0) return rc;
     if (rc == 1) return RX_OK;
   }
@@ -316,7 +374,29 @@
         t.w = (uint16_t)g.ntaps;
         ++g.ntaps;
       }
-  return wgrad_launch(dt, dy->ptr, x->ptr, dw, g, ws, ws_bytes, (hipStream_t)stream);
+  return wgrad_launch(dt, dy->ptr, x->ptr, dw, g, ws, ws_bytes, (hipStream_t)stream, sq);
+}
+
+extern "C" int rx_conv3d_bwd_weight(rx_dtype dt, const rx_act* x, const rx_act* dy, float* dw, const int32_t kernel[3],
+                                    const int32_t stride[3], void* ws, size_t ws_bytes, void* stream) {
+  RX_RECORD(stream, [=, x_ = RxActV(x), dy_ = RxActV(dy), kernel_ = RxI3V(kernel), stride_ = RxI3V(stride)](void* s) { return rx_conv3d_bwd_weight(dt, x_.p(), dy_.p(), dw, kernel_.v, stride_.v, ws, ws_bytes, s); });
+  return conv3d_bwd_weight_impl(dt, x, dy, dw, kernel, stride, ws, ws_bytes, stream, nullptr);
+}
+
+extern "C" int rx_conv3d_bwd_weight_sq(rx_dtype dt, const rx_act* x, const rx_act* dy, float* dw, const int32_t kernel[3],
+                                       const int32_t stride[3], void* ws, size_t ws_bytes, float* sq_partial, long sq_len, void* stream) {
+  RX_RECORD(stream, [=, x_ = RxActV(x), dy_ = RxActV(dy), kernel_ = RxI3V(kernel), stride_ = RxI3V(stride)](void* s) { return rx_conv3d_bwd_weight_sq(dt, x_.p(), dy_.p(), dw, kernel_.v, stride_.v, ws, ws_bytes, sq_partial, sq_len, s); });
+  if (!sq_partial || sq_len < 0) RX_FAIL(RX_EINVAL, "rx_conv3d_bwd_weight_sq: bad arguments");
+  RxSqOut sq = {sq_partial, sq_len, 0, false};
+  return conv3d_bwd_weight_impl(dt, x, dy, dw, kernel, stride, ws, ws_bytes, stream, &sq);
+}
+
+extern "C" long rx_conv3d_bwd_weight_sq_partials(rx_dtype dt, const rx_act* x, const rx_act* dy, const int32_t kernel[3],
+                                                 const int32_t stride[3], void* ws, size_t ws_bytes) {
+  float dummy;
+  RxSqOut sq = {nullptr, 0, 0, true};
+  const int rc = conv3d_bwd_weight_impl(dt, x, dy, &dummy, kernel, stride, ws, ws_bytes, nullptr, &sq);
+  return rc == RX_OK ? sq.n : 0;
 }
 
 struct ConvTWgGeom {
@@ -452,7 +532,7 @@
 }
 
 static int convT_wgrad_try(rx_dtype dt, const rx_act* x, const rx_act* dy, const int32_t stride[3], float* dw, void* ws, size_t ws_bytes,
-                           hipStream_t st) {
+                           hipStream_t st, RxSqOut* sq) {
   const int taps = stride[0] * stride[1] * stride[2];
   const int R = x->c, C = dy->c;
   if (dt == RX_F32 || taps > 8 || R % 32 || C % 32 || x->ld % 8 || dy->ld % 8 || ((uintptr_t)x->ptr & 15) || ((uintptr_t)dy->ptr & 15)) return 0;
@@ -472,6 +552,10 @@
   g.q_per_split = (int)(((ktiles + S - 1) / S) * 64);
   const int S2 = (int)((NQ + g.q_per_split - 1) / g.q_per_split);
   const size_t lds = (size_t)64 * (R + taps * C) * 2;
+  if (sq && sq->dry) {
+    sq->n = rx_wgrad_reduce_sq_partials(S2, taps, R, C);
+    return 1;
+  }
   rx_note_kernel("convT_wgrad_kernel");
 #define RX_CTW(NR_, NC_)                                                                                                              \
   do {                                                                                                                                \
@@ -492,8 +576,8 @@
   }
 #undef RX_CTW_ALL
 #undef RX_CTW
-  rx_wgrad_reduce_launch((const float*)ws, S2, taps, R, C, dw, st);
-  return 1;
+  const int rc = rx_wgrad_reduce_launch((const float*)ws, S2, taps, R, C, dw, st, sq);
+  return rc ? rc : 1;
 }
 
 extern "C" size_t rx_convT3d_bwd_weight_workspace(const rx_act* x, const rx_act* dy, const int32_t stride[3]) {
@@ -506,18 +590,18 @@
   return a > b ? a : b;
 }
 
-extern "C" int rx_convT3d_bwd_weight(rx_dtype dt, const rx_act* x, const rx_act* dy, float* dw, const int32_t stride[3], void* ws,
-                                     size_t ws_bytes, void* stream) {
-  RX_RECORD(stream, [=, x_ = RxActV(x), dy_ = RxActV(dy), stride_ = RxI3V(stride)](void* s) { return rx_convT3d_bwd_weight(dt, x_.p(), dy_.p(), dw, stride_.v, ws, ws_bytes, s); });
+static int convT3d_bwd_weight_impl(rx_dtype dt, const rx_act* x, const rx_act* dy, float* dw, const int32_t stride[3], void* ws,
+                                   size_t ws_bytes, void* stream, RxSqOut* sq) {
   if (!rx_act_ok(x) || !rx_act_ok(dy)) RX_FAIL(RX_EINVAL, "rx_convT3d_bwd_weight: bad arguments");
   for (int i = 0; i < 3; ++i)
     if (stride[i] < 1 || stride[i] > RX_MAX_STRIDE) RX_FAIL(RX_EUNSUPPORTED, "rx_convT3d_bwd_weight: strides must be 1..%d per axis", RX_MAX_STRIDE);
   if (dy->n != x->n || dy->z != x->z * stride[0] || dy->y != x->y * stride[1] || dy->x != x->x * stride[2])
     RX_FAIL(RX_EINVAL, "rx_convT3d_bwd_weight: geometry mismatch");
   if (ws && dw) {
-    const int rc = convT_wgrad_try(dt, x, dy, stride, dw, ws, ws_bytes, (hipStream_t)stream);
+    const int rc = convT_wgrad_try(dt, x, dy, stride, dw, ws, ws_bytes, (hipStream_t)stream, sq);
     if (rc < 0) return rc;
     if (rc == 1) {
+      if (sq && sq->dry) return RX_OK;
       RX_CHECK_LAUNCH("rx_convT3d_bwd_weight(convT_wgrad)");
       return RX_OK;
     }
@@ -536,5 +620,27 @@
         t.w = (uint16_t)g.ntaps;
         ++g.ntaps;
       }
-  return wgrad_launch(dt, x->ptr, dy->ptr, dw, g, ws, ws_bytes, (hipStream_t)stream);
-}
+  return wgrad_launch(dt, x->ptr, dy->ptr, dw, g, ws, ws_bytes, (hipStream_t)stream, sq);
+}
+
+extern "C" int rx_convT3d_bwd_weight(rx_dtype dt, const rx_act* x, const rx_act* dy, float* dw, const int32_t stride[3], void* ws,
+                                     size_t ws_bytes, void* stream) {
+  RX_RECORD(stream, [=, x_ = RxActV(x), dy_ = RxActV(dy), stride_ = RxI3V(stride)](void* s) { return rx_convT3d_bwd_weight(dt, x_.p(), dy_.p(), dw, stride_.v, ws, ws_bytes, s); });
+  return convT3d_bwd_weight_impl(dt, x, dy, dw, stride, ws, ws_bytes, stream, nullptr);
+}
+
+extern "C" int rx_convT3d_bwd_weight_sq(rx_dtype dt, const rx_act* x, const rx_act* dy, float* dw, const int32_t stride[3], void* ws,
+                                        size_t ws_bytes, float* sq_partial, long sq_len, void* stream) {
+  RX_RECORD(stream, [=, x_ = RxActV(x), dy_ = RxActV(dy), stride_ = RxI3V(stride)](void* s) { return rx_convT3d_bwd_weight_sq(dt, x_.p(), dy_.p(), dw, stride_.v, ws, ws_bytes, sq_partial, sq_len, s); });
+  if (!sq_partial || sq_len < 0) RX_FAIL(RX_EINVAL, "rx_convT3d_bwd_weight_sq: bad arguments");
+  RxSqOut sq = {sq_partial, sq_len, 0, false};
+  return convT3d_bwd_weight_impl(dt, x, dy, dw, stride, ws, ws_bytes, stream, &sq);
+}
+
+extern "C" long rx_convT3d_bwd_weight_sq_partials(rx_dtype dt, const rx_act* x, const rx_act* dy, const int32_t stride[3], void* ws,
+                                                  size_t ws_bytes) {
+  float dummy;
+  RxSqOut sq = {nullptr, 0, 0, true};
+  const int rc = convT3d_bwd_weight_impl(dt, x, dy, &dummy, stride, ws, ws_bytes, nullptr, &sq);
+  return rc == RX_OK ? sq.n : 0;
+}
diff --git a/multi-task-3d-resencoder-unet_amd/csrc/rx_wgrad_halo.hip b/multi-task-3d-resencoder-unet_amd/csrc/rx_wgrad_halo.hip
--- a/multi-task-3d-resencoder-unet_amd/csrc/rx_wgrad_halo.hip
+++ b/multi-task-3d-resencoder-unet_amd/csrc/rx_wgrad_halo.hip
@@ -18,7 +18,21 @@
   int Zi, Yi, Xi;
   int order;
   int dbg;
+  float* sq;
 };
+
+template <int NW>
+__device__ __forceinline__ void wgh_sq_store(float sq, float* red, float* __restrict__ out) {
+  sq = wave_sum(sq);
+  if ((threadIdx.x & 63) == 0) red[threadIdx.x >> 6] = sq;
+  __syncthreads();
+  if (threadIdx.x == 0) {
+    float s = 0.f;
+#pragma unroll
+    for (int w = 0; w < NW; w += 2) s += red[w] + red[w + 1];
+    *out = s;
+  }
+}
 
 typedef __attribute__((address_space(3))) s16x4 lds_s16x4_h;
 
@@ -157,6 +171,7 @@
   const int col = lane & 31, fh = lane >> 5;
   if (g.S == 1) {
     float* sT = reinterpret_cast<float*>(smem);
+    float sq = 0.f;
 #pragma unroll
     for (int hb = 0; hb < 2; ++hb) {
       __syncthreads();
@@ -174,9 +189,12 @@
       __syncthreads();
       for (int idx = tid; idx < 16 * 216; idx += 256) {
         const int lr = idx / 216, i = idx - lr * 216;
-        *reinterpret_cast<f32x4*>(dw + ((long)(r0 + 16 * hb + lr) * g.Cc + c0) * 27 + 4 * i) = *reinterpret_cast<const f32x4*>(sT + 4 * idx);
-      }
-    }
+        const f32x4 v = *reinterpret_cast<const f32x4*>(sT + 4 * idx);
+        *reinterpret_cast<f32x4*>(dw + ((long)(r0 + 16 * hb + lr) * g.Cc + c0) * 27 + 4 * i) = v;
+        sq += (v[0] * v[0] + v[1] * v[1]) + (v[2] * v[2] + v[3] * v[3]);
+      }
+    }
+    if (g.sq) wgh_sq_store<4>(sq, sT + 16 * 32 * 27, g.sq + blockIdx.x);
     return;
   }
 #pragma unroll
@@ -385,6 +403,7 @@
   const int col = lane & 31, fh = lane >> 5;
   if (g.S == 1) {
     float* sT = reinterpret_cast<float*>(smem);
+    float sq = 0.f;
 #pragma unroll
     for (int hb = 0; hb < 2; ++hb) {
       __syncthreads();
@@ -404,9 +423,12 @@
       __syncthreads();
       for (int idx = tid; idx < 16 * 216; idx += 512) {
         const int lr = idx / 216, i = idx - lr * 216;
-        *reinterpret_cast<f32x4*>(dw + ((long)(r0 + 16 * hb + lr) * g.Cc + c0) * 27 + 4 * i) = *reinterpret_cast<const f32x4*>(sT + 4 * idx);
-      }
-    }
+        const f32x4 v = *reinterpret_cast<const f32x4*>(sT + 4 * idx);
+        *reinterpret_cast<f32x4*>(dw + ((long)(r0 + 16 * hb + lr) * g.Cc + c0) * 27 + 4 * i) = v;
+        sq += (v[0] * v[0] + v[1] * v[1]) + (v[2] * v[2] + v[3] * v[3]);
+      }
+    }
+    if (g.sq) wgh_sq_store<8>(sq, sT + 16 * 32 * 27, g.sq + blockIdx.x);
     return;
   }
   if (wave < 4) {
@@ -487,13 +509,22 @@
 }
 
 int rx_wgrad_halo_try(rx_dtype dt, const rx_act* x, const rx_act* dy, const int32_t stride[3], float* dw, void* ws, size_t ws_bytes,
-                      hipStream_t st) {
+                      hipStream_t st, RxSqOut* sq) {
   if (dt == RX_F32) return 0;
   if (x->c % 32 || dy->c % 32 || x->ld % 8 || dy->ld % 8 || ((uintptr_t)x->ptr & 15) || ((uintptr_t)dy->ptr & 15)) return 0;
   WgHaloGeom g;
   if (!wgh_plan(x, dy, stride, &g, ws_bytes)) return 0;
   const size_t lds = (size_t)(RX_WGH_MAX_VT + RX_WGH_MAX_HV) * 64;
   dim3 grid((g.R / 32) * g.panels_c, g.S);
+  if (sq) {
+    const long need = g.S == 1 ? (long)grid.x : rx_wgrad_reduce_sq_partials(g.S, 27, g.R, g.Cc);
+    if (sq->dry) {
+      sq->n = need;
+      return 1;
+    }
+    if (need > sq->cap) RX_FAIL(RX_EWORKSPACE, "wgrad_halo: %ld sum-of-squares partials needed, room for %ld", need, sq->cap);
+    if (g.S == 1) g.sq = sq->ptr, sq->n = need;
+  }
   static const int dbg = rx_env_mask("RX_DBG");
   g.dbg = dbg;
   g.order = 1;
@@ -514,7 +545,7 @@
       hipLaunchKernelGGL((wgrad_halo16ws_kernel<bf16_t, false>), grid, dim3(512), 2 * lds16, st, (const bf16_t*)dy->ptr, (const bf16_t*)x->ptr, (float*)ws, dw, g);
     else
       hipLaunchKernelGGL((wgrad_halo16ws_kernel<f16_t, false>), grid, dim3(512), 2 * lds16, st, (const f16_t*)dy->ptr, (const f16_t*)x->ptr, (float*)ws, dw, g);
-    if (g.S > 1) rx_wgrad_reduce_launch((const float*)ws, g.S, 27, g.R, g.Cc, dw, st);
+    if (g.S > 1 && rx_wgrad_reduce_launch((const float*)ws, g.S, 27, g.R, g.Cc, dw, st, sq)) return RX_EWORKSPACE;
     hipError_t e16 = hipGetLastError();
     if (e16 != hipSuccess) {
       rx_set_error("wgrad_halo16: %s", hipGetErrorString(e16));
@@ -530,7 +561,7 @@
     (void)hipFuncSetAttribute(reinterpret_cast<const void*>(&wgrad_halo_kernel<f16_t>), hipFuncAttributeMaxDynamicSharedMemorySize, (int)lds);
     hipLaunchKernelGGL((wgrad_halo_kernel<f16_t>), grid, dim3(256), lds, st, (const f16_t*)dy->ptr, (const f16_t*)x->ptr, (float*)ws, dw, g);
   }
-  if (g.S > 1) rx_wgrad_reduce_launch((const float*)ws, g.S, 27, g.R, g.Cc, dw, st);
+  if (g.S > 1 && rx_wgrad_reduce_launch((const float*)ws, g.S, 27, g.R, g.Cc, dw, st, sq)) return RX_EWORKSPACE;
   hipError_t e = hipGetLastError();
   if (e != hipSuccess) {
     rx_set_error("wgrad_halo: %s", hipGetErrorString(e));
diff --git a/multi-task-3d-resencoder-unet_amd/engine/lib.py b/multi-task-3d-resencoder-unet_amd/engine/lib.py
--- a/multi-task-3d-resencoder-unet_amd/engine/lib.py
+++ b/multi-task-3d-resencoder-unet_amd/engine/lib.py
@@ -56,10 +56,14 @@
     "rx_instnorm_act_bwd_apply": (c_int, [c_int, _P, _P, c_void_p, _P, c_float, c_void_p, _P, _P, c_int, c_void_p]),
     "rx_conv3d_bwd_weight_workspace": (c_size_t, [_P, _P, I3]),
     "rx_conv3d_bwd_weight": (c_int, [c_int, _P, _P, c_void_p, I3, I3, c_void_p, c_size_t, c_void_p]),
+    "rx_conv3d_bwd_weight_sq_partials": (ctypes.c_long, [c_int, _P, _P, I3, I3, c_void_p, c_size_t]),
+    "rx_conv3d_bwd_weight_sq": (c_int, [c_int, _P, _P, c_void_p, I3, I3, c_void_p, c_size_t, c_void_p, ctypes.c_long, c_void_p]),
     "rx_convT3d_fwd": (c_int, [c_int, _P, c_void_p, c_void_p, _P, I3, c_void_p, c_size_t, c_void_p]),
     "rx_convT3d_bwd_data": (c_int, [c_int, _P, c_void_p, _P, I3, c_int, c_void_p, c_size_t, c_void_p]),
     "rx_convT3d_bwd_weight_workspace": (c_size_t, [_P, _P, I3]),
     "rx_convT3d_bwd_weight": (c_int, [c_int, _P, _P, c_void_p, I3, c_void_p, c_size_t, c_void_p]),
+    "rx_convT3d_bwd_weight_sq_partials": (ctypes.c_long, [c_int, _P, _P, I3, c_void_p, c_size_t]),
+    "rx_convT3d_bwd_weight_sq": (c_int, [c_int, _P, _P, c_void_p, I3, c_void_p, c_size_t, c_void_p, ctypes.c_long, c_void_p]),
     "rx_instnorm_stats_workspace": (c_size_t, [_P]),
     "rx_instnorm_stats": (c_int, [c_int, _P, c_float, c_void_p, c_void_p, c_size_t, c_void_p]),
     "rx_instnorm_act_fwd": (c_int, [c_int, _P, c_void_p, _P, _P, c_float, c_void_p]),
@@ -93,6 +97,8 @@
                                          c_void_p]),
     "rx_grad_norm_clip_partials": (ctypes.c_long, [c_int, c_void_p]),
     "rx_grad_norm_clip": (c_int, [c_int, c_void_p, c_void_p, c_float, c_void_p, ctypes.c_long, c_void_p, c_void_p]),
+    "rx_grad_norm_clip_spans": (c_int, [c_int, c_void_p, c_void_p, c_int, c_void_p, c_void_p, c_float, c_void_p, ctypes.c_long,
+                                        c_void_p, c_void_p, c_void_p]),
     "rx_head_bwd": (c_int, [c_int, c_void_p, _P, c_void_p, c_int, _P, c_void_p, c_void_p, c_void_p, c_size_t,
                             c_void_p]),
     "rx_channel_sum_workspace": (c_size_t, [_P]),
diff --git a/multi-task-3d-resencoder-unet_amd/engine/ops.py b/multi-task-3d-resencoder-unet_amd/engine/ops.py
--- a/multi-task-3d-resencoder-unet_amd/engine/ops.py
+++ b/multi-task-3d-resencoder-unet_amd/engine/ops.py
@@ -346,18 +346,29 @@
                                            int(accumulate_residual), stream_ptr()), "rx_instnorm_act_bwd_apply")
 
 
-def conv3d_bwd_weight(x, dy, dw, kernel, stride, ws=None):
+def conv3d_bwd_weight(x, dy, dw, kernel, stride, ws=None, sq=None):
     need = load().rx_conv3d_bwd_weight_workspace(byref(x.desc()), byref(dy.desc()), I3(*kernel))
     ws = workspace(need) if ws is None else ws
+    n_sq = 0
+    if sq is not None:
+        n_sq = int(load().rx_conv3d_bwd_weight_sq_partials(_code(x.dtype), byref(x.desc()), byref(dy.desc()), I3(*kernel),
+                                                           I3(*stride), *_ws_args(ws)))
 
     def go():
-        check(load().rx_conv3d_bwd_weight(_code(x.dtype), byref(x.desc()), byref(dy.desc()), _ptr(dw), I3(*kernel),
-                                          I3(*stride), *_ws_args(ws), stream_ptr()), "rx_conv3d_bwd_weight")
+        if n_sq > 0:
+            check(load().rx_conv3d_bwd_weight_sq(_code(x.dtype), byref(x.desc()), byref(dy.desc()), _ptr(dw), I3(*kernel),
+                                                 I3(*stride), *_ws_args(ws), _ptr(sq), sq.numel(), stream_ptr()),
+                  "rx_conv3d_bwd_weight_sq")
+        else:
+            check(load().rx_conv3d_bwd_weight(_code(x.dtype), byref(x.desc()), byref(dy.desc()), _ptr(dw), I3(*kernel),
+                                              I3(*stride), *_ws_args(ws), stream_ptr()), "rx_conv3d_bwd_weight")
     if _PROF is None:
-        return go()
+        go()
+        return n_sq
     n = dy.dims[0]
     name = f"wgrad:wgrad_kernel<{64 if dy.c % 64 == 0 else 32},{64 if x.c % 64 == 0 else 32}>"
     _PROF.run(name, 2.0 * n * dy.voxels * dy.c * x.c * _taps(kernel), 1, go)
+    return n_sq
 
 
 def convT3d_fwd(x, w_fwd, bias, y, stride, ws=None):
@@ -372,11 +383,20 @@
                                      int(accumulate), *_ws_args(ws), stream_ptr()), "rx_convT3d_bwd_data")
 
 
-def convT3d_bwd_weight(x, dy, dw, stride, ws=None):
+def convT3d_bwd_weight(x, dy, dw, stride, ws=None, sq=None):
     need = load().rx_convT3d_bwd_weight_workspace(byref(x.desc()), byref(dy.desc()), I3(*stride))
     ws = workspace(need) if ws is None else ws
-    check(load().rx_convT3d_bwd_weight(_code(x.dtype), byref(x.desc()), byref(dy.desc()), _ptr(dw), I3(*stride),
-                                       *_ws_args(ws), stream_ptr()), "rx_convT3d_bwd_weight")
+    n_sq = 0
+    if sq is not None:
+        n_sq = int(load().rx_convT3d_bwd_weight_sq_partials(_code(x.dtype), byref(x.desc()), byref(dy.desc()), I3(*stride),
+                                                            *_ws_args(ws)))
+    if n_sq > 0:
+        check(load().rx_convT3d_bwd_weight_sq(_code(x.dtype), byref(x.desc()), byref(dy.desc()), _ptr(dw), I3(*stride),
+                                              *_ws_args(ws), _ptr(sq), sq.numel(), stream_ptr()), "rx_convT3d_bwd_weight_sq")
+    else:
+        check(load().rx_convT3d_bwd_weight(_code(x.dtype), byref(x.desc()), byref(dy.desc()), _ptr(dw), I3(*stride),
+                                           *_ws_args(ws), stream_ptr()), "rx_convT3d_bwd_weight")
+    return n_sq
 
 
 def instnorm_stats(y, stats, eps=1e-5, ws=None):
@@ -765,4 +785,4 @@
 convT3d_fwd = _hbm("convT_fwd", lambda x, w_fwd, bias, y, stride, ws=None: _tb(x) + _tb(y))(convT3d_fwd)
 convT3d_bwd_data = _hbm("convT_bwd_data", lambda dy, w_bwd, dx, stride, accumulate=False, ws=None:
                         _tb(dy) + _tb(dx) * (2 if accumulate else 1))(convT3d_bwd_data)
-convT3d_bwd_weight = _hbm("convT_bwd_weight", lambda x, dy, dw, stride, ws=None: _tb(x) + _tb(dy))(convT3d_bwd_weight)
+convT3d_bwd_weight = _hbm("convT_bwd_weight", lambda x, dy, dw, stride, ws=None, sq=None: _tb(x) + _tb(dy))(convT3d_bwd_weight)
diff --git a/multi-task-3d-resencoder-unet_amd/engine/plan.py b/multi-task-3d-resencoder-unet_amd/engine/plan.py
--- a/multi-task-3d-resencoder-unet_amd/engine/plan.py
+++ b/multi-task-3d-resencoder-unet_amd/engine/plan.py
@@ -2,6 +2,7 @@
 from typing import Callable, Dict, List, Optional
 
 import os
+import weakref
 
 import torch
 from torch import nn
@@ -127,6 +128,11 @@
         self._on_side = False
         self._use_gstore = False
         self._gflat_range = (0, 0)
+        self._sqflat = None
+        self._sq_views: Dict[int, torch.Tensor] = {}
+        self._sq_by_ptr: Dict[int, int] = {}
+        self._sq_n: Dict[int, int] = {}
+        self._sq_stamp = None
         self._pack_slots: List[int] = []
         self._unstable_params = False
         self._ws_refs: List[object] = []
@@ -866,7 +872,10 @@
                             elif kind == "stem":
                                 ops.stem_conv_bwd_weight(P._x, dy, dw, a["kernel"], ws)
                             else:
-                                ops.conv3d_bwd_weight(a["x"].act, dy, dw, a["kernel"], a["stride"], ws)
+                                sq = P._sq_span(a["widx"])
+                                n_sq = ops.conv3d_bwd_weight(a["x"].act, dy, dw, a["kernel"], a["stride"], ws, sq=sq)
+                                if sq is not None:
+                                    P._sq_n[a["widx"]] = n_sq
                             done(a["widx"])
                             if db is not None:
                                 ops.channel_sum(dy, db, ws)
@@ -909,7 +918,10 @@
                         db = new_grad(a["bidx"]) if a["bidx"] is not None else None
 
                         def launches(ws):
-                            ops.convT3d_bwd_weight(a["x"].act, gy, dw, a["stride"], ws)
+                            sq = P._sq_span(a["widx"])
+                            n_sq = ops.convT3d_bwd_weight(a["x"].act, gy, dw, a["stride"], ws, sq=sq)
+                            if sq is not None:
+                                P._sq_n[a["widx"]] = n_sq
                             done(a["widx"])
                             if db is not None:
                                 ops.channel_sum(gy, db, ws)
@@ -1100,11 +1112,39 @@
             for idx, o in offs.items():
                 p = self.params[idx]
                 self._gviews[idx] = self._gflat[o:o + p.numel()].view(p.shape)
+            soffs, m = {}, 0
+            for idx in offs:
+                p = self.params[idx]
+                if p.dim() == 5 and self.grad_order.count(idx) == 1 and idx not in self._pad_idx:
+                    soffs[idx] = (m, (p.shape[0] * p.shape[1] + 255) // 256 * p[0, 0].numel())
+                    m += soffs[idx][1]
+            self._sqflat = torch.zeros(max(m, 1), dtype=torch.float32, device=self.device)
+            self.bytes_alloc += self._sqflat.numel() * 4
+            for idx, (o, cap) in soffs.items():
+                self._sq_views[idx] = self._sqflat[o:o + cap]
+                self._sq_by_ptr[self._gviews[idx].data_ptr()] = idx
+            _SQ_PLANS.add(self)
         lo, hi = self._gflat_range
         for p in self.params:
             gr = p.grad
             if gr is not None and lo <= gr.data_ptr() < hi:
                 p.grad = gr.clone()
+
+    def _sq_span(self, idx):
+        return self._sq_views.get(idx) if self._use_gstore else None
+
+    def grad_sq_span(self, g):
+        if self._gflat is None or self._sq_stamp is None:
+            return None
+        if self._gflat._version != self._sq_stamp or g._version != self._sq_stamp:
+            return None
+        idx = self._sq_by_ptr.get(g.data_ptr())
+        if idx is None:
+            return None
+        n = self._sq_n.get(idx, 0)
+        if n <= 0 or n > self._sq_views[idx].numel() or g.numel() != self.params[idx].numel() or not g.is_contiguous():
+            return None
+        return self._sq_views[idx], n
 
     def _graphs_on(self):
         return (self.use_graphs and self.device.type == "cuda" and self.needs_grad
@@ -1335,9 +1375,11 @@
         self._ensure_side()
         self.net._weights_epoch = getattr(self.net, "_weights_epoch", 0) + 1
         self._grads = [None] * len(self.params)
+        self._sq_stamp = None
         if programs:
             sync = self.grad_sync
             self._use_gstore = sync is None
+            self._sq_n = {}
             if sync is None:
                 self._grad_store()
             else:
@@ -1351,7 +1393,13 @@
             if replayed and sync is None:
                 for idx in set(self.grad_order):
                     self._grads[idx] = self._gviews[idx]
+            if replayed:
+                self._sq_n = dict(st.get("sq_n", {}))
+            else:
+                st["sq_n"] = dict(self._sq_n)
             grads = self._backward_finish()
+            if sync is None:
+                self._sq_stamp = self._gflat._version
             return [t.detach() if t is not None else None for t in grads]
         self._use_gstore = False
         if self.grad_sync is not None:
@@ -1379,3 +1427,26 @@
         if "owned" not in st:
             st["owned"] = {t.data_ptr() for t in grads if t is not None}
         return [t.detach() if t is not None else None for t in grads]
+
+
+_SQ_PLANS = weakref.WeakSet()
+
+
+def grad_sq_spans(grads):
+    plans = [p for p in _SQ_PLANS if p._sq_stamp is not None]
+    if not plans:
+        return list(grads), []
+    scan, spans = [], []
+    for g in grads:
+        hit = None
+        ptr = g.data_ptr()
+        for p in plans:
+            lo, hi = p._gflat_range
+            if lo <= ptr < hi:
+                hit = p.grad_sq_span(g)
+                break
+        if hit is None:
+            scan.append(g)
+        else:
+            spans.append(hit)
+    return scan, spans
diff --git a/multi-task-3d-resencoder-unet_amd/training/optim/engine_adamw.py b/multi-task-3d-resencoder-unet_amd/training/optim/engine_adamw.py
--- a/multi-task-3d-resencoder-unet_amd/training/optim/engine_adamw.py
+++ b/multi-task-3d-resencoder-unet_amd/training/optim/engine_adamw.py
@@ -18,6 +18,7 @@
         self.model = model
         self._clip = None
         self._norm_ws = None
+        self._span_ws = None
 
     @torch.no_grad()
     def clip_grad_norm(self, max_norm, norm_type=2.0):
@@ -26,17 +27,31 @@
             return torch.zeros(())
         if (float(norm_type) == 2.0
                 and all(g.is_cuda and g.dtype == torch.float32 and g.is_contiguous() for g in grads)):
-            n = len(grads)
+            from ...engine import ops as _ops
+            from ...engine.plan import grad_sq_spans
+            scan, spans = grad_sq_spans(grads)
+            dev = grads[0].device
+            n = len(scan)
             VP, LP = ctypes.c_void_p * n, ctypes.c_long * n
-            numel = LP(*[g.numel() for g in grads])
-            need = load().rx_grad_norm_clip_partials(n, numel)
-            if self._norm_ws is None or self._norm_ws.numel() < need or self._norm_ws.device != grads[0].device:
-                self._norm_ws = torch.empty(int(need), dtype=torch.float32, device=grads[0].device)
-            out = torch.empty(2, dtype=torch.float32, device=grads[0].device)
-            from ...engine import ops as _ops
-            _ops.timed_bytes("grad_norm_clip", 4 * sum(g.numel() for g in grads), lambda: check(
-                load().rx_grad_norm_clip(n, VP(*[g.data_ptr() for g in grads]), numel, float(max_norm), _p(self._norm_ws),
-                                         self._norm_ws.numel(), _p(out), stream_ptr()), "rx_grad_norm_clip"))
+            numel = LP(*[g.numel() for g in scan])
+            need = load().rx_grad_norm_clip_partials(n, numel) if n else 0
+            if self._norm_ws is None or self._norm_ws.numel() < need or self._norm_ws.device != dev:
+                self._norm_ws = torch.empty(max(int(need), 1), dtype=torch.float32, device=dev)
+            out = torch.empty(2, dtype=torch.float32, device=dev)
+            if not spans:
+                _ops.timed_bytes("grad_norm_clip", 4 * sum(g.numel() for g in scan), lambda: check(
+                    load().rx_grad_norm_clip(n, VP(*[g.data_ptr() for g in scan]), numel, float(max_norm), _p(self._norm_ws),
+                                             self._norm_ws.numel(), _p(out), stream_ptr()), "rx_grad_norm_clip"))
+            else:
+                k = len(spans)
+                SP, SL = ctypes.c_void_p * k, ctypes.c_long * k
+                if self._span_ws is None or self._span_ws.numel() < k or self._span_ws.device != dev:
+                    self._span_ws = torch.empty(k, dtype=torch.float64, device=dev)
+                _ops.timed_bytes("grad_norm_clip", 4 * (sum(g.numel() for g in scan) + sum(c for _, c in spans)), lambda: check(
+                    load().rx_grad_norm_clip_spans(n, VP(*[g.data_ptr() for g in scan]), numel, k,
+                                                   SP(*[t.data_ptr() for t, _ in spans]), SL(*[c for _, c in spans]),
+                                                   float(max_norm), _p(self._norm_ws), self._norm_ws.numel(), _p(self._span_ws),
+                                                   _p(out), stream_ptr()), "rx_grad_norm_clip_spans"))
             self._clip = out[1:2]
             return out[0]
         norms = torch._foreach_norm(grads, norm_type)
```

After: 118.7 patches/s (median of 6 runs). About the same (+0.5%).
